# pmelchior/proxmin

Hardware: AMD Instinct MI355X
Metric: NMF iterations/sec at Y=16384x16384, K=64 (higher is better)
Workload: dtype f16x2r (fp16 split MFMA, fp32 accumulate: the residual from the high x high product + an exact K x K correction, two-term gradients; exact fp32's error class)

## Files before the change

### proxmin_amd/csrc/k_gfix.hip

```cpp
#include "pmx_common.h"

constexpr int GFIX_PARTS = 128;

struct GfixArgs {
    const float* X[2];
    int64_t rows[2];
    int K;
    const float* absmax;
    float* part;
    float* Q;
    float* out[2];
    int ld;
    int want[2];
    const DevStatus* status;
    long long* prof;
};
#define GFIX_STAMP(i) do { if (a.prof != nullptr && blockIdx.x == 0 && blockIdx.y == 0 && threadIdx.x == 0) a.prof[i] = wall_clock64(); } while (0)

typedef _Float16 gf16x8 __attribute__((ext_vector_type(8)));

__device__ __forceinline__ float gfix_scale(const float* absmax, int f, float* red) {
    float m = 0.f;
    for (int i = threadIdx.x; i < 256; i += blockDim.x) m = fmaxf(m, absmax[f * 256 + i]);
#pragma unroll
    for (int o = 32; o > 0; o >>= 1) m = fmaxf(m, __shfl_xor(m, o));
    if ((threadIdx.x & 63) == 0) red[threadIdx.x >> 6] = m;
    __syncthreads();
    float mx = red[0];
    for (int i = 1; i < (int)(blockDim.x >> 6); ++i) mx = fmaxf(mx, red[i]);
    int q = 0;
    (void)frexpf(mx, &q);
    return ldexpf(1.f, mx > 0.f ? 14 - q : 0);
}

template <int KT, int W>
__device__ __forceinline__ void gfix_gram_wave(const GfixArgs& a, int f, float* red) {
    constexpr int K = 32 * KT, TPW = KT * KT / 4, NB = KT == 2 ? 8 : 4;
    const int lane = threadIdx.x & 63, l31 = lane & 31, hi = lane >> 5;
    const int64_t rows = a.rows[f];
    const int64_t per = 16 * ((rows + 16 * GFIX_PARTS - 1) / (16 * GFIX_PARTS));
    const int64_t r0 = (int64_t)blockIdx.x * per, r1 = r0 + per < rows ? r0 + per : rows;
    const float* X = a.X[f] + 32 * 0 + l31;
    f32x16 acc0[TPW], accr[TPW];
#pragma unroll
    for (int t = 0; t < TPW; ++t)
#pragma unroll
        for (int i = 0; i < 16; ++i) { acc0[t][i] = 0.f; accr[t][i] = 0.f; }
    float v[NB][KT][8];
#define GFIX_REQUEST(rb_)                                                                          \
    _Pragma("unroll") for (int s = 0; s < NB; ++s)                                                 \
    _Pragma("unroll") for (int q = 0; q < 8; ++q) {                                                \
        const int64_t r = (rb_) + 16 * s + 8 * hi + q;                                             \
        _Pragma("unroll") for (int c = 0; c < KT; ++c) v[s][c][q] = r < r1 ? X[r * K + 32 * c] : 0.f; \
    }
    GFIX_STAMP(0);
    if (r0 < r1) { GFIX_REQUEST(r0) }
    const float sc = gfix_scale(a.absmax, f, red), un = 1.f / (sc * sc);
    GFIX_STAMP(1);
    for (int64_t rb = r0; rb < r1; rb += 16 * NB) {
        gf16x8 h[NB][KT], l[NB][KT];
#pragma unroll
        for (int s = 0; s < NB; ++s)
#pragma unroll
            for (int c = 0; c < KT; ++c)
#pragma unroll
                for (int q = 0; q < 8; ++q) {
                    const float x = v[s][c][q] * sc;
                    const _Float16 t = (_Float16)x;
                    h[s][c][q] = t;
                    l[s][c][q] = (_Float16)(x - (float)t);
                }
        if (rb + 16 * NB < r1) { GFIX_REQUEST(rb + 16 * NB) }
#pragma unroll
        for (int s = 0; s < NB; ++s)
#pragma unroll
            for (int t = 0; t < TPW; ++t) {
                constexpr int idx0 = W * TPW;
                const int ti = (idx0 + t) / KT, tj = (idx0 + t) % KT;
                acc0[t] = __builtin_amdgcn_mfma_f32_32x32x16_f16(h[s][ti], l[s][tj], acc0[t], 0, 0, 0);
                accr[t] = __builtin_amdgcn_mfma_f32_32x32x16_f16(l[s][ti], l[s][tj], accr[t], 0, 0, 0);
                acc0[t] = __builtin_amdgcn_mfma_f32_32x32x16_f16(h[s][ti], h[s][tj], acc0[t], 0, 0, 0);
                accr[t] = __builtin_amdgcn_mfma_f32_32x32x16_f16(l[s][ti], h[s][tj], accr[t], 0, 0, 0);
            }
    }
#undef GFIX_REQUEST
    GFIX_STAMP(2);
    float* out = a.part + ((int64_t)f * GFIX_PARTS + blockIdx.x) * 2 * K * K;
#pragma unroll
    for (int t = 0; t < TPW; ++t) {
        const int ti = (W * TPW + t) / KT, tj = (W * TPW + t) % KT;
#pragma unroll
        for (int i = 0; i < 16; ++i) {
            const int kp = 32 * ti + (i & 3) + 8 * (i >> 2) + 4 * hi, k = 32 * tj + l31;
            out[kp * K + k] = acc0[t][i] * un;
            out[K * K + kp * K + k] = accr[t][i] * un;
        }
    }
    GFIX_STAMP(3);
}
template <int W>
__device__ __forceinline__ void gfix_gram_wave_k128(const GfixArgs& a, int f, float* red, gf16x8* frag) {
    constexpr int K = 128, KT = 4, NB = 8;
    const int lane = threadIdx.x & 63, l31 = lane & 31, hi = lane >> 5;
    const int64_t rows = a.rows[f];
    const int64_t per = 16 * ((rows + 16 * GFIX_PARTS - 1) / (16 * GFIX_PARTS));
    const int64_t r0 = (int64_t)blockIdx.x * per, r1 = r0 + per < rows ? r0 + per : rows;
    const float* X = a.X[f] + 32 * W + l31;
    f32x16 acc0[KT], accr[KT];
#pragma unroll
    for (int t = 0; t < KT; ++t)
#pragma unroll
        for (int i = 0; i < 16; ++i) { acc0[t][i] = 0.f; accr[t][i] = 0.f; }
    float v[NB][8];
#define GFIX_REQUEST(rb_)                                                                          \
    _Pragma("unroll") for (int s = 0; s < NB; ++s)                                                 \
    _Pragma("unroll") for (int q = 0; q < 8; ++q) {                                                \
        const int64_t r = (rb_) + 16 * s + 8 * hi + q;                                             \
        v[s][q] = r < r1 ? X[r * K] : 0.f;                                                         \
    }
    if (r0 < r1) { GFIX_REQUEST(r0) }
    const float sc = gfix_scale(a.absmax, f, red), un = 1.f / (sc * sc);
    for (int64_t rb = r0; rb < r1; rb += 16 * NB) {
        gf16x8 h[NB], l[NB];
#pragma unroll
        for (int s = 0; s < NB; ++s) {
#pragma unroll
            for (int q = 0; q < 8; ++q) {
                const float x = v[s][q] * sc;
                const _Float16 t = (_Float16)x;
                h[s][q] = t;
                l[s][q] = (_Float16)(x - (float)t);
            }
            frag[((s * KT + W) * 2 + 0) * 64 + lane] = h[s];
            frag[((s * KT + W) * 2 + 1) * 64 + lane] = l[s];
        }
        if (rb + 16 * NB < r1) { GFIX_REQUEST(rb + 16 * NB) }
        __syncthreads();
#pragma unroll
        for (int s = 0; s < NB; ++s)
#pragma unroll
            for (int tj = 0; tj < KT; ++tj) {
                const gf16x8 hj = tj == W ? h[s] : frag[((s * KT + tj) * 2 + 0) * 64 + lane];
                const gf16x8 lj = tj == W ? l[s] : frag[((s * KT + tj) * 2 + 1) * 64 + lane];
                acc0[tj] = __builtin_amdgcn_mfma_f32_32x32x16_f16(h[s], lj, acc0[tj], 0, 0, 0);
                accr[tj] = __builtin_amdgcn_mfma_f32_32x32x16_f16(l[s], lj, accr[tj], 0, 0, 0);
                acc0[tj] = __builtin_amdgcn_mfma_f32_32x32x16_f16(h[s], hj, acc0[tj], 0, 0, 0);
                accr[tj] = __builtin_amdgcn_mfma_f32_32x32x16_f16(l[s], hj, accr[tj], 0, 0, 0);
            }
        __syncthreads();
    }
#undef GFIX_REQUEST
    float* out = a.part + ((int64_t)f * GFIX_PARTS + blockIdx.x) * 2 * K * K;
#pragma unroll
    for (int tj = 0; tj < KT; ++tj)
#pragma unroll
        for (int i = 0; i < 16; ++i) {
            const int kp = 32 * W + (i & 3) + 8 * (i >> 2) + 4 * hi, k = 32 * tj + l31;
            out[kp * K + k] = acc0[tj][i] * un;
            out[K * K + kp * K + k] = accr[tj][i] * un;
        }
}
template <int KT>
__global__ __launch_bounds__(256) void k_gfix_gram(GfixArgs a) {
    __shared__ float red[4];
    if (chain_halted(a.status)) return;
    const int f = blockIdx.y;
    if (!a.want[1 - f]) return;
    const int w = __builtin_amdgcn_readfirstlane(threadIdx.x >> 6);
    if constexpr (KT == 4) {
        extern __shared__ gf16x8 gfrag[];
        if (w == 0) gfix_gram_wave_k128<0>(a, f, red, gfrag);
        else if (w == 1) gfix_gram_wave_k128<1>(a, f, red, gfrag);
        else if (w == 2) gfix_gram_wave_k128<2>(a, f, red, gfrag);
        else gfix_gram_wave_k128<3>(a, f, red, gfrag);
    } else {
        if (w == 0) gfix_gram_wave<KT, 0>(a, f, red);
        else if (w == 1) gfix_gram_wave<KT, 1>(a, f, red);
        else if (w == 2) gfix_gram_wave<KT, 2>(a, f, red);
        else gfix_gram_wave<KT, 3>(a, f, red);
    }
}

__global__ __launch_bounds__(256) void k_gfix_reduce(GfixArgs a) {
    if (chain_halted(a.status)) return;
    const int f = blockIdx.y;
    if (!a.want[1 - f]) return;
    GFIX_STAMP(4);
    const int n = 2 * a.K * a.K;
    const int t = blockIdx.x * 256 + threadIdx.x, e = t >> 2, q = t & 3;
    static_assert(GFIX_PARTS == 128, "four threads x 32 partials");
    double s = 0.0;
    if (e < n) {
        const float* p = a.part + (int64_t)f * GFIX_PARTS * n + (int64_t)(q * 32) * n + e;
        float v[32];
#pragma unroll
        for (int i = 0; i < 32; ++i) v[i] = p[(int64_t)i * n];
#pragma unroll
        for (int i = 0; i < 32; ++i) s += (double)v[i];
    }
    const int base = threadIdx.x & 60;
    double tot = __shfl(s, base);
#pragma unroll
    for (int i = 1; i < 4; ++i) tot += __shfl(s, base + i);
    if (e < n && q == 0) a.Q[(int64_t)f * n + e] = (float)tot;
    GFIX_STAMP(5);
}

template <int KT>
__global__ __launch_bounds__(KT == 4 ? 512 : 256) void k_gfix_apply(GfixArgs a) {
    constexpr int K = 32 * KT, LDQ = K + 8;
    constexpr int NT = KT == 4 ? 512 : 256, NW = NT / 64;
    extern __shared__ _Float16 qpl[];
    __shared__ float red[8];
    if (chain_halted(a.status)) return;
    const int f = blockIdx.y;
    if (!a.want[f]) return;
    const int tid = threadIdx.x, lane = tid & 63, w = tid >> 6, l31 = lane & 31, hi = lane >> 5;
    const int64_t rows = a.rows[f];
    const float* X = a.X[f];
    float* out = a.out[f];
    const int64_t ntask = (rows + 31) / 32 * KT, stride = (int64_t)gridDim.x * NW;
    if ((int64_t)blockIdx.x * NW >= ntask) return;
    GFIX_STAMP(6);
    f32x4 x[K / 16][2];
#define GFIX_LOAD_X(t_)                                                                                                   \
    {                                                                                                                     \
        const int64_t row_ = ((t_) / KT) * 32 + l31;                                                                      \
        const f32x4* xr = reinterpret_cast<const f32x4*>(X + (row_ < rows ? row_ : 0) * K + 8 * hi);                       \
        _Pragma("unroll") for (int ks = 0; ks < K / 16; ++ks) { x[ks][0] = xr[4 * ks]; x[ks][1] = xr[4 * ks + 1]; }       \
    }
    const int64_t task0 = (int64_t)blockIdx.x * NW + w;
    if (task0 < ntask) GFIX_LOAD_X(task0)
    constexpr int TPK = NT / K, NBLK = K / 8 / TPK;
    const int kcol = tid % K, kb0 = tid / K;
    float tq[2][NBLK][8];
    {
        const float* src = a.Q + (int64_t)(1 - f) * 2 * K * K;
#pragma unroll
        for (int m = 0; m < 2; ++m)
#pragma unroll
            for (int i = 0; i < NBLK; ++i)
#pragma unroll
                for (int e = 0; e < 8; ++e) tq[m][i][e] = src[(size_t)m * K * K + (size_t)(8 * (kb0 + TPK * i) + e) * K + kcol];
    }
    float mx[2] = {0.f, 0.f};
#pragma unroll
    for (int m = 0; m < 2; ++m)
#pragma unroll
        for (int i = 0; i < NBLK; ++i)
#pragma unroll
            for (int e = 0; e < 8; ++e) mx[m] = fmaxf(mx[m], fabsf(tq[m][i][e]));
#pragma unroll
    for (int o = 32; o > 0; o >>= 1) { mx[0] = fmaxf(mx[0], __shfl_xor(mx[0], o)); mx[1] = fmaxf(mx[1], __shfl_xor(mx[1], o)); }
    __shared__ float redq[2][NW];
    if (lane == 0) { redq[0][w] = mx[0]; redq[1][w] = mx[1]; }
    const float sc = gfix_scale(a.absmax, f, red);
    GFIX_STAMP(7);
    float sq[2];
#pragma unroll
    for (int m = 0; m < 2; ++m) {
        float v = redq[m][0];
#pragma unroll
        for (int i = 1; i < NW; ++i) v = fmaxf(v, redq[m][i]);
        int q = 0;
        (void)frexpf(v, &q);
        sq[m] = ldexpf(1.f, v > 0.f ? 14 - q : 0);
    }
#pragma unroll
    for (int m = 0; m < 2; ++m) {
        _Float16* ph = qpl + (size_t)((1 - m) * 2) * K * LDQ + (size_t)kcol * LDQ;
        _Float16* pl = ph + (size_t)K * LDQ;
#pragma unroll
        for (int i = 0; i < NBLK; ++i) {
            gf16x8 h8, l8;
#pragma unroll
            for (int e = 0; e < 8; ++e) {
                const float v = tq[m][i][e] * sq[m];
                const _Float16 h = (_Float16)v;
                h8[e] = h;
                l8[e] = (_Float16)(v - (float)h);
            }
            *reinterpret_cast<gf16x8*>(ph + 8 * (kb0 + TPK * i)) = h8;
            *reinterpret_cast<gf16x8*>(pl + 8 * (kb0 + TPK * i)) = l8;
        }
    }
    __syncthreads();
    GFIX_STAMP(8);
    for (int64_t task = (int64_t)blockIdx.x * NW + w; task < ntask; task += stride) {
        const int64_t rt = task / KT;
        const int c = (int)(task % KT);
        const bool live = rt * 32 + l31 < rows;
        if (task != task0) GFIX_LOAD_X(task)
        f32x16 acc1, acc2;
#pragma unroll
        for (int i = 0; i < 16; ++i) { acc1[i] = 0.f; acc2[i] = 0.f; }
        const _Float16* qb = qpl + (size_t)(32 * c + l31) * LDQ + 8 * hi;
#pragma unroll
        for (int ks = 0; ks < K / 16; ++ks) {
            gf16x8 xh, xl, xm;
#pragma unroll
            for (int e = 0; e < 8; ++e) {
                const float v = (live ? x[ks][e >> 2][e & 3] : 0.f) * sc;
                const _Float16 h = (_Float16)v;
                const float r1 = v - (float)h;
                const _Float16 l = (_Float16)r1;
                xh[e] = h; xl[e] = l; xm[e] = (_Float16)(r1 - (float)l);
            }
            const gf16x8 qrh = *reinterpret_cast<const gf16x8*>(qb + 16 * ks);
            const gf16x8 qrl = *reinterpret_cast<const gf16x8*>(qb + (size_t)K * LDQ + 16 * ks);
            const gf16x8 q0h = *reinterpret_cast<const gf16x8*>(qb + (size_t)2 * K * LDQ + 16 * ks);
            const gf16x8 q0l = *reinterpret_cast<const gf16x8*>(qb + (size_t)3 * K * LDQ + 16 * ks);
            acc1 = __builtin_amdgcn_mfma_f32_32x32x16_f16(xl, qrh, acc1, 0, 0, 0);
            acc2 = __builtin_amdgcn_mfma_f32_32x32x16_f16(xm, q0h, acc2, 0, 0, 0);
            acc1 = __builtin_amdgcn_mfma_f32_32x32x16_f16(xh, qrl, acc1, 0, 0, 0);
            acc2 = __builtin_amdgcn_mfma_f32_32x32x16_f16(xl, q0l, acc2, 0, 0, 0);
            acc1 = __builtin_amdgcn_mfma_f32_32x32x16_f16(xh, qrh, acc1, 0, 0, 0);
            acc2 = __builtin_amdgcn_mfma_f32_32x32x16_f16(xl, q0h, acc2, 0, 0, 0);
        }
        const float u1 = 1.f / (sc * sq[1]), u2 = 1.f / (sc * sq[0]);
#pragma unroll
        for (int i = 0; i < 16; ++i) {
            const int64_t r = rt * 32 + (i & 3) + 8 * (i >> 2) + 4 * hi;
            if (r < rows) out[r * a.ld + 32 * c + l31] = acc1[i] * u1 + acc2[i] * u2;
        }
        GFIX_STAMP(9);
    }
#undef GFIX_LOAD_X
    GFIX_STAMP(10);
}

static hipError_t launch_gfix(const GfixArgs& a, hipStream_t s) {
    const int n = 2 * a.K * a.K;
    const size_t lds = (size_t)4 * a.K * (a.K + 8) * sizeof(_Float16);
    const int64_t rmax = a.rows[0] > a.rows[1] ? a.rows[0] : a.rows[1];
    const int nw = a.K == 128 ? 8 : 4;
    unsigned nb = (unsigned)(((rmax + 31) / 32 * (a.K / 32) + nw - 1) / nw);
    if (nb > (a.K == 128 ? 128u : 256u)) nb = a.K == 128 ? 128 : 256;
    if (a.K == 64) {
        hipError_t e = hipFuncSetAttribute((const void*)k_gfix_apply<2>, hipFuncAttributeMaxDynamicSharedMemorySize, (int)lds);
        if (e != hipSuccess) return e;
        hipLaunchKernelGGL(k_gfix_gram<2>, dim3(GFIX_PARTS, 2), dim3(256), 0, s, a);
        hipLaunchKernelGGL(k_gfix_reduce, dim3((n * 4 + 255) / 256, 2), dim3(256), 0, s, a);
        hipLaunchKernelGGL(k_gfix_apply<2>, dim3(nb, 2), dim3(256), lds, s, a);
    } else if (a.K == 128) {
        hipError_t e = hipFuncSetAttribute((const void*)k_gfix_apply<4>, hipFuncAttributeMaxDynamicSharedMemorySize, (int)lds);
        if (e != hipSuccess) return e;
        e = hipFuncSetAttribute((const void*)k_gfix_gram<4>, hipFuncAttributeMaxDynamicSharedMemorySize, 64 * 1024);
        if (e != hipSuccess) return e;
        hipLaunchKernelGGL(k_gfix_gram<4>, dim3(GFIX_PARTS, 2), dim3(256), 64 * 1024, s, a);
        hipLaunchKernelGGL(k_gfix_reduce, dim3((n * 4 + 255) / 256, 2), dim3(256), 0, s, a);
        hipLaunchKernelGGL(k_gfix_apply<4>, dim3(nb, 2), dim3(512), lds, s, a);
    } else return hipErrorInvalidValue;
    return hipGetLastError();
}
```

### proxmin_amd/csrc/k_update.hip

```cpp
#include <type_traits>
#include "pmx_common.h"

template <int CTRL>
__device__ __forceinline__ float dpp_f(float v) {
    return __builtin_bit_cast(float, __builtin_amdgcn_update_dpp(0, __builtin_bit_cast(int, v), CTRL, 0xf, 0xf, true));
}
template <int CTRL>
__device__ __forceinline__ double dpp_d(double v) {
    const unsigned long long u = __builtin_bit_cast(unsigned long long, v);
    const unsigned lo = (unsigned)__builtin_amdgcn_update_dpp(0, (int)(unsigned)u, CTRL, 0xf, 0xf, true);
    const unsigned hi = (unsigned)__builtin_amdgcn_update_dpp(0, (int)(unsigned)(u >> 32), CTRL, 0xf, 0xf, true);
    return __builtin_bit_cast(double, ((unsigned long long)hi << 32) | lo);
}
constexpr int DPP_XOR1 = 0xB1, DPP_XOR2 = 0x4E, DPP_HALF_MIRROR = 0x141, DPP_MIRROR = 0x140;
constexpr int SWZ_XOR16 = (0x10 << 10) | 0x1f;

constexpr int SWZ_XOR8 = (0x08 << 10) | 0x1f, SWZ_XOR4 = (0x04 << 10) | 0x1f;
__device__ __forceinline__ double swz16_d(double v) {
    const unsigned long long u = __builtin_bit_cast(unsigned long long, v);
    const unsigned lo = (unsigned)__builtin_amdgcn_ds_swizzle((int)(unsigned)u, SWZ_XOR16);
    const unsigned hi = (unsigned)__builtin_amdgcn_ds_swizzle((int)(unsigned)(u >> 32), SWZ_XOR16);
    return __builtin_bit_cast(double, ((unsigned long long)hi << 32) | lo);
}
template <class T, int G>
// ... 1440 lines not shown
                }
                cs[c] += x;
            }
        }
    ROW_LOOP_END
    double red[2] = {(double)d2, (double)n2};
    block_sum_store<2>(red, part_ptr(a.s.partials, SL_DIFF2, j) + blockIdx.x, (int64_t)2 * EW_BLOCKS, scratch);
    colsum_store<NC>(cs, a.colpart, j, sm);
    if (a.absmax_out != nullptr) {
        const double m = wave_max((double)xmax);
        __syncthreads();
        if ((threadIdx.x & 63) == 0) scratch[threadIdx.x >> 6] = m;
        __syncthreads();
        if (threadIdx.x == 0) {
            double mm = scratch[0];
            for (int q = 1; q < EW_WAVES; ++q) mm = fmax(mm, scratch[q]);
            a.absmax_out[j * EW_BLOCKS + blockIdx.x] = (float)mm;
        }
    }
}

struct AdaDecideArgs {
    AlphaArgs al;
    double* partials;
    double e_rel[2];
    int check_convergence;
    int has_prox[2];
    int host_tau[2];
};
__global__ __launch_bounds__(EW_THREADS) void k_ada_decide(AdaDecideArgs a) {
    __shared__ double scratch[EW_WAVES];
    DevStatus* st = a.al.status;
    if (chain_halted(st)) return;
    __shared__ int need;
    if (threadIdx.x == 0) need = st->need_sub[0] | st->need_sub[1];
    __syncthreads();
    if (need) {
        if (threadIdx.x == 0) {
            st->reason = HALT_NEED_SUB;
            __threadfence();
            st->halt = 1;
        }
        return;
    }
    double d[2] = {0, 0}, n[2] = {0, 0};
    if (a.check_convergence)
        for (int j = 0; j < 2; ++j) {
            d[j] = fold_partials(part_ptr(a.partials, SL_DIFF2, j), scratch);
            n[j] = fold_partials(part_ptr(a.partials, SL_NORM2, j), scratch);
        }
    compute_alpha(a.al);
    if (threadIdx.x == 0) {
        int all = 1;
        for (int j = 0; j < 2; ++j) {
            const int c = a.check_convergence ? (d[j] <= a.e_rel[j] * a.e_rel[j] * n[j]) : 0;
            st->conv[j] = c;
            st->norms[j][0] = d[j];
            st->norms[j][1] = n[j];
            all &= c;
            const int tau = a.has_prox[j] ? st->sub_tau[j] : a.host_tau[j];
            st->sub_total[j] += tau;
            st->last_tau[j] = tau;
            st->sub_done[j] = 0;
            st->sub_tau[j] = 0;
        }
        st->it_done += 1;
        if (a.check_convergence && all) {
            st->stopped = 1;
            st->reason = HALT_CONVERGED;
            __threadfence();
            st->halt = 1;
        }
    }
}

struct GridBar {
    unsigned cnt[8][16];
    unsigned top[16];
    unsigned gen[8][16];
    unsigned verdict[16];
    unsigned epoch[16];
};
__device__ __forceinline__ unsigned gb_load(const unsigned* p) { return __hip_atomic_load(p, __ATOMIC_RELAXED, __HIP_MEMORY_SCOPE_AGENT); }
__device__ __forceinline__ void gb_store(unsigned* p, unsigned v) { __hip_atomic_store(p, v, __ATOMIC_RELAXED, __HIP_MEMORY_SCOPE_AGENT); }
__device__ __forceinline__ void gb_arrive(GridBar* b, unsigned e, bool census) {
    const unsigned ng = 8, per = gridDim.x / ng, g = blockIdx.x & 7;
    const unsigned a = __hip_atomic_fetch_add(&b->cnt[g][0], 1u, __ATOMIC_RELAXED, __HIP_MEMORY_SCOPE_AGENT);
    if (a + 1 == per * e) {
        const unsigned t = __hip_atomic_fetch_add(&b->top[0], 1u, __ATOMIC_RELAXED, __HIP_MEMORY_SCOPE_AGENT);
        if (t + 1 == ng * e) {
            unsigned word = 2 * e;
            if (census) {
                unsigned expect = 2 * (e - 1);
                if (!__hip_atomic_compare_exchange_strong(&b->verdict[0], &expect, word, __ATOMIC_RELAXED, __ATOMIC_RELAXED, __HIP_MEMORY_SCOPE_AGENT)) word = expect;
            } else {
                gb_store(&b->verdict[0], word);
            }
            for (unsigned q = 0; q < ng; ++q) gb_store(&b->gen[q][0], word);
        }
    }
}
__device__ __forceinline__ unsigned gb_wait(GridBar* b, unsigned e, long long give_up_ticks) {
    const unsigned g = blockIdx.x & 7;
    const long long t0 = wall_clock64();
    for (;;) {
        const unsigned v = gb_load(&b->gen[g][0]);
        if ((v >> 1) >= e) return v;
        __builtin_amdgcn_s_sleep(4);
        if (give_up_ticks > 0 && wall_clock64() - t0 > give_up_ticks) {
            unsigned expect = 2 * (e - 1);
            if (__hip_atomic_compare_exchange_strong(&b->verdict[0], &expect, 2 * e + 1, __ATOMIC_RELAXED, __ATOMIC_RELAXED, __HIP_MEMORY_SCOPE_AGENT)) {
                for (unsigned q = 0; q < 8; ++q) gb_store(&b->gen[q][0], 2 * e + 1);
                return 2 * e + 1;
            }
            give_up_ticks = 0;
        }
    }
}
__device__ __forceinline__ void gb_sync(GridBar* b, unsigned e, DevStatus* st) {
    asm volatile("s_waitcnt vmcnt(0)" ::: "memory");
    __syncthreads();
    if (threadIdx.x == 0) {
        gb_arrive(b, e, false);
        const unsigned g = blockIdx.x & 7;
        const long long t0 = wall_clock64();
        for (unsigned spins = 1; (gb_load(&b->gen[g][0]) >> 1) < e; ++spins) {
            __builtin_amdgcn_s_sleep(4);
            if ((spins & 1023u) == 0 && wall_clock64() - t0 > 10000000) {
                st->tail_fault = 2;
                st->reason = HALT_ERROR;
                __threadfence();
                st->halt = 1;
                break;
            }
        }
    }
    __syncthreads();
}

constexpr int TAIL_NT = 4;
struct TailArgs {
    MomentArgs m;
    ProxSeq prox[2];
    double e_rel[2];
    int prox_max_iter;
    double* colpart;
    float* absmax_out;
    AlphaArgs al;
    int decide_check;
    GridBar* bar;
    int slots[2];
    long long* prof;
    int prof_fine;
};
template <int NC>
__global__ __launch_bounds__(EW_THREADS) void k_ada_tail(TailArgs a) {
    __shared__ double scratch[4 * TAIL_NT * EW_WAVES];
    __shared__ double dbuf[EW_BLOCKS + 8];
    __shared__ unsigned s_word;
    extern __shared__ float lds[];
    static_assert(EW_BLOCKS == 2 * MAXK, "the step-size phase gives one (block, component) to each workgroup");
    DevStatus* st = a.m.status;
    if (chain_halted(st)) return;
    const int tid = threadIdx.x, l32 = tid & 31;
    const int K = a.m.K;
    GridBar* bar = a.bar;
    unsigned ep = bar->epoch[0];
    int nstamp = 0;
    auto stamp = [&]() { if (a.prof != nullptr && blockIdx.x == 0 && tid == 0) a.prof[nstamp++] = wall_clock64(); };
    stamp();
    if (tid == 0) gb_arrive(bar, ep + 1, true);
    const int64_t hw = ((int64_t)blockIdx.x * EW_THREADS + tid) >> 5;
    const int64_t nhw = ((int64_t)EW_BLOCKS * EW_THREADS) >> 5;
    const int nslot = a.slots[0] + a.slots[1];
    float* Lx = lds;
    float* Lz = lds + (size_t)nslot * NC * EW_THREADS;
    float* Lp = lds + (size_t)2 * nslot * NC * EW_THREADS;
    auto slot = [&](int j, int i, int c) { return ((size_t)((j ? a.slots[0] : 0) + i) * NC + c) * EW_THREADS + tid; };
    bool ok[NC];
#pragma unroll
    for (int c = 0; c < NC; ++c) ok[c] = l32 + 32 * c < K;
    const MomentScalars ms = moment_scalars(a.m);
    const bool any_prox = a.m.has_prox[0] || a.m.has_prox[1];

    float g_pre[NC], x_pre[NC];
    const bool pre = a.slots[0] > 0 && hw < a.m.rows[0];
    if (pre) {
        load_grad<NC>(g_pre, ok, a.m.slab[0], a.m.rows[0], K, hw, l32);
#pragma unroll
        for (int c = 0; c < NC; ++c) x_pre[c] = ok[c] ? a.m.X[0][hw * K + l32 + 32 * c] : 0.f;
    }
    float alpha0[NC], alpha1[NC];
#pragma unroll
    for (int c = 0; c < NC; ++c) {
        alpha0[c] = ok[c] ? st->alpha[0][l32 + 32 * c] : 0.f;
        alpha1[c] = ok[c] ? st->alpha[1][l32 + 32 * c] : 0.f;
    }
    const int last_tau0 = st->last_tau[0], last_tau1 = st->last_tau[1];
    {
        if (tid == 0) s_word = gb_wait(bar, ep + 1, 200000);
        __syncthreads();
        if (s_word & 1u) {
            if (blockIdx.x == 0 && tid == 0) {
                st->tail_fault = 1;
                st->reason = HALT_ERROR;
                __threadfence();
                st->halt = 1;
            }
            return;
        }
        ep += 1;
    }
    stamp();
    float mpsi0 = -1.f, mpsi1 = -1.f;
    for (int j = 0; j < 2; ++j) {
        const int64_t rows = a.m.rows[j];
        float alpha[NC];
#pragma unroll
        for (int c = 0; c < NC; ++c) alpha[c] = j ? alpha1[c] : alpha0[c];
        float maxpsi = -1.f;
        for (int i = 0; i < a.slots[j]; ++i) {
            const int64_t r = hw + (int64_t)i * nhw;
            if (r >= rows) break;
            float g[NC], xo[NC];
            if (j == 0 && i == 0 && pre) {
#pragma unroll
                for (int c = 0; c < NC; ++c) { g[c] = g_pre[c]; xo[c] = x_pre[c]; }
            } else {
                load_grad<NC>(g, ok, a.m.slab[j], rows, K, r, l32);
#pragma unroll
                for (int c = 0; c < NC; ++c) xo[c] = ok[c] ? a.m.X[j][r * K + l32 + 32 * c] : 0.f;
            }
#pragma unroll
            for (int c = 0; c < NC; ++c) {
                if (!ok[c]) continue;
                const int64_t e = r * K + l32 + 32 * c;
                float psi;
                const float xn = moment_elem(a.m, ms, j, e, g[c], alpha[c], xo[c], psi);
                if (a.m.check_convergence) a.m.Xp[j][e] = xo[c];
                Lx[slot(j, i, c)] = xn;
                Lp[slot(j, i, c)] = psi;
                maxpsi = nanmaxf(maxpsi, psi);
            }
        }
        if (j) mpsi1 = maxpsi; else mpsi0 = maxpsi;
    }
    {
        const double mv0 = wave_nanmax((double)mpsi0), mv1 = wave_nanmax((double)mpsi1);
        __syncthreads();
        if ((tid & 63) == 0) { scratch[tid >> 6] = mv0; scratch[EW_WAVES + (tid >> 6)] = mv1; }
        __syncthreads();
        if (tid == 0 || tid == 64) {
            const int jj = tid >> 6;
            double m = scratch[jj * EW_WAVES];
            for (int q = 1; q < EW_WAVES; ++q) m = nanmax(m, scratch[jj * EW_WAVES + q]);
            sc1_store(part_ptr(a.m.partials, SL_MAXPSI, jj) + blockIdx.x, m);
        }
    }

    int tau0 = 0, tau1 = 0;
    stamp();
    if (any_prox) {
        gb_sync(bar, ++ep, st);
        stamp();
        bool done0 = !a.m.has_prox[0], done1 = !a.m.has_prox[1];
        double mp0, mp1;
        {
            const int lane = tid & 63;
            const double* q0 = part_ptr(a.m.partials, SL_MAXPSI, 0);
            const double* q1 = part_ptr(a.m.partials, SL_MAXPSI, 1);
            double u0[EW_BLOCKS / 64], u1[EW_BLOCKS / 64];
#pragma unroll
            for (int i = 0; i < EW_BLOCKS / 64; ++i) { u0[i] = sc1_load(q0 + i * 64 + lane); u1[i] = sc1_load(q1 + i * 64 + lane); }
            double v0 = -1.0, v1 = -1.0;
#pragma unroll
            for (int i = 0; i < EW_BLOCKS / 64; ++i) { v0 = nanmax(v0, u0[i]); v1 = nanmax(v1, u1[i]); }
            mp0 = wave_nanmax(v0);
            mp1 = wave_nanmax(v1);
        }
        stamp();
        auto steps = [&](int j, float (&gam)[NC], float (&rat)[NC]) {
            const float mp = (float)(j ? mp1 : mp0);
#pragma unroll
            for (int c = 0; c < NC; ++c) {
                const float al = j ? alpha1[c] : alpha0[c];
                gam[c] = al / mp;
                rat[c] = gam[c] / al;
            }
        };
        auto passes = [&](int j, int i, int n, bool first_round, const float (&gam)[NC], const float (&rat)[NC], float (&z)[NC],
                          auto sums_c, float (&d2)[TAIL_NT], float (&n2)[TAIL_NT]) {
            constexpr bool SUMS = decltype(sums_c)::value;
            float x[NC], ps[NC];
#pragma unroll
            for (int c = 0; c < NC; ++c) {
                x[c] = Lx[slot(j, i, c)];
                ps[c] = Lp[slot(j, i, c)];
                z[c] = first_round ? x[c] : Lz[slot(j, i, c)];
                if (!ok[c]) { x[c] = 0.f; ps[c] = 0.f; z[c] = 0.f; }
            }
#pragma unroll
            for (int q = 0; q < TAIL_NT; ++q) {
                if (q < n) {
                    float v[NC];
#pragma unroll
                    for (int c = 0; c < NC; ++c) v[c] = z[c] - rat[c] * ps[c] * (z[c] - x[c]);
                    prox_row(v, ok, a.prox[j], gam);
#pragma unroll
                    for (int c = 0; c < NC; ++c) {
                        if (SUMS && ok[c]) {
                            const float d = v[c] - z[c];
                            d2[q] += d * d;
                            n2[q] += z[c] * z[c];
                        }
                        z[c] = v[c];
                    }
                }
            }
        };
        using yes = std::integral_constant<bool, true>;
        using no = std::integral_constant<bool, false>;
        int t0_0 = 0, t0_1 = 0;
        for (int round = 0; !(done0 && done1); ++round) {
            int nt_0 = TAIL_NT, nt_1 = TAIL_NT;
            if (round == 0) {
                const int l0 = last_tau0, l1 = last_tau1;
                nt_0 = l0 >= 1 && l0 <= TAIL_NT ? l0 : TAIL_NT;
                nt_1 = l1 >= 1 && l1 <= TAIL_NT ? l1 : TAIL_NT;
            }
            double red[2][2 * TAIL_NT];
#pragma unroll
            for (int q = 0; q < 2 * TAIL_NT; ++q) { red[0][q] = 0.0; red[1][q] = 0.0; }
            for (int j = 0; j < 2; ++j) {
                if (j ? done1 : done0) continue;
                const int nt = j ? nt_1 : nt_0;
                float gam[NC], rat[NC];
                steps(j, gam, rat);
                float d2[TAIL_NT], n2[TAIL_NT];
#pragma unroll
                for (int q = 0; q < TAIL_NT; ++q) { d2[q] = 0.f; n2[q] = 0.f; }
                for (int i = 0; i < a.slots[j]; ++i) {
                    if (hw + (int64_t)i * nhw >= a.m.rows[j]) break;
                    float z[NC];
                    passes(j, i, nt, round == 0, gam, rat, z, yes{}, d2, n2);
                    if (round == 0) {
#pragma unroll
                        for (int c = 0; c < NC; ++c) Lz[slot(j, i, c)] = z[c];
                    }
                }
#pragma unroll
                for (int q = 0; q < TAIL_NT; ++q) {
                    if (j) { red[1][2 * q] = (double)d2[q]; red[1][2 * q + 1] = (double)n2[q]; }
                    else { red[0][2 * q] = (double)d2[q]; red[0][2 * q + 1] = (double)n2[q]; }
                }
                if (round == 0 && a.prof_fine) stamp();
            }
            {
                static_assert(4 * TAIL_NT == 16, "wave_sum16");
                const int lane = tid & 63, w = tid >> 6;
                double all[16];
#pragma unroll
                for (int q = 0; q < 2 * TAIL_NT; ++q) { all[q] = red[0][q]; all[2 * TAIL_NT + q] = red[1][q]; }
                const double tot = wave_sum16(all);
                __syncthreads();
                if (lane < 16) scratch[lane * EW_WAVES + w] = tot;
                __syncthreads();
                if (tid < 4 * TAIL_NT) {
                    const int jj = tid / (2 * TAIL_NT), q = tid - jj * 2 * TAIL_NT;
                    if (!(jj ? done1 : done0)) {
                        double sum = 0.0;
                        for (int u = 0; u < EW_WAVES; ++u) sum += scratch[tid * EW_WAVES + u];
                        sc1_store(part_ptr(a.m.partials, SL_SUBR0 + 2 * TAIL_NT * (round & 3), jj) + blockIdx.x + (int64_t)q * 2 * EW_BLOCKS, sum);
                    }
                }
            }
            if (round == 0) stamp();
            gb_sync(bar, ++ep, st);
            if (round == 0) stamp();
            for (int j = 0; j < 2; ++j) {
                if (j ? done1 : done0) continue;
                const int nt = j ? nt_1 : nt_0, t0 = j ? t0_1 : t0_0;
                const int w = tid >> 6;
                __syncthreads();
                if (w < 2 * nt) {
// ... 602 lines not shown
};
template <int NC>
__global__ __launch_bounds__(EW_THREADS) void k_shard_pack_split(PackSplitArgs a) {
    const int64_t ex0 = a.sncol * a.K;
    const int64_t sc0 = ex0 + (int64_t)a.KP * a.KP + 2 * MAXK;
    if (chain_halted(a.status)) {
        if (blockIdx.x == 0 && threadIdx.x < a.world) a.comm[threadIdx.x * a.chunk + sc0 + SHARD_HALT_SLOT] = 1.f;
        return;
    }
    const int K = a.K;
    if (blockIdx.x >= PACK_XWG) {
        if (a.fold_grad) {
            const int l32 = threadIdx.x & 31;
            const int64_t hw_ = ((int64_t)(blockIdx.x - PACK_XWG) * EW_THREADS + threadIdx.x) >> 5;
            const int64_t nhw_ = ((int64_t)EW_BLOCKS * EW_THREADS) >> 5;
            for (int64_t r = hw_; r < a.N; r += nhw_) {
                bool ok[NC];
                float g[NC];
#pragma unroll
                for (int c = 0; c < NC; ++c) ok[c] = l32 + 32 * c < K;
                load_grad<NC>(g, ok, a.slabS, a.N, K, r, l32);
                const int q = (int)r / (int)a.sncol;
                float* dst = a.comm + (int64_t)q * a.chunk + (int64_t)((int)r - q * (int)a.sncol) * K;
#pragma unroll
                for (int c = 0; c < NC; ++c)
                    if (ok[c]) dst[l32 + 32 * c] = g[c];
            }
        }
        return;
    }
    const int t = threadIdx.x;
    if (blockIdx.x < 2) {
        const int j = blockIdx.x;
        __shared__ double asum[ALPHA_NG][MAXK];
        colsum_fold(a.colpart + (int64_t)j * EW_BLOCKS * MAXK, K, false, asum);
        if (t < MAXK) {
            double s = 0.0;
            for (int q = 0; q < ALPHA_NG; ++q) s += asum[q][t];
            const float v = (float)s;
            for (int q = 0; q < a.world; ++q) a.comm[q * a.chunk + ex0 + (int64_t)a.KP * a.KP + j * MAXK + t] = v;
        }
        return;
    }
    const double* const four[4] = {a.partials + ((int64_t)SL_DIFF2 * 2 + 0) * EW_BLOCKS, a.partials + ((int64_t)SL_NORM2 * 2 + 0) * EW_BLOCKS,
                                   a.partials + ((int64_t)SL_DIFF2 * 2 + 1) * EW_BLOCKS, a.partials + ((int64_t)SL_NORM2 * 2 + 1) * EW_BLOCKS};
    double sums[4];
    fold_partials_many<4>(four, sums);
    for (int q = 0; q < a.world; ++q) {
        float* ex = a.comm + q * a.chunk + ex0;
        if (a.gramA != nullptr)
            for (int e = t; e < a.KP * a.KP; e += EW_THREADS) ex[e] = (float)a.gramA[e];
        else if (a.zero_gram)
            for (int e = t; e < a.KP * a.KP; e += EW_THREADS) ex[e] = 0.f;
        if (t < 32) ex[a.KP * a.KP + 2 * MAXK + t] = t < 4 ? (float)sums[t] : 0.f;
    }
}
struct ShardPostSplitArgs {
    DevStatus* status;
    const float* extras;
    int64_t rows_global[2];
    int K;
    int use_fixed;
    float fixed[2];
    double e_rel[2];
    int check_convergence;
    int have_prev;
};
__global__ __launch_bounds__(EW_THREADS) void k_shard_post_split(ShardPostSplitArgs a) {
    DevStatus* st = a.status;
    if (chain_halted(st)) return;
    const float* sc = a.extras + 2 * MAXK;
    if (sc[SHARD_HALT_SLOT] > 0.5f) {
        if (threadIdx.x == 0) {
            st->reason = HALT_PEER;
            __threadfence();
            st->halt = 1;
        }
        return;
    }
    const int t = threadIdx.x;
    if (a.use_fixed != 2 && t < a.K)
        for (int j = 0; j < 2; ++j)
            st->alpha[j][t] = a.use_fixed ? a.fixed[j] : (float)((double)a.extras[j * MAXK + t] / (double)a.rows_global[j]) / 10.f;
    if (a.check_convergence && a.have_prev && t == 0) {
        const double dA = (double)sc[0], nA = (double)sc[1], dS = (double)sc[2], nS = (double)sc[3];
        const int cA = dA <= a.e_rel[0] * a.e_rel[0] * nA;
        const int cS = dS <= a.e_rel[1] * a.e_rel[1] * nS;
        st->conv[0] = cA;
        st->conv[1] = cS;
        st->norms[0][0] = dA; st->norms[0][1] = nA;
        st->norms[1][0] = dS; st->norms[1][1] = nS;
        if (cA && cS) {
            st->stopped = 1;
            st->reason = HALT_CONVERGED;
            __threadfence();
            st->halt = 1;
        }
    }
}

#define DISPATCH_NC(K, KERNEL, grid, stream, args)                                               \
    do {                                                                                         \
        if ((K) <= 32) hipLaunchKernelGGL(KERNEL<1>, grid, dim3(EW_THREADS), 0, stream, args);    \
        else if ((K) <= 64) hipLaunchKernelGGL(KERNEL<2>, grid, dim3(EW_THREADS), 0, stream, args); \
        else hipLaunchKernelGGL(KERNEL<4>, grid, dim3(EW_THREADS), 0, stream, args);              \
    } while (0)

#define DISPATCH_NC_ME(K, me, KERNEL, grid, stream, args)                                                          \
    do {                                                                                                           \
        if (!(me)) DISPATCH_NC(K, KERNEL, grid, stream, args);                                                     \
        else if ((K) <= 32) hipLaunchKernelGGL((KERNEL<1, true>), grid, dim3(EW_THREADS), 0, stream, args);         \
        else if ((K) <= 64) hipLaunchKernelGGL((KERNEL<2, true>), grid, dim3(EW_THREADS), 0, stream, args);         \
        else hipLaunchKernelGGL((KERNEL<4, true>), grid, dim3(EW_THREADS), 0, stream, args);                        \
    } while (0)

void launch_fold(const FoldArgs& a, int nblocks_y, hipStream_t s) { DISPATCH_NC(a.K, k_fold, dim3(EW_BLOCKS, nblocks_y), s, a); }
void launch_prox_apply(const ProxArgs& a, hipStream_t s) { DISPATCH_NC_ME(a.K, seq_has_me(a.prox), k_prox_apply, dim3(EW_BLOCKS), s, a); }
void launch_pgm_update(const PgmArgs& a, hipStream_t s) {
    DISPATCH_NC_ME(a.K, seq_has_me(a.prox[0]) || seq_has_me(a.prox[1]), k_pgm_update, dim3(a.nbx > 0 ? a.nbx : EW_BLOCKS, 2), s, a);
}
void launch_pgm_unity(const PgmUnityArgs& a, hipStream_t s) {
    DISPATCH_NC_ME(a.u.K, seq_has_me(a.u.prox[0]) || seq_has_me(a.u.prox[1]), k_pgm_unity, dim3(a.u.nbx > 0 ? a.u.nbx : EW_BLOCKS, 2), s, a);
}
void launch_bb_reduce(const BBArgs& a, hipStream_t s) { DISPATCH_NC(a.K, k_bb_reduce, dim3(EW_BLOCKS, 2), s, a); }
void launch_bb_step(const BBStepArgs& a, hipStream_t s) { hipLaunchKernelGGL(k_bb_step, dim3(1), dim3(EW_THREADS), 0, s, a); }
void launch_bt_update(const BtArgs& a, hipStream_t s) { DISPATCH_NC_ME(a.K, seq_has_me(a.prox[0]) || seq_has_me(a.prox[1]), k_bt_update, dim3(EW_BLOCKS, 2), s, a); }
void launch_bt_collect(const BtCollectArgs& a, hipStream_t s) { hipLaunchKernelGGL(k_bt_collect, dim3(1), dim3(EW_THREADS), 0, s, a); }
void launch_bt_finish(const BtFinishArgs& a, hipStream_t s) { hipLaunchKernelGGL(k_bt_finish, dim3(EW_BLOCKS, 2), dim3(EW_THREADS), 0, s, a); }
void launch_pgm_decide(const DecideArgs& a, hipStream_t s) { hipLaunchKernelGGL(k_pgm_decide, dim3(1), dim3(EW_THREADS), 0, s, a); }
void launch_colsum(const ColsumArgs& a, hipStream_t s) { DISPATCH_NC(a.K, k_colsum, dim3(EW_BLOCKS, 2), s, a); }
void launch_alpha_init(const AlphaArgs& a, hipStream_t s) { hipLaunchKernelGGL(k_alpha_init, dim3(1), dim3(EW_THREADS), 0, s, a); }
void launch_colscale(const ColScaleArgs& a, hipStream_t s) { DISPATCH_NC(a.K, k_colscale, dim3(EW_BLOCKS), s, a); }
void launch_ada_moment(const MomentArgs& a, hipStream_t s) { DISPATCH_NC(a.K, k_ada_moment, dim3(EW_BLOCKS, 2), s, a); }
#define DISPATCH_NC_NT(K, NT, ME, KERNEL, grid, stream, args)                                                      \
    do {                                                                                                           \
        if ((K) <= 32) hipLaunchKernelGGL((KERNEL<1, NT, ME>), grid, dim3(EW_THREADS), 0, stream, args);            \
        else if ((K) <= 64) hipLaunchKernelGGL((KERNEL<2, NT, ME>), grid, dim3(EW_THREADS), 0, stream, args);       \
        else hipLaunchKernelGGL((KERNEL<4, NT, ME>), grid, dim3(EW_THREADS), 0, stream, args);                      \
    } while (0)
template <bool ME>
static void launch_ada_sub_t(const SubArgs& a, hipStream_t s) {
    if (a.nt == 1) DISPATCH_NC_NT(a.K, 1, ME, k_ada_sub, dim3(EW_BLOCKS, 2), s, a);
    else if (a.nt == 4) DISPATCH_NC_NT(a.K, 4, ME, k_ada_sub, dim3(EW_BLOCKS, 2), s, a);
    else DISPATCH_NC_NT(a.K, SUB_NT_MAX, ME, k_ada_sub, dim3(EW_BLOCKS, 2), s, a);
}
void launch_ada_sub(const SubArgs& a, hipStream_t s) {
    if (seq_has_me(a.prox[0]) || seq_has_me(a.prox[1])) launch_ada_sub_t<true>(a, s);
    else launch_ada_sub_t<false>(a, s);
}
void launch_ada_finish(const FinishArgs& a, hipStream_t s) {
    DISPATCH_NC_ME(a.s.K, seq_has_me(a.s.prox[0]) || seq_has_me(a.s.prox[1]), k_ada_finish, dim3(EW_BLOCKS, 2), s, a);
}
void launch_ada_decide(const AdaDecideArgs& a, hipStream_t s) { hipLaunchKernelGGL(k_ada_decide, dim3(1), dim3(EW_THREADS), 0, s, a); }
static size_t ada_tail_lds_bytes(const TailArgs& a) {
    const int NC = a.m.K <= 32 ? 1 : (a.m.K <= 64 ? 2 : 4);
    const size_t arr = (size_t)(a.slots[0] + a.slots[1]) * NC * EW_THREADS * sizeof(float);
    return 2 * arr + std::max(arr, (size_t)(EW_THREADS / 32) * MAXK * sizeof(float));
}
constexpr size_t ADA_TAIL_LDS_MAX = 160 * 1024 - 6 * 1024;
template <int NC>
static hipError_t launch_ada_tail_t(const TailArgs& a, hipStream_t s) {
    const size_t lds = ada_tail_lds_bytes(a);
    hipError_t e = hipFuncSetAttribute((const void*)k_ada_tail<NC>, hipFuncAttributeMaxDynamicSharedMemorySize, (int)lds);
    if (e != hipSuccess) return e;
    hipLaunchKernelGGL(k_ada_tail<NC>, dim3(EW_BLOCKS), dim3(EW_THREADS), lds, s, a);
    return hipGetLastError();
}
hipError_t launch_ada_tail(const TailArgs& a, hipStream_t s) {
    if (a.m.K <= 32) return launch_ada_tail_t<1>(a, s);
    if (a.m.K <= 64) return launch_ada_tail_t<2>(a, s);
    return launch_ada_tail_t<4>(a, s);
}
void launch_bsdmm_update(const BsdmmArgs& a, hipStream_t s) {
    bool me = seq_has_me(a.prox_f);
    for (int i = 0; i < a.n_g && i < PMX_MAX_G; ++i) me = me || seq_has_me(a.prox_g[i]);
    DISPATCH_NC_ME(a.K, me, k_bsdmm_update, dim3(EW_BLOCKS), s, a);
}
void launch_shard_pack(const PackArgs& a, hipStream_t s) { DISPATCH_NC(a.K, k_shard_pack, dim3(EW_BLOCKS + PACK_XWG), s, a); }
void launch_shard_gram_in(const GramInArgs& a, hipStream_t s) { hipLaunchKernelGGL(k_shard_gram_in, dim3((a.n + 255) / 256), dim3(256), 0, s, a); }
void launch_shard_post(const ShardPostArgs& a, hipStream_t s) { hipLaunchKernelGGL(k_shard_post, dim3(1), dim3(EW_THREADS), 0, s, a); }
void launch_shard_pack_split(const PackSplitArgs& a, hipStream_t s) { DISPATCH_NC(a.K, k_shard_pack_split, dim3(EW_BLOCKS + PACK_XWG), s, a); }
void launch_shard_post_split(const ShardPostSplitArgs& a, hipStream_t s) { hipLaunchKernelGGL(k_shard_post_split, dim3(1), dim3(EW_THREADS), 0, s, a); }
void launch_bsdmm_decide(const BsdmmDecideArgs& a, hipStream_t s) { hipLaunchKernelGGL(k_bsdmm_decide, dim3(1), dim3(EW_THREADS), 0, s, a); }
```

### proxmin_amd/csrc/pmx_api.hip

```cpp
#include <stdarg.h>
#include <stdio.h>
#include <string.h>
#include <math.h>
#include <vector>
#include <string>
#include <algorithm>
#include <mutex>

#include <fcntl.h>
#include <sys/file.h>
#include <unistd.h>
#include <dlfcn.h>
#include <link.h>
#include "pmx_common.h"
#include "chain_link.h"
#include "k_grad.hip"
#include "k_grad_bf16.hip"
#include "k_grad_k128.hip"
#include "k_grad_f16_k32.hip"
#include "k_grad_f32pc.hip"
#include "k_update.hip"
#include "k_gram.hip"
#include "k_gfix.hip"
#include "k_small_f64.hip"
#include "k_grad_f64.hip"
#include "k_big_f64.hip"
#include "k_xfer.hip"

static thread_local char g_err[512] = "";
void pmx_set_error(const char* fmt, ...) {
    va_list ap;
    va_start(ap, fmt);
    vsnprintf(g_err, sizeof(g_err), fmt, ap);
    va_end(ap);
}
#define FAIL(code, ...)            \
    do {                           \
        pmx_set_error(__VA_ARGS__); \
        return (code);             \
    } while (0)

enum Algo { ALG_NONE = 0, ALG_PGM, ALG_ADAPROX, ALG_BSDMM };

struct pmx_ctx {
    int device = 0;
    hipStream_t stream = nullptr;
    bool own_stream = false;
    int64_t M = 0, N = 0, K = 0;
    int KP = 0, mode = PMX_MODE_F32;
    int64_t rows[2] = {0, 0};

    const float* Y = nullptr;
    float* Yown = nullptr;
    int64_t ldY = 0;
    bool haveY = false;
    int64_t Mk = 0, Nk = 0;
    int64_t rowsK[2] = {0, 0};
    bool framed = false;
    int64_t Kk = 0;
    float* Xk[2] = {nullptr, nullptr};

    float* X[2] = {nullptr, nullptr};
    float* G[2] = {nullptr, nullptr};
    float* Xe[2] = {nullptr, nullptr};
    float* Xp[2] = {nullptr, nullptr};
    float* Mm[2] = {nullptr, nullptr};
    float* Vv[2] = {nullptr, nullptr};
    float* Vh[2] = {nullptr, nullptr};
    float* Psi[2] = {nullptr, nullptr};
    float* zb[2][2] = {{nullptr, nullptr}, {nullptr, nullptr}};
    float* Zg[2][PMX_MAX_G] = {};
    float* Ug[2][PMX_MAX_G] = {};
    float* bbX[2] = {nullptr, nullptr};
    float* bbG[2] = {nullptr, nullptr};

    bool f64 = false;
    double* Yd = nullptr;
    double* Xd[2] = {nullptr, nullptr};
    double* Xed[2] = {nullptr, nullptr};
    double* Gd[2] = {nullptr, nullptr};
    double* slabd[2] = {nullptr, nullptr};
    double* Md[2] = {nullptr, nullptr};
    double* Vd[2] = {nullptr, nullptr};
    double* Vhd[2] = {nullptr, nullptr};
    double* Xpd[2] = {nullptr, nullptr};
    double* Psid[2] = {nullptr, nullptr};
    double* zd[2] = {nullptr, nullptr};
    double* alpha64 = nullptr;
    double* Zd[2][PMX_MAX_G] = {};
    double* Ud[2][PMX_MAX_G] = {};
    int t64x = 0, t64y = 0;
    bool f64big = false;
    double* gramPart64 = nullptr;
    double* colpart64 = nullptr;
    int nsplit64[2] = {1, 1}, bps64[2] = {1, 1};
    int nsub64 = 4;
    bool Wd_on = false;
    double* Xprevd[2] = {nullptr, nullptr};
    double* Wd = nullptr;
    double* Xk64[2] = {nullptr, nullptr};
    int64_t ldY64 = 0;

    bool host_grad = false;
    float* Tg[2][PMX_MAX_G] = {};
    float* Tf[2] = {};
    unsigned long long* k1prof = nullptr;
    K1Kind k1 = K1_F32;
    bool k1_pairs = true;
    float rangeRatio = 65536.f;
    int rangeFaults = 0;
    int f16_r3 = 0;
    float* fixPart = nullptr;
    float* fixQ = nullptr;
    float* fixSlab[2] = {nullptr, nullptr};
    long long* fixProf = nullptr;
    bool fix_on = false;
    bool k1_sync_check = false;
    int ncu = 0;
    _Float16* A16[2] = {nullptr, nullptr};
    float* absmax = nullptr;
    float ymax = 0.f;
    float wmax = 1.f;
    bool absmax_by_finish = false;
    bool gram_by_update = false;
    bool bsd_decide_pending = false;
    BsdmmDecideArgs bsd_decide{};
    bool gram_fresh[2] = {false, false};
    bool gram_in_update = true;
    bool fold_in_k1 = true;
    K1GramFold k1_fold{};
    bool decide_pending = false;
    __bf16* Bp[2] = {nullptr, nullptr};
    __bf16* Bt[2] = {nullptr, nullptr};
    int64_t rowsPad[2] = {0, 0};
    GradPlan plan{};
    int chainL = 0;
    unsigned* chainFlags = nullptr;
    unsigned chainSeq = 0;
    int nSlabA = 0;
    int nSlabS = 0;
    int chainFaults = 0;
    int hook_inject_k1 = 0;
    std::string hook_tail_lockfile;
    bool tail_fused = false;
    GridBar* gridbar = nullptr;
    long long* tailprof = nullptr;
    unsigned* tickets = nullptr;
    bool pgm_long = false;
    double* unityPart = nullptr;
    unsigned ticketLaunches = 0;
    int tailFaults = 0;
    float* slab[2] = {nullptr, nullptr};
    const float* W = nullptr;
    int64_t ldW = 0;
    float* Wown = nullptr;
    double* lossPart = nullptr;
    int nloss = 0;

    double* partials = nullptr;
    double* colpart = nullptr;
    float* gramPart = nullptr;
    double* gramG = nullptr;
    double* eigQ = nullptr;
    DevStatus* dstatus = nullptr;
    DevStatus* hstatus = nullptr;

    Algo algo = ALG_NONE;
    pmx_pgm_params pgm{};
    pmx_adaprox_params ada{};
    pmx_bsdmm_params bsd{};
    int host_tau[2] = {0, 0};
    int it = 0;
    double nest_t = 1.0;
    double btT[2] = {1.0, 1.0};
    double bt_fprev = 0.0, bt_fnow = 0.0;
    bool bt_grad_fresh = false;
    int bt_pending = 0;
    int bt_trial = 3;
    float* btBuf[2] = {nullptr, nullptr};
    float omega_cur = 0.f;
    int nsub_guess = 2;
    int sub_nt = SUB_NT_MAX;
    struct SubRec { int it = -1, nt = 0, enq = 0; } sub_rec[64];
    std::vector<void*> allocs;

    bool timing = false;
    int timing_stride = 1;
    unsigned timing_seq = 0;
    std::vector<hipEvent_t> ev;
    size_t ev_used = 0;

    int ph_every = 0;
    unsigned ph_seq = 0;
    bool ph_cur = false, ph_prev = false;
    std::vector<hipEvent_t> ph_ev;
    std::vector<int> ph_mark;

    int rank = 0, world = 1;
    int64_t M_global = 0;
    float* comm = nullptr;
    bool comm_gram_dirty = true;
    bool shard_grad_from_comm = false;
    bool ssplit = false;
    int64_t scol0 = 0, sncol = 0;
    float* comm_out = nullptr;
    pmx_prox* tabs = nullptr;
    bool tab_set[PMX_MAX_TABLES] = {};
    float* stepArr[2] = {nullptr, nullptr};
    int step_arr_mask = 0;
    void* rccl_comm = nullptr;
    int rccl_rank = 0, rccl_world = 0;
};

static int dalloc(pmx_ctx* c, void** p, size_t bytes, bool zero = true) {
    if (*p) return PMX_OK;
    hipError_t e = hipMalloc(p, bytes ? bytes : 16);
    if (e != hipSuccess) FAIL(PMX_E_NOMEM, "hipMalloc(%zu) failed: %s", bytes, hipGetErrorString(e));
    c->allocs.push_back(*p);
    if (zero) HIP_CHECK(hipMemsetAsync(*p, 0, bytes ? bytes : 16, c->stream));
    return PMX_OK;
}
template <class T>
static int dallocT(pmx_ctx* c, T** p, size_t count, bool zero = true) { return dalloc(c, (void**)p, count * sizeof(T), zero); }

static ProxSeq to_dev(const pmx_proxseq& p, const pmx_prox* tab) {
    ProxSeq d{};
    d.n = p.n;
    d.repeat = p.repeat < 1 ? 1 : p.repeat;
    for (int i = 0; i < PMX_MAX_SEQ; ++i) d.seq[i] = p.seq[i];
    d.tab = tab;
    return d;
}
static bool prox_long_axis(const pmx_proxseq& p) {
    for (int i = 0; i < p.n && i < PMX_MAX_SEQ; ++i)
        if ((p.seq[i].op == PMX_PROX_UNITY || p.seq[i].op == PMX_PROX_UNITY_PLUS) && p.seq[i].unit != 0) return true;
    return false;
}
static bool seq_is_projection(const pmx_proxseq& p) {
    for (int i = 0; i < p.n; ++i) {
        const pmx_prox& q = p.seq[i];
        const bool box = q.op == PMX_PROX_ID || q.op == PMX_PROX_ZERO || q.op == PMX_PROX_PLUS ||
                         ((q.op == PMX_PROX_MIN || q.op == PMX_PROX_MAX || q.op == PMX_PROX_HARD || q.op == PMX_PROX_HARD_PLUS) && !q.relative);
        if (!box) return false;
    }
    return true;
}
static bool prox_has_max_entropy(const pmx_proxseq& p) {
    for (int i = 0; i < p.n && i < PMX_MAX_SEQ; ++i)
        if (p.seq[i].op == PMX_PROX_MAX_ENTROPY || p.seq[i].op == PMX_PROX_COMPONENTS) return true;
    return false;
}
static bool row_op_ok(int op) {
    return op == PMX_PROX_ID || op == PMX_PROX_ZERO || op == PMX_PROX_PLUS || (op >= PMX_PROX_MIN && op <= PMX_PROX_MAX_ENTROPY);
}
static int check_prox(const pmx_proxseq& p, const char* what, bool long_axis_ok = false, const bool* tab_set = nullptr, int ntables = -1) {
    if (p.n < 0 || p.n > PMX_MAX_SEQ) FAIL(PMX_E_INVALID, "%s: bad operator count %d", what, p.n);
    for (int i = 0; i < p.n; ++i) {
        const pmx_prox& q = p.seq[i];
        if (q.op < PMX_PROX_ID || q.op > PMX_PROX_COMPONENTS) FAIL(PMX_E_INVALID, "%s: unknown prox op %d", what, q.op);
        if (q.op != PMX_PROX_COMPONENTS) continue;
        if (q.unit != 0) FAIL(PMX_E_INVALID, "%s: PMX_PROX_COMPONENTS works along the components of a row (unit 0)", what);
        if (q.reserved < 1) FAIL(PMX_E_INVALID, "%s: PMX_PROX_COMPONENTS without a table (reserved = 1 + its index)", what);
        if (tab_set != nullptr && q.reserved > PMX_MAX_TABLES)
            FAIL(PMX_E_UNSUPPORTED, "%s: table %d of at most %d per-component tables", what, q.reserved - 1, PMX_MAX_TABLES);
        if (tab_set != nullptr ? !tab_set[q.reserved - 1] : q.reserved > ntables)
            FAIL(PMX_E_INVALID, "%s: PMX_PROX_COMPONENTS names table %d, which has not been set (pmx_prox_table)", what, q.reserved - 1);
    }
    if (prox_long_axis(p) && !long_axis_ok)
        FAIL(PMX_E_UNSUPPORTED, "%s: prox_unity along the row dimension (numpy axis=0 on A / axis=1 on S) needs a grid-wide sum per "
                                "application: pgm / FISTA run it inside the update chain (pmx_pgm_begin without line search, user prox, "
                                "row sharding or fp64), every other solver entry point does not contain it (the host wrappers apply it "
                                "between kernel launches through pmx_prox_apply)", what);
    return PMX_OK;
}

static int apply_prox_standalone(float* X, int64_t rows, int K, const pmx_proxseq& prox, const float* step_k, double* colpart, hipStream_t stream,
                                 const pmx_prox* tab = nullptr) {
    bool along_rows = false;
    for (int i = 0; i < prox.n; ++i)
        along_rows |= (prox.seq[i].op == PMX_PROX_UNITY || prox.seq[i].op == PMX_PROX_UNITY_PLUS) && prox.seq[i].unit != 0;
    ProxArgs a{};
    a.X = X;
    a.rows = rows;
    a.K = K;
    for (int k = 0; k < K; ++k) a.stepk[k] = step_k[k];
    if (!along_rows) {
        a.prox = to_dev(prox, tab);
        launch_prox_apply(a, stream);
        return PMX_OK;
    }
    const int repeat = prox.repeat < 1 ? 1 : prox.repeat;
    for (int r = 0; r < repeat; ++r)
        for (int i = 0; i < prox.n; ++i) {
            pmx_proxseq one{};
            one.n = 1; one.repeat = 1; one.seq[0] = prox.seq[i];
            const bool rows_unity = (one.seq[0].op == PMX_PROX_UNITY || one.seq[0].op == PMX_PROX_UNITY_PLUS) && one.seq[0].unit != 0;
            if (!rows_unity) {
// ... 204 lines not shown
        if (rc == PMX_OK) rc = dallocT(c, &c->fixQ, (size_t)4 * c->Kk * c->Kk);
        for (int j = 0; j < 2 && rc == PMX_OK; ++j) rc = dallocT(c, &c->fixSlab[j], (size_t)c->rowsK[j] * c->Kk);
        if (rc == PMX_OK && getenv("PMX_GFIX_PROF")) rc = dallocT(c, &c->fixProf, 16);
    }
    for (int t = 0; t < 2 && rc == PMX_OK && c->k1 == K1_F16_K128; ++t) rc = dallocT(c, &c->A16[t], (size_t)Mk * c->Kk, c->framed || c->Kk != K);
    for (int j = 0; j < 2 && rc == PMX_OK && c->Kk != K; ++j) rc = dallocT(c, &c->Xk[j], (size_t)c->rowsK[j] * c->Kk);
    if (c->k1 == K1_BF16 || c->k1 == K1_BF16_V7 || c->k1 == K1_F16_V8) {
        for (int j = 0; j < 2 && rc == PMX_OK; ++j) {
            c->rowsPad[j] = (c->rowsK[j] + 127) / 128 * 128;
            rc = dallocT(c, &c->Bp[j], (size_t)3 * c->rowsPad[j] * c->KP, false);
            if (rc == PMX_OK) rc = dallocT(c, &c->Bt[j], (size_t)2 * c->KP * c->rowsPad[j], false);
        }
    }
    for (int j = 0; j < 2 && rc == PMX_OK; ++j) {
        rc = dallocT(c, &c->X[j], (size_t)c->rowsK[j] * K);
        if (rc == PMX_OK) rc = dallocT(c, &c->G[j], (size_t)c->rows[j] * K);
    }
    if (rc == PMX_OK) rc = dallocT(c, &c->slab[0], (size_t)c->nSlabA * Mk * c->Kk, false);
    if (rc == PMX_OK) rc = dallocT(c, &c->slab[1], (size_t)c->plan.nSlabS * Nk * c->Kk, false);
    if (rc == PMX_OK) rc = dallocT(c, &c->lossPart, (size_t)2 * c->plan.gridX * c->plan.gridY);
    if (rc == PMX_OK) rc = dallocT(c, &c->partials, (size_t)SL_COUNT * 2 * EW_BLOCKS);
    if (rc == PMX_OK) rc = dallocT(c, &c->colpart, (size_t)2 * EW_BLOCKS * MAXK);
    if (rc == PMX_OK) rc = dallocT(c, &c->gramPart, (size_t)2 * GRAM_BLOCKS * c->KP * c->KP);
    if (rc == PMX_OK) rc = dallocT(c, &c->gramG, (size_t)2 * c->KP * c->KP);
    if (rc == PMX_OK) rc = dallocT(c, &c->eigQ, (size_t)2 * c->KP * c->KP);
    if (rc == PMX_OK) rc = dallocT(c, &c->dstatus, 1);
    if (rc == PMX_OK) {
        hipError_t e = hipHostMalloc((void**)&c->hstatus, sizeof(DevStatus), hipHostMallocDefault);
        if (e != hipSuccess) { pmx_set_error("hipHostMalloc: %s", hipGetErrorString(e)); rc = PMX_E_NOMEM; }
    }
    if (rc != PMX_OK) { pmx_ctx_destroy(c); return rc; }
    *out = c;
    return PMX_OK;
}

extern "C" int pmx_ctx_destroy(pmx_ctx* c) {
    if (!c) return PMX_OK;
    (void)hipSetDevice(c->device);
    if (c->stream) (void)hipStreamSynchronize(c->stream);
    (void)pmx_comm_destroy(c);
    for (void* p : c->allocs) (void)hipFree(p);
    for (auto& e : c->ev) (void)hipEventDestroy(e);
    for (auto& e : c->ph_ev) (void)hipEventDestroy(e);
    if (c->hstatus) (void)hipHostFree(c->hstatus);
    if (c->own_stream && c->stream) (void)hipStreamDestroy(c->stream);
    delete c;
    return PMX_OK;
}

extern "C" int pmx_set_timing(pmx_ctx* c, int on) {
    if (!c) FAIL(PMX_E_INVALID, "ctx is NULL");
    HIP_CHECK(hipSetDevice(c->device));
    HIP_CHECK(hipStreamSynchronize(c->stream));
    if (on && c->ev.empty()) {
        c->ev.resize(2 * 8192);
        for (auto& e : c->ev) HIP_CHECK(hipEventCreate(&e));
    }
    c->timing = on != 0;
    c->timing_stride = on > 1 ? on : 1;
    c->timing_seq = 0;
    c->ev_used = 0;
    return PMX_OK;
}

extern "C" int pmx_get_timing(pmx_ctx* c, double* total_ms, int* launches) {
    if (!c || !total_ms || !launches) FAIL(PMX_E_INVALID, "NULL argument");
    HIP_CHECK(hipSetDevice(c->device));
    HIP_CHECK(hipStreamSynchronize(c->stream));
    std::vector<float> d;
    float mx = 0.f;
    for (size_t i = 0; i + 1 < c->ev_used; i += 2) {
        float ms = 0.f;
        HIP_CHECK(hipEventElapsedTime(&ms, c->ev[i], c->ev[i + 1]));
        d.push_back(ms);
        mx = std::max(mx, ms);
    }
    double tot = 0.0;
    int n = 0;
    for (float ms : d)
        if (ms >= 0.05f * mx) { tot += ms; ++n; }
    *total_ms = tot;
    *launches = n;
    return PMX_OK;
}

static int phase_mark(pmx_ctx* c, int m) {
    if (c->ph_every <= 0) return PMX_OK;
    if (m == 0) {
        if (c->ph_prev && c->ph_mark.size() < c->ph_ev.size()) {
            HIP_CHECK(hipEventRecord(c->ph_ev[c->ph_mark.size()], c->stream));
            c->ph_mark.push_back(6);
        }
        c->ph_cur = (c->ph_seq++ % (unsigned)c->ph_every) == 0 && c->ph_mark.size() + 8 <= c->ph_ev.size();
        c->ph_prev = c->ph_cur;
    }
    if (!c->ph_cur) return PMX_OK;
    HIP_CHECK(hipEventRecord(c->ph_ev[c->ph_mark.size()], c->stream));
    c->ph_mark.push_back(m);
    return PMX_OK;
}
extern "C" int pmx_set_phase_timing(pmx_ctx* c, int every) {
    if (!c) FAIL(PMX_E_INVALID, "ctx is NULL");
    HIP_CHECK(hipSetDevice(c->device));
    HIP_CHECK(hipStreamSynchronize(c->stream));
    if (every > 0 && c->ph_ev.empty()) {
        c->ph_ev.resize(4096);
        for (auto& e : c->ph_ev) HIP_CHECK(hipEventCreate(&e));
    }
    c->ph_every = every > 0 ? every : 0;
    c->ph_seq = 0;
    c->ph_cur = c->ph_prev = false;
    c->ph_mark.clear();
    return PMX_OK;
}
extern "C" int pmx_get_phase_timing(pmx_ctx* c, double ms[6], int* iterations) {
    if (!c || !ms || !iterations) FAIL(PMX_E_INVALID, "NULL argument");
    HIP_CHECK(hipSetDevice(c->device));
    HIP_CHECK(hipStreamSynchronize(c->stream));
    double sum[6] = {0, 0, 0, 0, 0, 0};
    int cnt[6] = {0, 0, 0, 0, 0, 0};
    for (size_t i = 0; i + 1 < c->ph_mark.size(); ++i) {
        const int a = c->ph_mark[i], b = c->ph_mark[i + 1];
        if (b != a + 1 || a > 5) continue;
        float t = 0.f;
        HIP_CHECK(hipEventElapsedTime(&t, c->ph_ev[i], c->ph_ev[i + 1]));
        sum[a] += t;
        cnt[a] += 1;
    }
    for (int a = 0; a < 6; ++a) ms[a] = cnt[a] ? sum[a] / cnt[a] : 0.0;
    *iterations = cnt[0];
    return PMX_OK;
}

extern "C" int pmx_k1_info(pmx_ctx* c, int info[8]) {
    if (!c || !info) FAIL(PMX_E_INVALID, "NULL argument");
    const K1Inst inst = k1_instance(c->k1, c->f16_r3, c->W != nullptr, true, c->k1_pairs);
    switch (c->k1) {
    case K1_F32: info[0] = 0; break;
    case K1_BF16: case K1_BF16_V7: info[0] = 1; break;
    case K1_F16_V8: info[0] = inst == K1_V7 ? 1 : inst == K1_HH ? 11 : inst == K1_R3 ? 9 : 2; break;
    case K1_SMALL: info[0] = 4; break;
    case K1_F16_K128: info[0] = inst == K1_HH ? 12 : 5; break;
    case K1_F32PC: info[0] = 6; break;
    case K1_F64_SMALL: info[0] = 7; break;
    case K1_F16_K32: info[0] = inst == K1_R3 ? 10 : 8; break;
    case K1_F64_BIG: info[0] = 13; break;
    }
    info[1] = c->chainL;
    info[2] = c->nSlabA;
    info[3] = c->nSlabS;
    info[4] = c->plan.gridX;
    info[5] = c->plan.gridY;
    info[6] = c->plan.RP;
    info[7] = c->chainFaults + 1000 * c->tailFaults + (c->tail_fused ? 1000000 : 0) + 10000000 * std::min(c->rangeFaults, 9);
    return PMX_OK;
}

extern "C" int pmx_k1_frame(pmx_ctx* c, int64_t frame[3]) {
    if (!c || !frame) FAIL(PMX_E_INVALID, "NULL argument");
    frame[0] = c->f64 ? c->M : c->Mk;
    frame[1] = c->f64 ? c->N : c->Nk;
    frame[2] = c->f64 ? c->K : c->Kk;
    return PMX_OK;
}

extern "C" int pmx_ctx_sync(pmx_ctx* c) {
    if (!c) FAIL(PMX_E_INVALID, "ctx is NULL");
    HIP_CHECK(hipStreamSynchronize(c->stream));
    return PMX_OK;
}

static int measure_ymax(pmx_ctx* c) {
    if (!k1_fp16(c->k1)) return PMX_OK;
    launch_absmax_pitched(c->Y, c->ldY, c->M, c->N, c->absmax + 512, c->stream);
    HIP_CHECK(hipGetLastError());
    float h[256];
    HIP_CHECK(hipMemcpyAsync(h, c->absmax + 512, sizeof(h), hipMemcpyDeviceToHost, c->stream));
    HIP_CHECK(hipStreamSynchronize(c->stream));
    float m = 0.f;
    for (float v : h) m = v > m ? v : m;
    if (!(m < 3.0e38f)) FAIL(PMX_E_INVALID, "Y contains non-finite values");
    c->ymax = m;
    return PMX_OK;
}

static int own_frame_copy(pmx_ctx* c, float** own, const float* src, int64_t ld, hipMemcpyKind kind) {
    if (!*own) {
        int rc = dallocT(c, own, (size_t)c->Mk * c->Nk, c->framed);
        if (rc != PMX_OK) return rc;
    }
    HIP_CHECK(hipMemcpy2DAsync(*own, c->Nk * sizeof(float), src, ld * sizeof(float), c->N * sizeof(float), c->M, kind, c->stream));
    HIP_CHECK(hipStreamSynchronize(c->stream));
    return PMX_OK;
}

extern "C" int pmx_set_Y_host(pmx_ctx* c, const float* Y, int64_t ld) {
    if (!c || !Y) FAIL(PMX_E_INVALID, "NULL argument");
    if (c->f64) FAIL(PMX_E_UNSUPPORTED, "an fp64 context takes Y through pmx_set_Y_host_f64");
    if (ld < c->N) FAIL(PMX_E_INVALID, "ld %lld < N", (long long)ld);
    HIP_CHECK(hipSetDevice(c->device));
    int rc = own_frame_copy(c, &c->Yown, Y, ld, hipMemcpyHostToDevice);
    if (rc != PMX_OK) return rc;
    c->Y = c->Yown;
    c->ldY = c->Nk;
    c->haveY = true;
    return measure_ymax(c);
}

extern "C" int pmx_set_Y_device(pmx_ctx* c, const float* dY, int64_t ld, int copy) {
    if (!c || !dY) FAIL(PMX_E_INVALID, "NULL argument");
    if (c->f64) FAIL(PMX_E_UNSUPPORTED, "an fp64 context takes Y through pmx_set_Y_host_f64");
    if (ld < c->N) FAIL(PMX_E_INVALID, "ld %lld < N", (long long)ld);
    HIP_CHECK(hipSetDevice(c->device));
    if (copy || c->framed) {
        int rc = own_frame_copy(c, &c->Yown, dY, ld, hipMemcpyDeviceToDevice);
        if (rc != PMX_OK) return rc;
        c->Y = c->Yown;
        c->ldY = c->Nk;
    } else {
        c->Y = dY;
        c->ldY = ld;
    }
    c->haveY = true;
    return measure_ymax(c);
}

static int measure_wmax(pmx_ctx* c) {
    c->wmax = 1.f;
    if (!k1_fp16(c->k1) || !c->W) return PMX_OK;
    launch_absmax_pitched(c->W, c->ldW, c->M, c->N, c->absmax + 512, c->stream);
    HIP_CHECK(hipGetLastError());
    float h[256];
    HIP_CHECK(hipMemcpyAsync(h, c->absmax + 512, sizeof(h), hipMemcpyDeviceToHost, c->stream));
    HIP_CHECK(hipStreamSynchronize(c->stream));
    float m = 1.f;
    for (float v : h) m = v > m ? v : m;
    if (!(m < 3.0e38f)) FAIL(PMX_E_INVALID, "W contains non-finite values");
    c->wmax = m;
    return PMX_OK;
}

static int set_W_common(pmx_ctx* c, const float* W, int64_t ld, int from_host, int copy) {
    if (c && c->f64 && W) FAIL(PMX_E_UNSUPPORTED, "weights are not implemented in fp64 contexts");
    if (!c) FAIL(PMX_E_INVALID, "ctx is NULL");
    if (!W) { c->W = nullptr; c->ldW = 0; c->wmax = 1.f; return PMX_OK; }
    if (ld < c->N) FAIL(PMX_E_INVALID, "ld %lld < N", (long long)ld);
    if (c->k1 == K1_F16_K32) FAIL(PMX_E_UNSUPPORTED, "k_grad_f16_k32 takes no weights; create the context with PMX_MODE_F32");
    if (c->k1 == K1_BF16)
        FAIL(PMX_E_UNSUPPORTED, "a weighted likelihood in a split-precision mode needs K = 64 with M %% 128 = 0, N %% 256 = 0 or K = 128 with M %% 128 = 0, N %% 128 = 0; create the context with PMX_MODE_F32");
    if (c->comm) FAIL(PMX_E_UNSUPPORTED, "weights are not supported in row-sharded runs");
    HIP_CHECK(hipSetDevice(c->device));
    if (from_host || copy || c->framed) {
        int rc = own_frame_copy(c, &c->Wown, W, ld, from_host ? hipMemcpyHostToDevice : hipMemcpyDeviceToDevice);
        if (rc != PMX_OK) return rc;
        c->W = c->Wown;
        c->ldW = c->Nk;
    } else {
        c->W = W;
        c->ldW = ld;
    }
    return measure_wmax(c);
}
extern "C" int pmx_set_W_host(pmx_ctx* c, const float* W, int64_t ld) { return set_W_common(c, W, ld, 1, 1); }
extern "C" int pmx_set_W_device(pmx_ctx* c, const float* dW, int64_t ld, int copy) { return set_W_common(c, dW, ld, 0, copy); }

static int buf_lookup(pmx_ctx* c, int buf, float*** slot, int64_t* count, bool create) {
    if (c->f64) FAIL(PMX_E_UNSUPPORTED, "an fp64 context has no float arrays: pmx_upload_f64 / pmx_download_f64");
    int j;
    float** p = nullptr;
    if (buf >= PMX_BUF_A && buf <= PMX_BUF_PSI_ST) {
        j = buf & 1;
        switch (buf >> 1) {
            case 0: p = &c->X[j]; break;
            case 1: p = &c->G[j]; break;
            case 2: p = &c->Mm[j]; break;
            case 3: p = &c->Vv[j]; break;
            case 4: p = &c->Vh[j]; break;
            case 5: p = (c->algo == ALG_PGM && c->pgm.accelerated) ? &c->Xe[j] : &c->X[j]; break;
            case 6: p = &c->Xp[j]; break;
            case 7: p = &c->Psi[j]; break;
        }
    } else if (buf >= PMX_BUF_Z0 && buf < PMX_BUF_Z0 + 2 * PMX_MAX_G) {
        j = (buf - PMX_BUF_Z0) / PMX_MAX_G;
        p = &c->Zg[j][(buf - PMX_BUF_Z0) % PMX_MAX_G];
    } else if (buf >= PMX_BUF_U0 && buf < PMX_BUF_U0 + 2 * PMX_MAX_G) {
        j = (buf - PMX_BUF_U0) / PMX_MAX_G;
        p = &c->Ug[j][(buf - PMX_BUF_U0) % PMX_MAX_G];
    } else if (buf >= PMX_BUF_TG0 && buf < PMX_BUF_TG0 + 2 * PMX_MAX_G) {
        j = (buf - PMX_BUF_TG0) / PMX_MAX_G;
        p = &c->Tg[j][(buf - PMX_BUF_TG0) % PMX_MAX_G];
    } else if (buf == PMX_BUF_STEP_A || buf == PMX_BUF_STEP_ST) {
        j = buf - PMX_BUF_STEP_A;
        p = &c->stepArr[j];
    } else if (buf == PMX_BUF_BT_A || buf == PMX_BUF_BT_ST) {
        j = buf - PMX_BUF_BT_A;
        p = &c->btBuf[j];
    } else FAIL(PMX_E_INVALID, "unknown buffer id %d", buf);
    *count = c->rows[j] * c->K;
    if (!*p) {
        if (!create) FAIL(PMX_E_STATE, "buffer %d has not been created yet", buf);
        int rc = dallocT(c, p, (size_t)c->rowsK[j] * c->K);
        if (rc != PMX_OK) return rc;
    }
    *slot = p;
    return PMX_OK;
}

// ... 172 lines not shown
extern "C" int pmx_factor_from_device(pmx_ctx* c, int buf, const void* dptr, int64_t stride0, int64_t stride1, int is_f64) {
    if (c) { c->absmax_by_finish = false; c->gram_by_update = false; c->bt_grad_fresh = false; }
    void* arr; int64_t rows, sr, sk;
    int rc = xfer_lookup(c, buf, dptr, stride0, stride1, is_f64, true, &arr, &rows, &sr, &sk);
    if (rc != PMX_OK) return rc;
    HIP_CHECK(hipDeviceSynchronize());
    if (c->f64) launch_xfer<double>((double*)arr, (double*)const_cast<void*>(dptr), rows, c->K, sr, sk, false, c->stream);
    else launch_xfer<float>((float*)arr, (float*)const_cast<void*>(dptr), rows, c->K, sr, sk, false, c->stream);
    HIP_CHECK(hipGetLastError());
    HIP_CHECK(hipStreamSynchronize(c->stream));
    return PMX_OK;
}

extern "C" int pmx_factor_to_device(pmx_ctx* c, int buf, void* dptr, int64_t stride0, int64_t stride1, int is_f64) {
    void* arr; int64_t rows, sr, sk;
    int rc = xfer_lookup(c, buf, dptr, stride0, stride1, is_f64, false, &arr, &rows, &sr, &sk);
    if (rc != PMX_OK) return rc;
    if (c->f64) launch_xfer<double>((double*)arr, (double*)dptr, rows, c->K, sr, sk, true, c->stream);
    else launch_xfer<float>((float*)arr, (float*)dptr, rows, c->K, sr, sk, true, c->stream);
    HIP_CHECK(hipGetLastError());
    HIP_CHECK(hipStreamSynchronize(c->stream));
    return PMX_OK;
}

static int read_status(pmx_ctx* c) {
    HIP_CHECK(hipMemcpyAsync(c->hstatus, c->dstatus, sizeof(DevStatus), hipMemcpyDeviceToHost, c->stream));
    HIP_CHECK(hipStreamSynchronize(c->stream));
    return PMX_OK;
}

static int reset_status(pmx_ctx* c) {
    DevStatus s;
    memset(&s, 0, sizeof(s));
    for (int f = 0; f < 2; ++f)
        for (int k = 0; k < MAXK; ++k) s.eigvec[f][k] = 1.0;
    memcpy(c->hstatus, &s, sizeof(s));
    HIP_CHECK(hipMemcpyAsync(c->dstatus, c->hstatus, sizeof(DevStatus), hipMemcpyHostToDevice, c->stream));
    HIP_CHECK(hipStreamSynchronize(c->stream));
    return PMX_OK;
}

static const char* chain_error_text(pmx_ctx* c) {
    if (c->hstatus && c->hstatus->k1_fault == 4)
        return "mode f16x2: K max|A| max|S| is more than 2^16 max|Y| -- one fp16 scale cannot carry this residual (f16_range_fault); create the context with PMX_MODE_F32";
    return "device chain reported an error";
}
static int clear_halt(pmx_ctx* c) {
    static const int zeros[2] = {0, 0};
    HIP_CHECK(hipMemcpyAsync(&c->dstatus->halt, zeros, sizeof(int) * 2, hipMemcpyHostToDevice, c->stream));
    HIP_CHECK(hipMemcpyAsync(&c->dstatus->need_sub[0], zeros, sizeof(int) * 2, hipMemcpyHostToDevice, c->stream));
    return PMX_OK;
}

static int chain_disable(pmx_ctx* c) {
    if (c->chainL == 0) return PMX_OK;
    c->chainL = 0;
    c->nSlabA = c->plan.nSlabA;
    float* big = nullptr;
    int rc = dallocT(c, &big, (size_t)c->nSlabA * c->Mk * c->Kk, false);
    if (rc != PMX_OK) return rc;
    c->slab[0] = big;
    return PMX_OK;
}
static int one_iteration_per_call(pmx_ctx* c) {
    c->k1_sync_check = true;
    return chain_disable(c);
}
static int k1_leave_f16(pmx_ctx* c) {
    c->mode = PMX_MODE_F32;
    select_k1(c, c->Mk, c->Nk, c->ncu);
    c->fix_on = false;
    if (c->k1_sync_check) {
        c->chainL = 0;
        c->nSlabA = c->plan.nSlabA;
    }
    c->chainFlags = nullptr;
    c->chainSeq = 0;
    c->slab[0] = c->slab[1] = nullptr;
    c->lossPart = nullptr;
    int rc = PMX_OK;
    if (c->chainL > 0) rc = dallocT(c, &c->chainFlags, (size_t)(c->plan.gridX * c->plan.gridY / c->chainL) * c->plan.RP * 4);
    if (rc == PMX_OK) rc = dallocT(c, &c->slab[0], (size_t)c->nSlabA * c->Mk * c->Kk, false);
    if (rc == PMX_OK) rc = dallocT(c, &c->slab[1], (size_t)c->plan.nSlabS * c->Nk * c->Kk, false);
    if (rc == PMX_OK) rc = dallocT(c, &c->lossPart, (size_t)2 * c->plan.gridX * c->plan.gridY);
    c->rangeFaults += 1;
    return rc;
}
static int chain_fault_fallback(pmx_ctx* c, int* again) {
    *again = 0;
    if (!c->hstatus->k1_fault && !c->hstatus->tail_fault) return PMX_OK;
    if (c->hstatus->tail_fault == 2)
        FAIL(PMX_E_HIP, "k_ada_tail: a grid barrier timed out after the census had passed (a workgroup was lost); the factors are not usable");
    int rc = PMX_OK;
    if (c->hstatus->k1_fault == 4) {
        rc = k1_leave_f16(c);
        if (rc != PMX_OK) return rc;
    } else if (c->hstatus->k1_fault) {
        rc = chain_disable(c);
        if (rc != PMX_OK) return rc;
        c->chainFaults += 1;
    }
    if (c->hstatus->tail_fault) {
        c->tail_fused = false;
        c->tailFaults += 1;
    }
    static const int zeros[4] = {0, 0, 0, 0};
    HIP_CHECK(hipMemcpyAsync(&c->dstatus->tail_fault, zeros, 3 * sizeof(int), hipMemcpyHostToDevice, c->stream));
    rc = clear_halt(c);
    if (rc != PMX_OK) return rc;
    HIP_CHECK(hipStreamSynchronize(c->stream));
    if (c->tickets) {
        HIP_CHECK(hipMemsetAsync(c->tickets, 0, sizeof(unsigned), c->stream));
        HIP_CHECK(hipStreamSynchronize(c->stream));
        c->ticketLaunches = 0;
    }
    c->hstatus->k1_fault = 0;
    c->hstatus->tail_fault = 0;
    c->hstatus->halt = 0;
    c->hstatus->reason = 0;
    c->absmax_by_finish = false;
    c->gram_by_update = false;
    *again = 1;
    return PMX_OK;
}

static GradArgs small_grad_args(pmx_ctx* c, const float* A, const float* St, int doA, int doS) {
    GradArgs g{};
    g.Y = c->Y; g.ldY = c->ldY;
    g.W = c->W; g.ldW = c->ldW;
    g.A = A; g.St = St;
    g.slabA = c->slab[0]; g.slabS = c->slab[1];
    g.lossPart = c->lossPart;
    g.status = c->dstatus;
    g.M = (int)c->Mk; g.N = (int)c->Nk; g.K = (int)c->Kk;
    g.RP = c->plan.RP;
    g.doA = doA; g.doS = doS;
    return g;
}
static bool eig_small_applies(const pmx_ctx* c) { return c->K <= 16 && c->M <= 8192 && c->N <= 8192; }
static EigArgs small_eig_args(pmx_ctx* c, const float* A, const float* St, bool wantStepA, bool wantStepS, double scale) {
    EigArgs e{};
    e.G = c->gramG; e.Gw = c->gramG; e.KP = c->KP; e.K = (int)c->K; e.status = c->dstatus;
    e.want[0] = wantStepS; e.want[1] = wantStepA;
    e.scale = scale;
    e.max_iter = 200;
    e.Q = c->eigQ;
    e.X[0] = A; e.X[1] = St;
    e.rows[0] = c->M; e.rows[1] = c->N;
    return e;
}

static int k1_prio_for(int kk) { return kk == 64 ? 0 : 1; }

static int enqueue_gfix(pmx_ctx* c, const float* A, const float* St, int doA, int doS, hipStream_t stream) {
    GfixArgs f{};
    f.X[0] = A; f.X[1] = St;
    f.rows[0] = c->M; f.rows[1] = c->N;
    f.K = (int)c->Kk;
    f.absmax = c->absmax;
    f.part = c->fixPart; f.Q = c->fixQ;
    f.out[0] = c->fixSlab[0]; f.out[1] = c->fixSlab[1];
    f.ld = (int)c->Kk;
    f.want[0] = (doA & 1) != 0; f.want[1] = doS != 0;
    f.status = c->dstatus;
    f.prof = c->fixProf;
    HIP_CHECK(launch_gfix(f, stream));
    return PMX_OK;
}

static void enqueue_absmax(pmx_ctx* c, const float* A, const float* St) {
    AbsmaxArgs am{};
    am.X[0] = A; am.X[1] = St;
    am.count[0] = c->M * c->Kk; am.count[1] = c->N * c->Kk;
    am.out = c->absmax;
    am.status = c->dstatus;
    launch_absmax(am, c->stream);
}
template <class Args>
static int chain_arm(pmx_ctx* c, Args& g) {
    if (c->chainSeq >= (1u << 21)) {
        HIP_CHECK(hipMemsetAsync(c->chainFlags, 0, (size_t)(c->plan.gridX * c->plan.gridY / c->chainL) * c->plan.RP * 4 * sizeof(unsigned), c->stream));
        c->chainSeq = 0;
    }
    g.chainL = c->chainL; g.chainFlags = c->chainFlags; g.chainBase = (++c->chainSeq) * 64u; g.wstatus = c->dstatus;
    g.chainInject = c->hook_inject_k1 > 0 && (int)c->chainSeq == c->hook_inject_k1;
    return PMX_OK;
}
template <class Launch>
static int k1_timed(pmx_ctx* c, Launch&& launch) {
    const bool timed = c->timing && (c->timing_seq++ % (unsigned)c->timing_stride) == 0 && c->ev_used + 2 <= c->ev.size();
    if (timed) HIP_CHECK(hipEventRecord(c->ev[c->ev_used], c->stream));
    HIP_CHECK(launch());
    c->nloss = c->plan.gridX * c->plan.gridY;
    if (timed) {
        HIP_CHECK(hipEventRecord(c->ev[c->ev_used + 1], c->stream));
        c->ev_used += 2;
    }
    return PMX_OK;
}
static GradV4Args v4_args(pmx_ctx* c, const float* A, const float* St, int doA, int doS) {
    GradV4Args g{};
    g.Y = c->Y; g.ldY = c->ldY;
    g.A = A; g.St = St;
    g.slabA = c->slab[0]; g.slabS = c->slab[1];
    g.lossPart = c->lossPart;
    g.status = c->dstatus;
    g.M = (int)c->Mk; g.N = (int)c->Nk;
    g.RP = c->plan.RP;
    g.doA = doA; g.doS = doS;
    g.gridX = c->plan.gridX; g.gridY = c->plan.gridY;
    return g;
}
static void v4_f16_args(pmx_ctx* c, GradV4Args& g, int kk) {
    g.absmax = c->absmax; g.ymax = c->ymax; g.wmax = c->wmax;
    g.wstatus = c->dstatus; g.rangeRatio = c->rangeRatio; g.r3 = c->f16_r3; g.consPrio = k1_prio_for(kk);
}

static int enqueue_small_front(pmx_ctx* c, const float* A, const float* St, double scale) {
    const GradArgs g = small_grad_args(c, A, St, 1, 1);
    const EigArgs e = small_eig_args(c, A, St, true, true, scale);
    return k1_timed(c, [&] { return launch_small_front(c->plan, g, e, c->stream); });
}

static int enqueue_grad_once(pmx_ctx* c, const float* A, const float* St, int doA, int doS, bool absmax_fresh) {
    const K1GramFold fold = c->k1_fold;
    c->k1_fold = K1GramFold{};
    if (c->host_grad) return PMX_OK;
    if (c->Kk != c->K) {
        PadArgs pa{};
        pa.src[0] = A; pa.src[1] = St;
        pa.dst[0] = c->Xk[0]; pa.dst[1] = c->Xk[1];
        pa.rows[0] = c->M; pa.rows[1] = c->N;
        pa.K = (int)c->K; pa.Kk = (int)c->Kk;
        pa.status = c->dstatus;
        launch_pad_factors(pa, c->stream);
        A = c->Xk[0]; St = c->Xk[1];
    }
    const bool grad = (doA & 1) || doS;
    if (k1_fp16(c->k1) && !absmax_fresh) enqueue_absmax(c, A, St);
    K1Inst inst = K1_PLAIN;
    int rc = PMX_OK;
    switch (c->k1) {
    case K1_F16_K128: {
        SplitAArgs sp{};
        sp.X = A; sp.count = c->M * c->Kk;  sp.absmax = c->absmax; sp.H = c->A16[0]; sp.L = c->A16[1]; sp.status = c->dstatus;
        launch_split_a_f16(sp, c->stream);
        GradK128Args g{};
        g.Y = c->Y; g.ldY = c->ldY;
        g.Ah = c->A16[0]; g.Al = c->A16[1]; g.St = St;
        g.slabA = c->slab[0]; g.slabS = c->slab[1];
        g.lossPart = c->lossPart;
        g.status = c->dstatus;
        g.M = (int)c->Mk; g.N = (int)c->Nk;
        g.RP = c->plan.RP;
        g.doA = doA; g.doS = doS;
        g.gridX = c->plan.gridX; g.gridY = c->plan.gridY;
        g.absmax = c->absmax; g.ymax = c->ymax;
        g.W = c->W; g.ldW = c->ldW; g.wmax = c->wmax;
        g.wstatus = c->dstatus; g.rangeRatio = c->rangeRatio;
        if (c->chainL > 0 && (doA & 1)) {
            g.chainStride = 1;
            rc = chain_arm(c, g);
        }
        inst = k1_instance(c->k1, c->f16_r3, c->W != nullptr, grad, true);
        g.hh = inst == K1_HH;
        g.consPrio = k1_prio_for(128);
        if (rc == PMX_OK) rc = k1_timed(c, [&] { return grad_launch_k128(g, inst, c->stream); });
        break;
    }
    case K1_F16_K32: {
        GradV4Args g = v4_args(c, A, St, doA, doS);
        v4_f16_args(c, g, 32);
        g.fold = fold;
        inst = k1_instance(c->k1, c->f16_r3, false, grad, true);
        rc = k1_timed(c, [&] { return grad_launch_f16_k32(g, inst, c->stream); });
        break;
    }
    case K1_F16_V8:
    case K1_BF16_V7: {
        GradV4Args g = v4_args(c, A, St, doA, doS);
        g.prof = c->k1prof;
        g.W = c->W; g.ldW = c->ldW;
        if (c->k1 == K1_F16_V8) {
            v4_f16_args(c, g, 64);
            c->k1_pairs = (c->ldY % 2) == 0 && (((uintptr_t)c->Y) & 7) == 0 && (c->W == nullptr || (c->ldW == c->ldY && (((uintptr_t)c->W) & 7) == 0));
            inst = k1_instance(c->k1, c->f16_r3, c->W != nullptr, grad, c->k1_pairs);
            g.y16 = c->k1_pairs && (c->ldY % 4) == 0 && (((uintptr_t)c->Y) & 15) == 0;
        }
        if (c->chainL > 0) rc = chain_arm(c, g);
        const bool v8 = c->k1 == K1_F16_V8 && inst != K1_V7;
        if (rc == PMX_OK) rc = k1_timed(c, [&] { return v8 ? grad_launch_f16_v8(g, inst, c->stream) : grad_launch_bf16_v7(g, c->stream); });
        break;
    }
    case K1_BF16: {
        PresplitArgs ps{};
        ps.X[0] = A; ps.X[1] = St;
        for (int j = 0; j < 2; ++j) { ps.Xp[j] = c->Bp[j]; ps.Xt[j] = c->Bt[j]; ps.rows[j] = c->rowsK[j]; ps.rowsPad[j] = c->rowsPad[j]; }
        ps.K = (int)c->Kk; ps.KP = c->KP;
        ps.status = c->dstatus;
        launch_presplit(ps, c->stream);
        GradBfArgs g{};
        g.Y = c->Y; g.ldY = c->ldY;
        g.Ap = c->Bp[0]; g.At = c->Bt[0]; g.Sp = c->Bp[1]; g.Stt = c->Bt[1];
        g.MPad = c->rowsPad[0]; g.NPad = c->rowsPad[1];
        g.slabA = c->slab[0]; g.slabS = c->slab[1];
        g.lossPart = c->lossPart;
        g.status = c->dstatus;
        g.M = (int)c->Mk; g.N = (int)c->Nk; g.K = (int)c->Kk;
        g.RP = c->plan.RP;
        g.doA = doA; g.doS = doS;
        g.prof = c->k1prof;
        g.W = c->W; g.ldW = c->ldW;
        rc = k1_timed(c, [&] { return grad_launch_bf16(c->plan, g, c->stream); });
        break;
    }
    default: {
        GradArgs g = small_grad_args(c, A, St, doA, doS);
        if (c->k1 == K1_F32PC) {
            g.fold = fold;
            if (c->chainL > 0) rc = chain_arm(c, g);
        }
        if (rc == PMX_OK)
            rc = k1_timed(c, [&] { return k1_small(c->k1) ? grad_launch_small(c->plan, g, c->stream) : c->k1 == K1_F32PC ? grad_launch_f32pc(c->plan, g, c->stream) : grad_launch_f32(c->plan, g, c->stream); });
        break;
    }
    }
    if (rc != PMX_OK) return rc;
    if (grad) c->fix_on = inst == K1_HH;
    if (inst == K1_HH) return enqueue_gfix(c, A, St, doA, doS, c->stream);
    return PMX_OK;
}

static int enqueue_grad(pmx_ctx* c, const float* A, const float* St, int doA, int doS, bool absmax_fresh = false) {
    int rc = enqueue_grad_once(c, A, St, doA, doS, absmax_fresh);
    if (rc != PMX_OK || !c->k1_sync_check || !k1_fp16(c->k1) || c->host_grad || !(doA | doS)) return rc;
    rc = read_status(c);
    if (rc != PMX_OK) return rc;
    if (c->hstatus->k1_fault != 4) return PMX_OK;
    int again = 0;
    rc = chain_fault_fallback(c, &again);
    if (rc != PMX_OK) return rc;
    return enqueue_grad_once(c, A, St, doA, doS, false);
}

static SlabRef slab_ref(pmx_ctx* c, int j) {
    SlabRef s;
    s.stride = c->rowsK[j] * c->Kk;
    s.ld = (int)c->Kk;
    if (c->host_grad) {
        s.base = c->G[j];
        s.n = 1;
        s.ld = (int)c->K;
        return s;
    }
    s.base = c->slab[j];
    s.n = j == 0 ? c->nSlabA : c->nSlabS;
    if (c->fix_on) s.extra = c->fixSlab[j];
    return s;
}

static int bsdmm_flush_decide(pmx_ctx* c) {
    if (!c->bsd_decide_pending) return PMX_OK;
    launch_bsdmm_decide(c->bsd_decide, c->stream);
    HIP_CHECK(hipGetLastError());
    c->bsd_decide_pending = false;
    return PMX_OK;
}
static int enqueue_steps(pmx_ctx* c, const float* A, const float* St, bool wantStepA, bool wantStepS, double scale, bool have_partials = false, bool with_decide = false) {
    if (eig_small_applies(c)) {
        int frc = bsdmm_flush_decide(c);
        if (frc != PMX_OK) return frc;
        const EigArgs e = small_eig_args(c, A, St, wantStepA, wantStepS, scale);
        HIP_CHECK(launch_eig(e, c->stream));
        return PMX_OK;
    }
    GramArgs g{};
    g.X[0] = A; g.X[1] = St;
    g.rows[0] = c->M; g.rows[1] = c->N;
    g.K = (int)c->K;
    g.part = c->gramPart;
    g.status = c->dstatus;
    g.want[0] = wantStepS;
    g.want[1] = wantStepA;
    if (!have_partials) launch_gram(g, c->KP, c->stream);
    GramReduceArgs r{};
    r.part = c->gramPart; r.G = c->gramG; r.KP = c->KP; r.status = c->dstatus;
    r.want[0] = g.want[0]; r.want[1] = g.want[1];
    r.nparts[0] = gram_nparts(c->M); r.nparts[1] = gram_nparts(c->N);
    if (with_decide) {
        r.dec_partials = c->partials; r.dec_status = c->dstatus;
        r.dec_e_rel[0] = c->pgm.e_rel[0]; r.dec_e_rel[1] = c->pgm.e_rel[1];
    }
    if (c->bsd_decide_pending) {
        r.dec_bsdmm = c->bsd_decide;
        c->bsd_decide_pending = false;
    }
    launch_gram_reduce(r, c->stream);
    EigArgs e{};
    e.G = c->gramG; e.KP = c->KP; e.K = (int)c->K; e.status = c->dstatus;
    e.want[0] = g.want[0]; e.want[1] = g.want[1];
    e.scale = scale;
    e.max_iter = 200;
    e.Q = c->eigQ;
    HIP_CHECK(launch_eig(e, c->stream));
    return PMX_OK;
}

static int enqueue_gram_only(pmx_ctx* c, const float* A, const float* St, bool wantA_factor, bool wantS_factor) {
    GramArgs g{};
    g.X[0] = A; g.X[1] = St;
    g.rows[0] = c->M; g.rows[1] = c->N;
    g.K = (int)c->K;
    g.part = c->gramPart;
    g.status = c->dstatus;
    g.want[0] = wantA_factor; g.want[1] = wantS_factor;
    launch_gram(g, c->KP, c->stream);
    GramReduceArgs r{};
    r.part = c->gramPart; r.G = c->gramG; r.KP = c->KP; r.status = c->dstatus;
    r.want[0] = g.want[0]; r.want[1] = g.want[1];
    r.nparts[0] = gram_nparts(c->M); r.nparts[1] = gram_nparts(c->N);
    launch_gram_reduce(r, c->stream);
    HIP_CHECK(hipGetLastError());
    return PMX_OK;
}
static int enqueue_eig_only(pmx_ctx* c, bool wantA_factor, bool wantS_factor, double scale) {
    EigArgs e{};
    e.G = c->gramG; e.KP = c->KP; e.K = (int)c->K; e.status = c->dstatus;
    e.want[0] = wantA_factor; e.want[1] = wantS_factor;
    e.scale = scale;
    e.max_iter = 200;
    e.Q = c->eigQ;
    HIP_CHECK(launch_eig(e, c->stream));
    return PMX_OK;
}
static int shard_gram_in(pmx_ctx* c) {
    GramInArgs g{};
    g.comm_gram = c->ssplit ? c->comm_out + c->sncol * c->K : c->comm + c->N * c->K;
    g.G = c->gramG;
    g.n = c->KP * c->KP;
    g.status = c->dstatus;
    g.peer_halt = c->algo == ALG_BSDMM ? c->comm + c->N * c->K + (int64_t)c->KP * c->KP + MAXK + SHARD_HALT_SLOT : nullptr;
    g.wstatus = c->dstatus;
    launch_shard_gram_in(g, c->stream);
    HIP_CHECK(hipGetLastError());
    return PMX_OK;
}

static int require_ready(pmx_ctx* c, bool f64_ok = false) {
    if (!c) FAIL(PMX_E_INVALID, "ctx is NULL");
    if (c->f64 && !f64_ok) FAIL(PMX_E_UNSUPPORTED, "this entry point has no fp64 implementation (PMX_MODE_F64 covers the fused pgm / FISTA, adaprox and bsdmm loops on small problems)");
    if (!c->haveY) FAIL(PMX_E_STATE, "Y has not been set");
    HIP_CHECK(hipSetDevice(c->device));
    return PMX_OK;
}
static int begin_call(pmx_ctx* c, Algo algo, bool f64_ok, bool reset_flags = true) {
    if (c && reset_flags) { c->absmax_by_finish = false; c->gram_by_update = false; }
    int rc = require_ready(c, f64_ok);
    if (rc != PMX_OK) return rc;
    if (algo != ALG_NONE && c->algo != algo)
        FAIL(PMX_E_STATE, "pmx_%s_begin has not been called", algo == ALG_PGM ? "pgm" : algo == ALG_ADAPROX ? "adaprox" : "bsdmm");
    return PMX_OK;
}
static double next_omega64(pmx_ctx* c) {
    if (!c->pgm.accelerated) return 0.0;
    const double t = c->nest_t;
    const double t1 = 0.5 * (1.0 + sqrt(4.0 * t * t + 1.0));
    c->nest_t = t1;
    return (t - 1.0) / t1;
}
static float next_omega(pmx_ctx* c) { return (float)next_omega64(c); }
static void enqueue_pgm_decide(pmx_ctx* c, int check = 1) {
    DecideArgs d{};
    d.status = c->dstatus; d.partials = c->partials;
    d.e_rel[0] = c->pgm.e_rel[0]; d.e_rel[1] = c->pgm.e_rel[1];
    d.check = check;
    launch_pgm_decide(d, c->stream);
}

static void fill_result(pmx_ctx* c, pmx_result* r, int it_before) {
    if (!r) return;
    const DevStatus* s = c->hstatus;
    r->iterations = s->it_done - it_before;
    r->total_iterations = s->it_done;
    r->stopped = s->stopped;
    r->converged[0] = s->conv[0];
    r->converged[1] = s->conv[1];
    r->steps[0] = s->step[0];
    r->steps[1] = s->step[1];
    r->sub_iterations[0] = s->sub_total[0];
    r->sub_iterations[1] = s->sub_total[1];
}

static int enqueue_front64_big(pmx_ctx* c, const double* A, const double* St, int doA, int doS, bool tiles, bool steps, double scale) {
    if (tiles) {
        const bool loss_only = !doA && !doS;
        const double* X[2] = {A, St};
        if (c->Xk64[0] || c->Xk64[1]) {
            Pad64Args pa{};
            for (int j = 0; j < 2; ++j) { pa.X[j] = X[j]; pa.P[j] = c->Xk64[j]; pa.rows[j] = c->Xk64[j] ? c->rows[j] : 0; }
            pa.K = (int)c->K; pa.KP = c->KP; pa.status = c->dstatus;
            launch_pad64(pa, c->stream);
            for (int j = 0; j < 2; ++j) if (c->Xk64[j]) X[j] = c->Xk64[j];
        }
        for (int j = 1; j >= 0; --j) {
            const bool want = j ? (doS || loss_only) : (doA != 0);
            if (!want) continue;
            Pass64Args p{};
            p.Y = c->Yd; p.ldY = c->ldY64;
            p.Wt = c->Wd_on ? c->Wd : nullptr;
            p.F = X[j]; p.W = X[1 - j];
// ... 949 lines not shown
    if (p.backtracking && phase != 0) FAIL(PMX_E_UNSUPPORTED, "pmx_pgm_split: not with backtracking");
    if (c->pgm_long) FAIL(PMX_E_UNSUPPORTED, "pmx_pgm_split: prox_unity along the row dimension runs inside pmx_pgm_run only (a split iteration takes it as a user prox: host_prox)");
    const float* A = p.accelerated ? c->Xe[0] : c->X[0];
    const float* St = p.accelerated ? c->Xe[1] : c->X[1];
    const bool any_host = p.host_prox[0] || p.host_prox[1];
    auto update = [&](int stage) {
        PgmArgs u = pgm_args(c);
        for (int j = 0; j < 2; ++j) {
            u.slab[j] = single_slab(c->G[j], c->K);
            u.T[j] = c->Xp[j];
            u.stepArr[j] = (c->step_arr_mask >> j) & 1 ? c->stepArr[j] : nullptr;
            u.mode[j] = stage == 1 ? (p.host_prox[j] ? 1 : 3) : (p.host_prox[j] ? 2 : 0);
        }
        u.omega_next = stage == 2 ? next_omega(c) : 0.f;
        launch_pgm_update(u, c->stream);
    };
    switch (phase) {
        case 0: {
            { rc = one_iteration_per_call(c); if (rc != PMX_OK) return rc; }
            if (!p.use_fixed_steps && !p.bb_type) {
                rc = enqueue_steps(c, A, St, true, true, (double)p.step_scale);
                if (rc != PMX_OK) return rc;
            } else if (p.use_fixed_steps && !steps) {
                rc = set_fixed_steps(c, p.fixed_steps);
                if (rc != PMX_OK) return rc;
            }
            rc = enqueue_grad(c, A, St, 1, 1);
            if (rc != PMX_OK) return rc;
            c->bt_grad_fresh = p.backtracking != 0;
            if (p.bb_type) {
                enqueue_bb(c, A, St);
            } else {
                FoldArgs f{};
                for (int j = 0; j < 2; ++j) { f.slab[j] = slab_ref(c, j); f.G[j] = c->G[j]; f.rows[j] = c->rows[j]; }
                f.K = (int)c->K;
                f.status = c->dstatus;
                launch_fold(f, 2, c->stream);
            }
            HIP_CHECK(hipGetLastError());
            rc = read_status(c);
            if (rc != PMX_OK) return rc;
            if (res) { res->steps[0] = c->hstatus->step[0]; res->steps[1] = c->hstatus->step[1]; }
            return PMX_OK;
        }
        case 1:
            if (!any_host) return PMX_OK;
            if (steps) { rc = set_fixed_steps(c, steps); if (rc != PMX_OK) return rc; }
            update(1);
            HIP_CHECK(hipGetLastError());
            HIP_CHECK(hipStreamSynchronize(c->stream));
            return PMX_OK;
        case 2: {
            const int it0 = c->hstatus->it_done;
            if (steps) { rc = set_fixed_steps(c, steps); if (rc != PMX_OK) return rc; }
            update(2);
            enqueue_pgm_decide(c);
            HIP_CHECK(hipGetLastError());
            c->it += 1;
            rc = read_status(c);
            if (rc != PMX_OK) return rc;
            fill_result(c, res, it0);
            return PMX_OK;
        }
        default: FAIL(PMX_E_INVALID, "bad phase %d", phase);
    }
}

extern "C" int pmx_adaprox_begin(pmx_ctx* c, const pmx_adaprox_params* p, int warm_moments) {
    int rc = begin_call(c, ALG_NONE, true);
    if (rc != PMX_OK) return rc;
    if (!p) FAIL(PMX_E_INVALID, "params is NULL");
    if (p->scheme < PMX_ADAM || p->scheme > PMX_RADAM) FAIL(PMX_E_INVALID, "unknown scheme %d", p->scheme);
    if (!(p->b2 >= 0 && p->b2 < 1)) FAIL(PMX_E_INVALID, "b2 out of [0,1)");
    if (!(p->eps >= 0)) FAIL(PMX_E_INVALID, "eps < 0");
    if (!(p->p > 0 && p->p <= 0.5)) FAIL(PMX_E_INVALID, "p out of (0,0.5]");
    for (int j = 0; j < 2; ++j) {
        rc = check_prox(p->prox[j], j ? "prox_S" : "prox_A", false, c->tab_set);
        if (rc != PMX_OK) return rc;
    }
    if (c->f64) {
        if (p->host_prox[0] || p->host_prox[1] || p->use_fixed_steps == 2)
            FAIL(PMX_E_UNSUPPORTED, "fp64 contexts run adaprox with this library's operators and step rule (no user prox / step)");
        c->ada = *p;
        c->algo = ALG_ADAPROX;
        c->it = 0;
        rc = reset_status(c);
        if (rc != PMX_OK) return rc;
        for (int j = 0; j < 2; ++j) {
            const size_t n = (size_t)c->rows[j] * c->K;
            const bool fresh_m = c->Md[j] == nullptr, fresh_v = c->Vd[j] == nullptr;
            rc = dallocT(c, &c->Md[j], n);
            if (rc == PMX_OK) rc = dallocT(c, &c->Vd[j], n);
            if (rc != PMX_OK) return rc;
            if (!warm_moments) {
                if (!fresh_m) HIP_CHECK(hipMemsetAsync(c->Md[j], 0, n * sizeof(double), c->stream));
                if (!fresh_v) HIP_CHECK(hipMemsetAsync(c->Vd[j], 0, n * sizeof(double), c->stream));
            }
            if (p->warm_vhat && !c->Vhd[j]) FAIL(PMX_E_STATE, "warm_vhat set but Vhat buffers were not uploaded");
            if (p->check_convergence) rc = dallocT(c, &c->Xpd[j], n, false);
            if (rc == PMX_OK && p->prox[j].n > 0) {
                rc = dallocT(c, &c->Psid[j], n, false);
                if (rc == PMX_OK) rc = dallocT(c, &c->zd[j], n, false);
            }
            if (rc != PMX_OK) return rc;
        }
        rc = dallocT(c, &c->alpha64, c->f64big ? 2 * MAXK : 32);
        if (rc == PMX_OK && c->f64big) rc = dallocT(c, &c->colpart64, (size_t)2 * EW_BLOCKS * MAXK);
        if (rc != PMX_OK) return rc;
        c->nsub64 = 4;
        HIP_CHECK(hipStreamSynchronize(c->stream));
        return PMX_OK;
    }
    c->ada = *p;
    c->algo = ALG_ADAPROX;
    c->it = 0;
    c->nsub_guess = 2;
    c->sub_nt = (getenv("PMX_SUB_BATCH") && atoi(getenv("PMX_SUB_BATCH")) == 1) ? 1 : SUB_NT_MAX;
    for (auto& r : c->sub_rec) r = pmx_ctx::SubRec{};
    rc = reset_status(c);
    if (rc != PMX_OK) return rc;
    for (int j = 0; j < 2; ++j) {
        const size_t n = (size_t)c->rows[j] * c->K;
        const bool fresh_m = c->Mm[j] == nullptr, fresh_v = c->Vv[j] == nullptr;
        rc = dallocT(c, &c->Mm[j], n);
        if (rc == PMX_OK) rc = dallocT(c, &c->Vv[j], n);
        if (rc != PMX_OK) return rc;
        if (!warm_moments) {
            if (!fresh_m) HIP_CHECK(hipMemsetAsync(c->Mm[j], 0, n * sizeof(float), c->stream));
            if (!fresh_v) HIP_CHECK(hipMemsetAsync(c->Vv[j], 0, n * sizeof(float), c->stream));
        }
        if (p->warm_vhat && !c->Vh[j]) FAIL(PMX_E_STATE, "warm_vhat set but Vhat buffers were not uploaded");
        if (p->check_convergence) {
            rc = dallocT(c, &c->Xp[j], n, false);
            if (rc != PMX_OK) return rc;
        }
        if (p->prox[j].n > 0 || p->host_prox[j]) {
            rc = dallocT(c, &c->Psi[j], n, false);
            if (rc == PMX_OK) rc = dallocT(c, &c->zb[j][0], n, false);
            if (rc == PMX_OK) rc = dallocT(c, &c->zb[j][1], n, false);
            if (rc != PMX_OK) return rc;
        }
    }
    c->tail_fused = false;
    if (!(getenv("PMX_TAIL_FUSED") && atoi(getenv("PMX_TAIL_FUSED")) == 0) && c->sub_nt != 1 && c->tailFaults == 0 &&
        !p->host_prox[0] && !p->host_prox[1] &&
        !prox_has_max_entropy(p->prox[0]) && !prox_has_max_entropy(p->prox[1])) {
        int ncu = 0;
        if (hipDeviceGetAttribute(&ncu, hipDeviceAttributeMultiprocessorCount, c->device) != hipSuccess) ncu = 0;
        TailArgs probe{};
        probe.m.K = (int)c->K;
        for (int j = 0; j < 2; ++j) probe.slots[j] = (int)((c->rows[j] + 8191) / 8192);
        if (ncu >= EW_BLOCKS && ada_tail_lds_bytes(probe) <= ADA_TAIL_LDS_MAX) {
            rc = dallocT(c, &c->gridbar, 1);
            if (rc == PMX_OK && getenv("PMX_TAIL_PROF")) rc = dallocT(c, &c->tailprof, 16);
            if (rc != PMX_OK) return rc;
            c->tail_fused = true;
        }
    }
    AlphaArgs al = alpha_args(c);
    al.use_fixed = p->use_fixed_steps;
    al.fixed[0] = (float)p->fixed_alpha[0];
    al.fixed[1] = (float)p->fixed_alpha[1];
    rc = enqueue_alpha_from_factors(c, al);
    if (rc != PMX_OK) return rc;
    HIP_CHECK(hipStreamSynchronize(c->stream));
    return PMX_OK;
}

static SubArgs sub_args(pmx_ctx* c, int t) {
    const pmx_adaprox_params& p = c->ada;
    SubArgs s{};
    for (int j = 0; j < 2; ++j) {
        s.X[j] = s_view(c, j, c->X[j]);
        s.Psi[j] = s_view(c, j, c->Psi[j]);
        s.zb[j][0] = s_view(c, j, c->zb[j][0]);
        s.zb[j][1] = s_view(c, j, c->zb[j][1]);
        s.rows[j] = upd_rows(c, j);
        s.prox[j] = to_dev(p.prox[j], c->tabs);
        s.e_rel[j] = p.e_rel[j];
        s.has_prox[j] = p.prox[j].n > 0;
    }
    s.K = (int)c->K;
    s.status = c->dstatus;
    s.partials = c->partials;
    s.t = t;
    s.nt = c->sub_nt;
    s.prox_max_iter = p.prox_max_iter;
    return s;
}

static int ada_enqueue_subs(pmx_ctx* c, int t0, int n) {
    const int nt = c->sub_nt;
    int t = t0;
    for (; t < t0 + n; t += nt) launch_ada_sub(sub_args(c, t), c->stream);
    return t;
}

static int ada_enqueue_tail(pmx_ctx* c, int t) {
    const pmx_adaprox_params& p = c->ada;
    FinishArgs f{};
    f.s = sub_args(c, t);
    f.Xp[0] = c->Xp[0]; f.Xp[1] = s_view(c, 1, c->Xp[1]);
    f.colpart = c->colpart;
    f.check_convergence = p.check_convergence;
    static_assert(EW_BLOCKS == 256, "k_grad_f16_v8 folds 256 partial maxima per factor");
    f.absmax_out = k1_fp16(c->k1) ? c->absmax : nullptr;
    launch_ada_finish(f, c->stream);
    AdaDecideArgs d{};
    d.al = alpha_args(c);
    d.al.use_fixed = p.use_fixed_steps;
    d.al.fixed[0] = (float)p.fixed_alpha[0];
    d.al.fixed[1] = (float)p.fixed_alpha[1];
    d.partials = c->partials;
    d.e_rel[0] = p.e_rel[0]; d.e_rel[1] = p.e_rel[1];
    d.check_convergence = c->comm ? 0 : p.check_convergence;
    d.has_prox[0] = p.prox[0].n > 0; d.has_prox[1] = p.prox[1].n > 0;
    d.host_tau[0] = c->host_tau[0]; d.host_tau[1] = c->host_tau[1];
    launch_ada_decide(d, c->stream);
    HIP_CHECK(hipGetLastError());
    return PMX_OK;
}

static MomentArgs moment_args(pmx_ctx* c, int it, double b1t, double b1prev, bool for_tail) {
    const pmx_adaprox_params& p = c->ada;
    MomentArgs m{};
    for (int j = 0; j < 2; ++j) {
        m.X[j] = s_view(c, j, c->X[j]); m.Xp[j] = s_view(c, j, c->Xp[j]);
        m.Mm[j] = s_view(c, j, c->Mm[j]); m.Vv[j] = s_view(c, j, c->Vv[j]);
        m.Vh[j] = p.warm_vhat ? s_view(c, j, c->Vh[j]) : nullptr;
        m.Psi[j] = for_tail ? nullptr : s_view(c, j, c->Psi[j]);
        m.slab[j] = slab_ref(c, j);
        m.rows[j] = upd_rows(c, j);
        m.has_prox[j] = p.prox[j].n > 0 || (!for_tail && p.host_prox[j]);
    }
    if (c->shard_grad_from_comm) m.slab[1] = comm_slab(c);
    m.K = (int)c->K;
    m.status = c->dstatus;
    m.partials = c->partials;
    m.scheme = p.scheme;
    m.it = it;
    m.b1t = b1t; m.b1prev = b1prev; m.b2 = p.b2; m.eps = p.eps; m.p = p.p;
    m.check_convergence = p.check_convergence;
    return m;
}
static int ada_enqueue_moment(pmx_ctx* c, int it, double b1t, double b1prev) {
    launch_ada_moment(moment_args(c, it, b1t, b1prev, false), c->stream);
    HIP_CHECK(hipGetLastError());
    return PMX_OK;
}

static int ada_enqueue_tail_fused(pmx_ctx* c, int it, double b1t, double b1prev) {
    const pmx_adaprox_params& p = c->ada;
    TailArgs t{};
    t.m = moment_args(c, it, b1t, b1prev, true);
    for (int j = 0; j < 2; ++j) {
        t.prox[j] = to_dev(p.prox[j], c->tabs);
        t.e_rel[j] = p.e_rel[j];
        t.slots[j] = (int)((upd_rows(c, j) + 8191) / 8192);
    }
    t.prox_max_iter = p.prox_max_iter;
    t.colpart = c->colpart;
    t.absmax_out = k1_fp16(c->k1) ? c->absmax : nullptr;
    t.al = alpha_args(c);
    t.al.use_fixed = p.use_fixed_steps;
    t.al.fixed[0] = (float)p.fixed_alpha[0];
    t.al.fixed[1] = (float)p.fixed_alpha[1];
    t.decide_check = c->comm ? 0 : 1;
    t.bar = c->gridbar;
    t.prof = c->tailprof;
    t.prof_fine = getenv("PMX_TAIL_PROF") && atoi(getenv("PMX_TAIL_PROF")) == 2;
    const char* lockfile = c->hook_tail_lockfile.empty() ? nullptr : c->hook_tail_lockfile.c_str();
    int lockfd = -1;
    if (lockfile) {
        lockfd = open(lockfile, O_CREAT | O_RDWR, 0600);
        if (lockfd < 0) FAIL(PMX_E_STATE, "PMX_TAIL_LOCKFILE: cannot open %s", lockfile);
        HIP_CHECK(hipStreamSynchronize(c->stream));
        if (flock(lockfd, LOCK_EX) != 0) { close(lockfd); FAIL(PMX_E_STATE, "PMX_TAIL_LOCKFILE: flock failed"); }
    }
    hipError_t le = launch_ada_tail(t, c->stream);
    if (lockfd >= 0) {
        hipError_t se = hipStreamSynchronize(c->stream);
        flock(lockfd, LOCK_UN);
        close(lockfd);
        HIP_CHECK(se);
    }
    HIP_CHECK(le);
    return PMX_OK;
}

static int ada_enqueue_head(pmx_ctx* c, int it, double b1t, double b1prev, bool after_tail) {
    int rc = enqueue_grad(c, c->X[0], c->X[1], 1, 1, after_tail);
    if (rc != PMX_OK) return rc;
    return ada_enqueue_moment(c, it, b1t, b1prev);
}

static int ada_pick_sub_batch(pmx_ctx* c, int wanted) {
    const pmx_adaprox_params& p = c->ada;
    const bool any_prox = p.prox[0].n > 0 || p.prox[1].n > 0;
    const int nsub = any_prox ? std::max(1, std::min(wanted, p.prox_max_iter)) : 0;
    if (c->sub_nt != 1) c->sub_nt = nsub <= 4 ? 4 : SUB_NT_MAX;
    return nsub;
}
static int ada_feed_more_subs(pmx_ctx* c, int* t_enq) {
    int rc = clear_halt(c);
    if (rc != PMX_OK) return rc;
    *t_enq = ada_enqueue_subs(c, *t_enq, std::min(std::max(4, *t_enq), 64));
    return ada_enqueue_tail(c, *t_enq);
}

static Ada64Args ada64_args(pmx_ctx* c, int it, double b1t, double b1prev) {
    const pmx_adaprox_params& p = c->ada;
    Ada64Args a{};
    for (int j = 0; j < 2; ++j) {
        a.X[j] = c->Xd[j]; a.Xp[j] = c->Xpd[j]; a.Mm[j] = c->Md[j]; a.Vv[j] = c->Vd[j];
        a.Vh[j] = p.warm_vhat ? c->Vhd[j] : nullptr;
        a.Psi[j] = c->Psid[j]; a.z[j] = c->zd[j];
        a.slab[j] = c->slabd[j];
        a.nslab[j] = j == 0 ? c->nSlabA : c->nSlabS;
        a.rows[j] = c->rows[j];
        a.prox[j] = to_dev(p.prox[j], c->tabs);
        a.has_prox[j] = p.prox[j].n > 0;
        a.e_rel[j] = p.e_rel[j];
        a.fixed[j] = p.fixed_alpha[j];
    }
    a.K = (int)c->K;
    a.status = c->dstatus;
    a.scheme = p.scheme;
    a.it = it;
    a.b1t = b1t; a.b1prev = b1prev;
    a.b2 = p.b2; a.eps = p.eps; a.p = p.p;
    a.check_convergence = p.check_convergence;
    a.prox_max_iter = p.prox_max_iter;
    a.use_fixed = p.use_fixed_steps;
    a.alpha_out = c->alpha64;
    return a;
}

extern "C" int pmx_adaprox_run(pmx_ctx* c, int n_iter, const double* b1, double b1_prev, pmx_result* res) {
    int rc = begin_call(c, ALG_ADAPROX, true);
    if (rc != PMX_OK) return rc;
    if (n_iter < 0 || (n_iter > 0 && !b1)) FAIL(PMX_E_INVALID, "bad n_iter / b1");
    for (int i = 0; i < n_iter; ++i)
        if (!(b1[i] >= 0 && b1[i] < 1)) FAIL(PMX_E_INVALID, "b1 out of [0,1)");
    const pmx_adaprox_params& p = c->ada;
    const bool any_prox = p.prox[0].n > 0 || p.prox[1].n > 0;
    const int it0 = c->hstatus->it_done;
    if (c->f64big) {
        auto args_of = [&](int gi) {
            Ada64bArgs b{};
            b.a = ada64_args(c, it0 + gi, b1[gi], gi == 0 ? b1_prev : b1[gi - 1]);
            b.partials = c->partials;
            b.colpart = c->colpart64;
            return b;
        };
        int gi = 0;
        while (gi < n_iter && !c->hstatus->stopped) {
            const int chunk = std::min(n_iter - gi, 16);
            const int nsub = any_prox ? std::max(1, std::min(c->nsub64, p.prox_max_iter)) : 0;
            for (int i = 0; i < chunk; ++i) {
                rc = enqueue_front64(c, c->Xd[0], c->Xd[1], 1, 1, true, false, 1.0);
                if (rc != PMX_OK) return rc;
                Ada64bArgs b = args_of(gi + i);
                launch_ada64b_head(b, c->stream);
                for (int t = 1; t <= nsub; ++t) { b.t = t; launch_ada64b_sub(b, c->stream); }
                b.t = nsub;
                launch_ada64b_close(b, c->stream);
                HIP_CHECK(hipGetLastError());
            }
            rc = read_status(c);
            if (rc != PMX_OK) return rc;
            if (c->hstatus->halt && c->hstatus->reason == HALT_ERROR) FAIL(PMX_E_HIP, "%s", chain_error_text(c));
            int done = c->hstatus->it_done - it0;
            int passes = nsub;
            while (c->hstatus->halt && c->hstatus->reason == HALT_NEED_SUB) {
                const int more = std::min(p.prox_max_iter - passes, std::max(passes, 4));
                if (more <= 0) FAIL(PMX_E_STATE, "adaprox (fp64): the proximal loop asks for passes beyond prox_max_iter");
                HIP_CHECK(hipMemsetAsync(&c->dstatus->halt, 0, 2 * sizeof(int), c->stream));
                Ada64bArgs b = args_of(done);
                for (int t = passes + 1; t <= passes + more; ++t) { b.t = t; launch_ada64b_sub(b, c->stream); }
                passes += more;
                b.t = passes;
                launch_ada64b_close(b, c->stream);
                HIP_CHECK(hipGetLastError());
                rc = read_status(c);
                if (rc != PMX_OK) return rc;
                if (c->hstatus->halt && c->hstatus->reason == HALT_ERROR) FAIL(PMX_E_HIP, "%s", chain_error_text(c));
                done = c->hstatus->it_done - it0;
            }
            if (any_prox) c->nsub64 = std::max(c->hstatus->last_tau[0], c->hstatus->last_tau[1]) + 2;
            gi = done;
        }
        fill_result(c, res, it0);
        return PMX_OK;
    }
    if (c->f64) {
        for (int left = n_iter, gi = 0; left > 0 && !c->hstatus->stopped; left -= 16) {
            for (int i = 0; i < std::min(left, 16); ++i, ++gi) {
                rc = enqueue_front64(c, c->Xd[0], c->Xd[1], 1, 1, true, false, 1.0);
                if (rc != PMX_OK) return rc;
                launch_ada64_iter(ada64_args(c, it0 + gi, b1[gi], gi == 0 ? b1_prev : b1[gi - 1]), c->stream);
                HIP_CHECK(hipGetLastError());
            }
            rc = read_status(c);
            if (rc != PMX_OK) return rc;
            if (c->hstatus->halt && c->hstatus->reason == HALT_ERROR) FAIL(PMX_E_HIP, "%s", chain_error_text(c));
        }
        fill_result(c, res, it0);
        return PMX_OK;
    }
    int done = 0;
    int tails = 0;
    while (done < n_iter && !c->hstatus->stopped) {
        const int chunk = std::min(n_iter - done, c->tail_fused ? 64 : 16);
        const int nsub = ada_pick_sub_batch(c, c->nsub_guess);
        for (int i = 0; i < chunk; ++i) {
            const int gi = done + i;
            if (c->tail_fused) {
                rc = enqueue_grad(c, c->X[0], c->X[1], 1, 1, tails > 0);
                if (rc == PMX_OK) rc = ada_enqueue_tail_fused(c, it0 + gi, b1[gi], gi == 0 ? b1_prev : b1[gi - 1]);
                ++tails;
                if (rc != PMX_OK) return rc;
                continue;
            }
            rc = ada_enqueue_head(c, it0 + gi, b1[gi], gi == 0 ? b1_prev : b1[gi - 1], tails > 0);
            if (rc != PMX_OK) return rc;
            rc = ada_enqueue_tail(c, ada_enqueue_subs(c, 0, nsub));
            ++tails;
            if (rc != PMX_OK) return rc;
        }
        rc = read_status(c);
        if (rc != PMX_OK) return rc;
        const int nsub_enq = nsub > 0 ? ((nsub + c->sub_nt - 1) / c->sub_nt) * c->sub_nt : 0;
        int t_enq = nsub_enq;
        while (c->hstatus->halt && c->hstatus->reason == HALT_NEED_SUB) {
            rc = ada_feed_more_subs(c, &t_enq);
            if (rc != PMX_OK) return rc;
            const int finished_if_ok = c->hstatus->it_done - it0 + 1;
            for (int gi = finished_if_ok; gi < done + chunk; ++gi) {
                rc = ada_enqueue_head(c, it0 + gi, b1[gi], gi == 0 ? b1_prev : b1[gi - 1], true);
                if (rc != PMX_OK) return rc;
                rc = ada_enqueue_tail(c, ada_enqueue_subs(c, 0, nsub));
                if (rc != PMX_OK) return rc;
            }
            const int it_before = c->hstatus->it_done;
            rc = read_status(c);
            if (rc != PMX_OK) return rc;
            if (c->hstatus->it_done > it_before) t_enq = nsub_enq;
        }
        done = c->hstatus->it_done - it0;
        {
            int again = 0;
            rc = chain_fault_fallback(c, &again);
            if (rc != PMX_OK) return rc;
            if (again) { tails = 0; continue; }
        }
        if (any_prox) c->nsub_guess = std::max(2, std::max(c->hstatus->last_tau[0], c->hstatus->last_tau[1]));
        if (c->hstatus->halt && c->hstatus->reason == HALT_ERROR) FAIL(PMX_E_HIP, "%s", chain_error_text(c));
    }
    if (c->tailprof && c->tail_fused) {
        long long h[16];
        HIP_CHECK(hipMemcpy(h, c->tailprof, sizeof(h), hipMemcpyDeviceToHost));
        static const char* nm[] = {"census", "moment", "B1", "maxpsi", "sub", "B2", "judge+replay", "finish", "B3", "decide"};
        static const char* nf[] = {"census", "moment", "B1", "maxpsi", "passesA", "sumsA", "passesS", "sumsS", "(end)", "B2", "judge+replay", "finish", "B3", "decide"};
        const bool fine = getenv("PMX_TAIL_PROF") && atoi(getenv("PMX_TAIL_PROF")) == 2;
        const int np = fine ? 14 : 10;
        fprintf(stderr, "[tailprof] us:");
        for (int i = 0; i < np; ++i) fprintf(stderr, " %s=%.2f", fine ? nf[i] : nm[i], (double)(h[i + 1] - h[i]) / 100.0);
        fprintf(stderr, " total=%.2f\n", (double)(h[np] - h[0]) / 100.0);
    }
    fill_result(c, res, it0);
    return PMX_OK;
}

extern "C" int pmx_adaprox_set_alpha(pmx_ctx* c, const float* alpha) {
    REJECT_F64(c);
    if (!c || !alpha) FAIL(PMX_E_INVALID, "NULL argument");
    if (c->algo != ALG_ADAPROX || c->ada.use_fixed_steps != 2) FAIL(PMX_E_STATE, "pmx_adaprox_begin with use_fixed_steps = 2 has not been called");
    HIP_CHECK(hipSetDevice(c->device));
    HIP_CHECK(hipMemcpyAsync(&c->dstatus->alpha[0][0], alpha, sizeof(float) * c->K, hipMemcpyHostToDevice, c->stream));
    HIP_CHECK(hipMemcpyAsync(&c->dstatus->alpha[1][0], alpha + c->K, sizeof(float) * c->K, hipMemcpyHostToDevice, c->stream));
    HIP_CHECK(hipStreamSynchronize(c->stream));
    return PMX_OK;
}

extern "C" int pmx_adaprox_split(pmx_ctx* c, int phase, int it, double b1_it, double b1_prev, const int* host_tau, double* maxpsi, pmx_result* res) {
    int rc = begin_call(c, ALG_ADAPROX, false);
    if (rc != PMX_OK) return rc;
    if (c->tail_fused) FAIL(PMX_E_STATE, "pmx_adaprox_split needs a context begun with host_prox");
    if (!(b1_it >= 0 && b1_it < 1)) FAIL(PMX_E_INVALID, "b1 out of [0,1)");
    const pmx_adaprox_params& p = c->ada;
    if (phase == 0) {
        { rc = one_iteration_per_call(c); if (rc != PMX_OK) return rc; }
        rc = ada_enqueue_head(c, it, b1_it, b1_prev, false);
        if (rc != PMX_OK) return rc;
        rc = read_status(c);
        if (rc != PMX_OK) return rc;
        if (maxpsi) {
            std::vector<double> h(2 * EW_BLOCKS);
            HIP_CHECK(hipMemcpy(h.data(), c->partials + (size_t)SL_MAXPSI * 2 * EW_BLOCKS, sizeof(double) * 2 * EW_BLOCKS, hipMemcpyDeviceToHost));
            for (int j = 0; j < 2; ++j) {
                double m = -1.0;
                for (int b = 0; b < EW_BLOCKS; ++b) { const double v = h[j * EW_BLOCKS + b]; m = (m != m || v != v) ? NAN : std::max(m, v); }
                maxpsi[j] = m;
            }
        }
        return PMX_OK;
    }
    if (phase != 1) FAIL(PMX_E_INVALID, "bad phase %d", phase);
    c->host_tau[0] = host_tau ? host_tau[0] : 0;
    c->host_tau[1] = host_tau ? host_tau[1] : 0;
    const bool any_prox = p.prox[0].n > 0 || p.prox[1].n > 0;
    const int it0 = c->hstatus->it_done;
    int t_enq = ada_enqueue_subs(c, 0, ada_pick_sub_batch(c, c->nsub_guess));
    rc = ada_enqueue_tail(c, t_enq);
    if (rc != PMX_OK) return rc;
    rc = read_status(c);
    if (rc != PMX_OK) return rc;
    while (c->hstatus->halt && c->hstatus->reason == HALT_NEED_SUB) {
        rc = ada_feed_more_subs(c, &t_enq);
        if (rc != PMX_OK) return rc;
        rc = read_status(c);
        if (rc != PMX_OK) return rc;
    }
    if (any_prox) c->nsub_guess = std::max(2, std::max(c->hstatus->last_tau[0], c->hstatus->last_tau[1]));
    c->host_tau[0] = c->host_tau[1] = 0;
    if (c->hstatus->halt && c->hstatus->reason == HALT_ERROR) FAIL(PMX_E_HIP, "%s", chain_error_text(c));
    fill_result(c, res, it0);
    return PMX_OK;
}

extern "C" int pmx_bsdmm_begin(pmx_ctx* c, const pmx_bsdmm_params* p) {
    int rc = begin_call(c, ALG_NONE, true);
    if (rc != PMX_OK) return rc;
    if (!p) FAIL(PMX_E_INVALID, "params is NULL");
    if (c->W || c->Wd_on)
        FAIL(PMX_E_INVALID, "The truth value of an array with more than one element is ambiguous. Use a.any() or a.all()");
    for (int j = 0; j < 2; ++j) {
        rc = check_prox(p->prox_f[j], j ? "prox_S" : "prox_A", false, c->tab_set);
        if (rc != PMX_OK) return rc;
        if (p->n_g[j] < 0 || p->n_g[j] > PMX_MAX_G) FAIL(PMX_E_UNSUPPORTED, "at most %d constraints per block", PMX_MAX_G);
        for (int i = 0; i < p->n_g[j]; ++i) {
            rc = check_prox(p->prox_g[j][i], "proxs_g", false, c->tab_set);
            if (rc != PMX_OK) return rc;
        }
    }
    if (p->n_order < 0 || p->n_order > 8) FAIL(PMX_E_INVALID, "update_order: at most 8 entries");
    for (int i = 0; i < p->n_order; ++i)
        if (p->order[i] != 0 && p->order[i] != 1) FAIL(PMX_E_INVALID, "update_order: block %d out of range", p->order[i]);
    c->bsd = *p;
    c->algo = ALG_BSDMM;
    c->it = 0;
    rc = reset_status(c);
    if (rc != PMX_OK) return rc;
    if (c->f64) {
        for (int j = 0; j < 2; ++j) {
            const size_t n = (size_t)c->rows[j] * c->K;
            for (int i = 0; i < p->n_g[j]; ++i) {
                rc = dallocT(c, &c->Zd[j][i], n, false);
                if (rc == PMX_OK) rc = dallocT(c, &c->Ud[j][i], n, false);
                if (rc != PMX_OK) return rc;
                HIP_CHECK(hipMemcpyAsync(c->Zd[j][i], c->Xd[j], n * sizeof(double), hipMemcpyDeviceToDevice, c->stream));
                HIP_CHECK(hipMemsetAsync(c->Ud[j][i], 0, n * sizeof(double), c->stream));
            }
        }
        HIP_CHECK(hipStreamSynchronize(c->stream));
        return PMX_OK;
    }
    for (int j = 0; j < 2; ++j) {
        const size_t n = (size_t)c->rows[j] * c->K;
        for (int i = 0; i < p->n_g[j]; ++i) {
            rc = dallocT(c, &c->Zg[j][i], n, false);
            if (rc == PMX_OK) rc = dallocT(c, &c->Ug[j][i], n, false);
            if (rc != PMX_OK) return rc;
            HIP_CHECK(hipMemcpyAsync(c->Zg[j][i], c->X[j], n * sizeof(float), hipMemcpyDeviceToDevice, c->stream));
            HIP_CHECK(hipMemsetAsync(c->Ug[j][i], 0, n * sizeof(float), c->stream));
        }
    }
    HIP_CHECK(hipStreamSynchronize(c->stream));
    return PMX_OK;
}

static BsdmmArgs bsdmm_args(pmx_ctx* c, int j) {
    const pmx_bsdmm_params& p = c->bsd;
    BsdmmArgs u{};
    u.X = c->X[j];
    u.slab = slab_ref(c, j);
    for (int i = 0; i < p.n_g[j]; ++i) { u.Z[i] = c->Zg[j][i]; u.U[i] = c->Ug[j][i]; u.prox_g[i] = to_dev(p.prox_g[j][i], c->tabs); }
    u.rows = c->rows[j];
    u.K = (int)c->K;
    u.j = j;
    u.n_g = p.n_g[j];
    u.prox_f = to_dev(p.prox_f[j], c->tabs);
    u.status = c->dstatus;
    u.partials = c->partials;
    return u;
}
static Bsdmm64Args bsdmm64_args(pmx_ctx* c, int j, int last_block) {
    const pmx_bsdmm_params& p = c->bsd;
    Bsdmm64Args u{};
    u.X = c->Xd[j];
    u.slab = c->slabd[j];
    u.nslab = j == 0 ? c->nSlabA : c->nSlabS;
    for (int i = 0; i < p.n_g[j]; ++i) { u.Z[i] = c->Zd[j][i]; u.U[i] = c->Ud[j][i]; u.prox_g[i] = to_dev(p.prox_g[j][i], c->tabs); }
    u.rows = c->rows[j];
    u.K = (int)c->K;
    u.j = j;
    u.n_g = p.n_g[j];
    u.prox_f = to_dev(p.prox_f[j], c->tabs);
    u.status = c->dstatus;
    u.e_rel = p.e_rel[j];
    u.e_abs = p.e_abs[j];
    u.last_block = last_block;
    return u;
}
static BsdmmDecideArgs bsdmm_decide_args(pmx_ctx* c, int j, int64_t size, int last_block) {
    const pmx_bsdmm_params& p = c->bsd;
    BsdmmDecideArgs d{};
    d.status = c->dstatus;
    d.partials = c->partials;
    d.j = j;
// ... 621 lines not shown
```

### proxmin_amd/engine.py

```python
from __future__ import annotations

import ctypes as C
import logging
import os

import numpy as np

from . import _lib

logger = logging.getLogger("proxmin")
_noticed = set()


def _notice(key, msg):
    if key not in _noticed:
        _noticed.add(key)
        logger.info(msg)


LIBRARY_DEFAULT_MODE = "f16x2r"
_DEFAULT_MODE = os.environ.get("PMX_MODE", LIBRARY_DEFAULT_MODE)
assert _DEFAULT_MODE in ("f32", "bf16x3", "f16x2", "f16x2r"), "PMX_MODE must be one of f32, bf16x3, f16x2, f16x2r"


# ... 208 lines not shown
        return self

    def __exit__(self, *exc):
        self.close()

    def sync(self):
        _lib.check(self.lib.pmx_ctx_sync(self.h))

    def set_Y(self, Y):
        ref = as_device_array(Y)
        if ref is not None:
            assert ref.shape == (self.M, self.N), "Y must be M x N"
            if ref.dtype == np.float64:
                if not self.f64:
                    raise NotImplementedError("a float64 device-resident Y is taken by the fp64 kernels only (library operators and step rules, K <= 128); "
                                              "this call computes in float32: hand it a float32 array")
                _lib.check(self.lib.pmx_set_Y_device_f64(self.h, C.c_void_p(int(ref.ptr)), int(ref.ld)))
                return
            if self.f64:
                raise NotImplementedError("an fp64 context takes a float64 Y")
            self.set_Y_device(ref.ptr, ld=ref.ld, copy=False, keepalive=ref.owner)
            return
        Y = np.asarray(Y)
        assert Y.shape == (self.M, self.N), "Y must be M x N"
        if self.f64:
            Yd = np.ascontiguousarray(Y, dtype=np.float64)
            _lib.check(self.lib.pmx_set_Y_host_f64(self.h, _vp(Yd), self.N))
            return
        Yf = _f32(Y)
        _lib.check(self.lib.pmx_set_Y_host(self.h, _vp(Yf), self.N))

    def set_Y_device(self, dptr, ld=None, copy=False, keepalive=None):
        if keepalive is not None:
            self._keep.append(keepalive)
        _lib.check(self.lib.pmx_set_Y_device(self.h, C.c_void_p(int(dptr)), int(ld or self.N), int(bool(copy))))
        if not copy and not self.f64:
            fr = self.k1_info()["frame"]
            if tuple(fr) != (self.M, self.N):
                _notice(("frame-copy", self.M, self.N, self.K),
                        "proxmin_amd: %d x %d x %d runs on the zero-padded frame %d x %d of its tuned kernel: the device array handed over with copy=False is "
                        "COPIED into a frame-sized buffer (%.2f GiB more device memory; PMX_FRAME=0 keeps the caller's array and the guarded kernels)"
                        % (self.M, self.N, self.K, fr[0], fr[1], fr[0] * fr[1] * 4 / 2.0 ** 30))

    def set_W(self, W):
        if W is None:
            _lib.check((self.lib.pmx_set_W_host_f64 if self.f64 else self.lib.pmx_set_W_host)(self.h, None, 0))
            return
        W = np.asarray(W)
        assert W.shape == (self.M, self.N), "W must be M x N"
        if self.f64:
            Wd = np.ascontiguousarray(W, dtype=np.float64)
            _lib.check(self.lib.pmx_set_W_host_f64(self.h, _vp(Wd), self.N))
            return
        Wf = _f32(W)
        _lib.check(self.lib.pmx_set_W_host(self.h, _vp(Wf), self.N))

    def set_W_device(self, dptr, ld=None, copy=False, keepalive=None):
        if keepalive is not None:
            self._keep.append(keepalive)
        _lib.check(self.lib.pmx_set_W_device(self.h, C.c_void_p(int(dptr)), int(ld or self.N), int(bool(copy))))

    def _upload(self, buf, arr2d):
        if self.f64:
            a = np.ascontiguousarray(arr2d, dtype=np.float64)
            _lib.check(self.lib.pmx_upload_f64(self.h, buf, _vp(a), a.size))
            return
        a = _f32(arr2d)
        _lib.check(self.lib.pmx_upload(self.h, buf, _vp(a), a.size))

    def _download(self, buf, rows):
        if self.f64:
            out = np.empty((rows, self.K), dtype=np.float64)
            _lib.check(self.lib.pmx_download_f64(self.h, buf, _vp(out), out.size))
            return out
        out = np.empty((rows, self.K), dtype=np.float32)
        _lib.check(self.lib.pmx_download(self.h, buf, _vp(out), out.size))
        return out

    def _check_ref(self, ref, j):
        want = (self.M, self.K) if j == 0 else (self.K, self.N)
        assert ref.shape == want, "A must be M x K and S K x N"
        if ref.device != self.device:
            raise ValueError("the array lives on GPU %d, this context on GPU %d" % (ref.device, self.device))
        if (ref.dtype == np.float64) != self.f64:
            raise NotImplementedError(_F64_FACTORS_IN_F32 if not self.f64 else "an fp64 context takes float64 device-resident factors")

    def _from_device(self, buf, ref, j=None):
        self._check_ref(ref, buf & 1 if j is None else j)
        old = self._kept_for.get(buf)
        if old is not None:
            self._keep[:] = [o for o in self._keep if o is not old]
        self._kept_for[buf] = ref.owner
        self._keep.append(ref.owner)
        _lib.check(self.lib.pmx_factor_from_device(self.h, buf, C.c_void_p(ref.ptr), ref.strides[0], ref.strides[1], int(self.f64)))

    def _to_device(self, buf, ref, j=None):
        self._check_ref(ref, buf & 1 if j is None else j)
        _lib.check(self.lib.pmx_factor_to_device(self.h, buf, C.c_void_p(ref.ptr), ref.strides[0], ref.strides[1], int(self.f64)))

    def set_factors(self, A, S):
        if isinstance(A, DeviceFactorRef) or isinstance(S, DeviceFactorRef):
            A, S = factor_pair(A, S)
            self._check_ref(A, 0)
            self._check_ref(S, 1)
            self._from_device(_lib.BUF_A, A)
            self._from_device(_lib.BUF_ST, S)
            return
        assert A.shape == (self.M, self.K) and S.shape == (self.K, self.N), "A must be M x K and S K x N"
        self._upload(_lib.BUF_A, A)
        self._upload(_lib.BUF_ST, np.asarray(S).T)

    def get_factors(self):
        return self._download(_lib.BUF_A, self.M), self._download(_lib.BUF_ST, self.N).T

    def write_factors(self, A, S):
        self._check_ref(A, 0)
        self._check_ref(S, 1)
        self._to_device(_lib.BUF_A, A)
        self._to_device(_lib.BUF_ST, S)

    def put(self, base, j, arr):
        if isinstance(arr, DeviceFactorRef):
            self._from_device(base + j, arr, j)
            return
        self._upload(base + j, arr if j == 0 else np.asarray(arr).T)

    def get(self, base, j):
        out = self._download(base + j, self.M if j == 0 else self.N)
        return out if j == 0 else out.T

    def set_timing(self, on=True, every=1):
        _lib.check(self.lib.pmx_set_timing(self.h, int(every) if on else 0))

    def get_timing(self):
        ms, n = C.c_double(), C.c_int()
        _lib.check(self.lib.pmx_get_timing(self.h, C.byref(ms), C.byref(n)))
        return ms.value, n.value

    PHASES = ("k1_with_prologue", "pack", "collective", "post", "update", "after_update_to_next_k1")

    def set_phase_timing(self, every=4):
        _lib.check(self.lib.pmx_set_phase_timing(self.h, int(every)))

    def get_phase_timing(self):
        ms, n = (C.c_double * 6)(), C.c_int()
        _lib.check(self.lib.pmx_get_phase_timing(self.h, ms, C.byref(n)))
        return {k: ms[i] for i, k in enumerate(self.PHASES)}, n.value

    def time_grad(self, do_A=True, do_S=True, reps=10):
        ms = C.c_double()
        _lib.check(self.lib.pmx_time_grad(self.h, int(do_A), int(do_S), int(reps), C.byref(ms)))
        return ms.value

    def k1_info(self):
        v = (C.c_int * 8)()
        _lib.check(self.lib.pmx_k1_info(self.h, v))
        keys = ("kernel", "chain", "slabs_A", "slabs_S", "row_regions", "col_regions", "panels_per_region", "chain_faults")
        d = dict(zip(keys, list(v)))
        d["kernel"] = ("k_grad_f32", "k_grad_bf16", "k_grad_f16_v8", "k_grad_f16_v9", "k_grad_small", "k_grad_f16_k128", "k_grad_f32_pc", "k64_front", "k_grad_f16_k32", "k_grad_f16_v8_r3", "k_grad_f16_k32_r3", "k_grad_f16_v8_hh", "k_grad_f16_k128_hh", "k64_grad_pass")[d["kernel"]]
        v7 = d.pop("chain_faults")
        d["chain_faults"], d["tail_faults"], d["tail_fused"] = v7 % 1000, (v7 // 1000) % 1000, bool((v7 // 1000000) % 10)
        d["range_faults"] = v7 // 10000000
        fr = (C.c_int64 * 3)()
        _lib.check(self.lib.pmx_k1_frame(self.h, fr))
        d["frame"] = (fr[0], fr[1])
        d["frame_K"] = fr[2]
        return d

    def grad(self):
        _lib.check(self.lib.pmx_grad(self.h))
        return self._download(_lib.BUF_GA, self.M), self._download(_lib.BUF_GST, self.N).T

    def loglike(self):
        out = C.c_double()
        _lib.check(self.lib.pmx_loglike(self.h, C.byref(out)))
        return out.value

    def step_pgm(self):
        out = (C.c_double * 2)()
        _lib.check(self.lib.pmx_step_pgm(self.h, out))
        return out[0], out[1]

    def step_adaprox(self):
        out = np.empty(2 * self.K, dtype=np.float32)
        _lib.check(self.lib.pmx_step_adaprox(self.h, _vp(out)))
        return out[: self.K].copy(), out[self.K:].copy()

    def _stamp_tables(self, seqs, first=0):
        from . import operators
        operators.check_tables(seqs, self.K)
        if first + sum(len(operators.seq_tables(q)) for q in seqs) > _lib.MAX_TABLES:
            raise NotImplementedError("more than %d per-component operator tables in one call" % _lib.MAX_TABLES)
        out, nxt = [], first
        for q in seqs:
            tables = operators.seq_tables(q)
            if not tables:
                out.append(q)
                continue
            c = _lib.ProxSeq.from_buffer_copy(q)
            for i in range(c.n):
                if c.seq[i].op == _lib.PROX["components"]:
                    tab = tables[c.seq[i].reserved - 1]
                    _lib.check(self.lib.pmx_prox_table(self.h, nxt, tab, len(tab)))
                    c.seq[i].reserved = nxt + 1
                    nxt += 1
            out.append(c)
        self._ntab = nxt
        return out

    def prox_apply(self, buf, seq, step_k):
        seq, = self._stamp_tables([seq], first=getattr(self, "_ntab_solver", 0))
        sk = np.ascontiguousarray(np.broadcast_to(np.asarray(step_k, dtype=np.float32).reshape(-1), (self.K,)))
        _lib.check(self.lib.pmx_prox_apply(self.h, int(buf), C.byref(seq), _vp(sk)))

    def pgm_begin(self, prox, accelerated=False, step_scale=1.0, fixed_steps=None, e_rel=(1e-6, 1e-6), bb=None, backtracking=False,
                  host_prox=(False, False), unweighted_rule=False):
        p = _lib.PgmParams()
        p.prox[0], p.prox[1] = self._stamp_tables(list(prox))
        self._ntab_solver = self._ntab
        p.accelerated = int(bool(accelerated))
        p.step_scale = float(step_scale)
        p.use_fixed_steps = int(fixed_steps is not None)
        p.unweighted_rule = int(bool(unweighted_rule))
        if fixed_steps is not None:
            p.fixed_steps[0], p.fixed_steps[1] = float(fixed_steps[0]), float(fixed_steps[1])
        p.e_rel[0], p.e_rel[1] = float(e_rel[0]), float(e_rel[1])
        if bb is not None:
            p.bb_type, p.bb_init_r = int(bb[0]), float(bb[1])
        p.backtracking = int(bool(backtracking))
        p.host_prox[0], p.host_prox[1] = int(bool(host_prox[0])), int(bool(host_prox[1]))
        _lib.check(self.lib.pmx_pgm_begin(self.h, C.byref(p)))

    def pgm_split(self, phase, steps=None):
        r = _lib.Result()
        st = (C.c_double * 2)(float(steps[0]), float(steps[1])) if steps is not None else None
        _lib.check(self.lib.pmx_pgm_split(self.h, int(phase), st, C.byref(r)))
        return r

    def pgm_bt_split(self, phase):
        r = _lib.Result()
        need, eff = C.c_int(), (C.c_double * 2)()
        _lib.check(self.lib.pmx_pgm_bt_split(self.h, int(phase), C.byref(need), eff, C.byref(r)))
        return need.value, (eff[0], eff[1]), r

    def pgm_set_fixed_steps(self, steps):
        _lib.check(self.lib.pmx_pgm_set_fixed_steps(self.h, (C.c_double * 2)(float(steps[0]), float(steps[1]))))

    def pgm_step_arrays(self, arrays):
        mask = 0
        for j, a in enumerate(arrays):
            if a is None:
                continue
            shape = (self.M, self.K) if j == 0 else (self.K, self.N)
            self.put(_lib.BUF_STEP_A, j, np.broadcast_to(np.asarray(a, dtype=np.float32), shape))
            mask |= 1 << j
        _lib.check(self.lib.pmx_pgm_step_arrays(self.h, mask))

    def pgm_run(self, n_iter):
        r = _lib.Result()
        _lib.check(self.lib.pmx_pgm_run(self.h, int(n_iter), C.byref(r)))
        return r

    def adaprox_begin(self, prox, scheme="adam", b2=0.999, eps=1e-8, p=0.25, check_convergence=True,
                      prox_max_iter=1000, warm_moments=False, warm_vhat=False, fixed_alpha=None, e_rel=(1e-6, 1e-6),
                      host_step=False, host_prox=(False, False)):
        q = _lib.AdaproxParams()
        q.prox[0], q.prox[1] = self._stamp_tables(list(prox))
        self._ntab_solver = self._ntab
        q.scheme = _lib.SCHEME[scheme]
        q.b2, q.eps, q.p = float(b2), float(eps), float(p)
        q.check_convergence = int(bool(check_convergence))
        q.prox_max_iter = int(prox_max_iter)
        q.warm_vhat = int(bool(warm_vhat))
        q.use_fixed_steps = 2 if host_step else int(fixed_alpha is not None)
        q.host_prox[0], q.host_prox[1] = int(bool(host_prox[0])), int(bool(host_prox[1]))
        if fixed_alpha is not None:
            q.fixed_alpha[0], q.fixed_alpha[1] = float(fixed_alpha[0]), float(fixed_alpha[1])
        q.e_rel[0], q.e_rel[1] = float(e_rel[0]), float(e_rel[1])
        _lib.check(self.lib.pmx_adaprox_begin(self.h, C.byref(q), int(bool(warm_moments))))

    def adaprox_run(self, b1_slice, b1_prev):
        b1 = np.ascontiguousarray(b1_slice, dtype=np.float64)
        r = _lib.Result()
        _lib.check(self.lib.pmx_adaprox_run(self.h, int(b1.size), b1.ctypes.data_as(C.POINTER(C.c_double)),
                                            float(b1_prev), C.byref(r)))
        return r

    def adaprox_set_alpha(self, alpha_A, alpha_S):
        a = np.ascontiguousarray(np.concatenate([np.asarray(alpha_A, np.float32).ravel(), np.asarray(alpha_S, np.float32).ravel()]))
        assert a.size == 2 * self.K
        _lib.check(self.lib.pmx_adaprox_set_alpha(self.h, _vp(a)))

    def adaprox_split(self, phase, it, b1_it, b1_prev, host_tau=(0, 0)):
        r = _lib.Result()
        tau = (C.c_int * 2)(int(host_tau[0]), int(host_tau[1]))
        mp = (C.c_double * 2)()
        _lib.check(self.lib.pmx_adaprox_split(self.h, int(phase), int(it), float(b1_it), float(b1_prev), tau, mp, C.byref(r)))
        return r, (mp[0], mp[1])

    def bsdmm_begin(self, prox_f, proxs_g, e_rel=(1e-6, 1e-6), e_abs=(0.0, 0.0), update_order=None):
        p = _lib.BsdmmParams()
        if update_order is not None:
            order = [int(j) for j in update_order]
            if len(order) > 8:
                raise NotImplementedError("update_order with more than 8 entries")
            p.n_order = len(order)
# ... 48 lines not shown
```

Baseline: 2853.

## Add optional gfix gram fusion into tail kernel and restructure K=64 gram partials

Restructures the K=64 correction-gram kernel so each block processes interleaved 32-row groups across 256 partitions with two-slot prefetch, and widens the partial reduction accordingly. Adds an opt-in path (env PMX_GFIX_IN_TAIL, default off) that computes the gram, reduce and apply stages inside the fused adaprox tail kernel using grid barriers, skipping separate gfix launches. Helpers are factored out for reuse by the tail. More partials increase reduction traffic, and the fused path adds LDS and barrier pressure in the tail.

```diff
diff --git a/proxmin_amd/csrc/k_gfix.hip b/proxmin_amd/csrc/k_gfix.hip
--- a/proxmin_amd/csrc/k_gfix.hip
+++ b/proxmin_amd/csrc/k_gfix.hip
@@ -1,6 +1,8 @@
 #include "pmx_common.h"
 
-constexpr int GFIX_PARTS = 128;
+constexpr int GFIX_PARTS = 256;
+constexpr int GFIX_GROUP = 32;
+constexpr int GFIX_SPAN = GFIX_GROUP * GFIX_PARTS;
 
 struct GfixArgs {
     const float* X[2];
@@ -19,9 +21,10 @@
 
 typedef _Float16 gf16x8 __attribute__((ext_vector_type(8)));
 
-__device__ __forceinline__ float gfix_scale(const float* absmax, int f, float* red) {
-    float m = 0.f;
-    for (int i = threadIdx.x; i < 256; i += blockDim.x) m = fmaxf(m, absmax[f * 256 + i]);
+template <bool SC1> __device__ __forceinline__ float gfix_ld(const float* p) { return SC1 ? __hip_atomic_load(p, __ATOMIC_RELAXED, __HIP_MEMORY_SCOPE_AGENT) : *p; }
+template <bool SC1> __device__ __forceinline__ void gfix_st(float* p, float v) { if (SC1) __hip_atomic_store(p, v, __ATOMIC_RELAXED, __HIP_MEMORY_SCOPE_AGENT); else *p = v; }
+
+__device__ __forceinline__ float gfix_scale_of(float m, float* red) {
 #pragma unroll
     for (int o = 32; o > 0; o >>= 1) m = fmaxf(m, __shfl_xor(m, o));
     if ((threadIdx.x & 63) == 0) red[threadIdx.x >> 6] = m;
@@ -32,71 +35,53 @@
     (void)frexpf(mx, &q);
     return ldexpf(1.f, mx > 0.f ? 14 - q : 0);
 }
-
-template <int KT, int W>
-__device__ __forceinline__ void gfix_gram_wave(const GfixArgs& a, int f, float* red) {
-    constexpr int K = 32 * KT, TPW = KT * KT / 4, NB = KT == 2 ? 8 : 4;
+__device__ __forceinline__ float gfix_scale(const float* absmax, int f, float* red) {
+    float m = 0.f;
+    for (int i = threadIdx.x; i < 256; i += blockDim.x) m = fmaxf(m, absmax[f * 256 + i]);
+    return gfix_scale_of(m, red);
+}
+
+template <int W, bool AHEAD, bool SC1, class Scale, class Fetch>
+__device__ __forceinline__ void gfix_gram_job(int nslot, Scale scale, Fetch fetch, float* out) {
+    constexpr int K = 64, KT = 2, ti = W / KT, tj = W % KT;
     const int lane = threadIdx.x & 63, l31 = lane & 31, hi = lane >> 5;
-    const int64_t rows = a.rows[f];
-    const int64_t per = 16 * ((rows + 16 * GFIX_PARTS - 1) / (16 * GFIX_PARTS));
-    const int64_t r0 = (int64_t)blockIdx.x * per, r1 = r0 + per < rows ? r0 + per : rows;
-    const float* X = a.X[f] + 32 * 0 + l31;
-    f32x16 acc0[TPW], accr[TPW];
-#pragma unroll
-    for (int t = 0; t < TPW; ++t)
-#pragma unroll
-        for (int i = 0; i < 16; ++i) { acc0[t][i] = 0.f; accr[t][i] = 0.f; }
-    float v[NB][KT][8];
-#define GFIX_REQUEST(rb_)                                                                          \
-    _Pragma("unroll") for (int s = 0; s < NB; ++s)                                                 \
-    _Pragma("unroll") for (int q = 0; q < 8; ++q) {                                                \
-        const int64_t r = (rb_) + 16 * s + 8 * hi + q;                                             \
-        _Pragma("unroll") for (int c = 0; c < KT; ++c) v[s][c][q] = r < r1 ? X[r * K + 32 * c] : 0.f; \
-    }
-    GFIX_STAMP(0);
-    if (r0 < r1) { GFIX_REQUEST(r0) }
-    const float sc = gfix_scale(a.absmax, f, red), un = 1.f / (sc * sc);
-    GFIX_STAMP(1);
-    for (int64_t rb = r0; rb < r1; rb += 16 * NB) {
-        gf16x8 h[NB][KT], l[NB][KT];
-#pragma unroll
-        for (int s = 0; s < NB; ++s)
+    f32x16 acc0, accr;
+#pragma unroll
+    for (int i = 0; i < 16; ++i) { acc0[i] = 0.f; accr[i] = 0.f; }
+    float v[2][KT][8];
+#define GFIX_REQUEST(i_, s_)                                                                        \
+    _Pragma("unroll") for (int q = 0; q < 8; ++q)                                                   \
+    _Pragma("unroll") for (int c = 0; c < KT; ++c) v[s_][c][q] = fetch((i_), 16 * (s_) + 8 * hi + q, 32 * c + l31);
+    if (AHEAD && nslot > 0) { GFIX_REQUEST(0, 0) GFIX_REQUEST(0, 1) }
+    const float sc = scale(), un = 1.f / (sc * sc);
+    for (int i = 0; i < nslot; ++i) {
+#pragma unroll
+        for (int s = 0; s < 2; ++s) {
+            if (!AHEAD) { GFIX_REQUEST(i, s) }
+            gf16x8 h[KT], l[KT];
 #pragma unroll
             for (int c = 0; c < KT; ++c)
 #pragma unroll
                 for (int q = 0; q < 8; ++q) {
                     const float x = v[s][c][q] * sc;
                     const _Float16 t = (_Float16)x;
-                    h[s][c][q] = t;
-                    l[s][c][q] = (_Float16)(x - (float)t);
+                    h[c][q] = t;
+                    l[c][q] = (_Float16)(x - (float)t);
                 }
-        if (rb + 16 * NB < r1) { GFIX_REQUEST(rb + 16 * NB) }
-#pragma unroll
-        for (int s = 0; s < NB; ++s)
-#pragma unroll
-            for (int t = 0; t < TPW; ++t) {
-                constexpr int idx0 = W * TPW;
-                const int ti = (idx0 + t) / KT, tj = (idx0 + t) % KT;
-                acc0[t] = __builtin_amdgcn_mfma_f32_32x32x16_f16(h[s][ti], l[s][tj], acc0[t], 0, 0, 0);
-                accr[t] = __builtin_amdgcn_mfma_f32_32x32x16_f16(l[s][ti], l[s][tj], accr[t], 0, 0, 0);
-                acc0[t] = __builtin_amdgcn_mfma_f32_32x32x16_f16(h[s][ti], h[s][tj], acc0[t], 0, 0, 0);
-                accr[t] = __builtin_amdgcn_mfma_f32_32x32x16_f16(l[s][ti], h[s][tj], accr[t], 0, 0, 0);
-            }
+            if (AHEAD && s == 1 && i + 1 < nslot) { GFIX_REQUEST(i + 1, 0) GFIX_REQUEST(i + 1, 1) }
+            acc0 = __builtin_amdgcn_mfma_f32_32x32x16_f16(h[ti], l[tj], acc0, 0, 0, 0);
+            accr = __builtin_amdgcn_mfma_f32_32x32x16_f16(l[ti], l[tj], accr, 0, 0, 0);
+            acc0 = __builtin_amdgcn_mfma_f32_32x32x16_f16(h[ti], h[tj], acc0, 0, 0, 0);
+            accr = __builtin_amdgcn_mfma_f32_32x32x16_f16(l[ti], h[tj], accr, 0, 0, 0);
+        }
     }
 #undef GFIX_REQUEST
-    GFIX_STAMP(2);
-    float* out = a.part + ((int64_t)f * GFIX_PARTS + blockIdx.x) * 2 * K * K;
-#pragma unroll
-    for (int t = 0; t < TPW; ++t) {
-        const int ti = (W * TPW + t) / KT, tj = (W * TPW + t) % KT;
-#pragma unroll
-        for (int i = 0; i < 16; ++i) {
-            const int kp = 32 * ti + (i & 3) + 8 * (i >> 2) + 4 * hi, k = 32 * tj + l31;
-            out[kp * K + k] = acc0[t][i] * un;
-            out[K * K + kp * K + k] = accr[t][i] * un;
-        }
-    }
-    GFIX_STAMP(3);
+#pragma unroll
+    for (int i = 0; i < 16; ++i) {
+        const int kp = 32 * ti + (i & 3) + 8 * (i >> 2) + 4 * hi, k = 32 * tj + l31;
+        gfix_st<SC1>(out + kp * K + k, acc0[i] * un);
+        gfix_st<SC1>(out + K * K + kp * K + k, accr[i] * un);
+    }
 }
 template <int W>
 __device__ __forceinline__ void gfix_gram_wave_k128(const GfixArgs& a, int f, float* red, gf16x8* frag) {
@@ -174,13 +159,45 @@
         else if (w == 2) gfix_gram_wave_k128<2>(a, f, red, gfrag);
         else gfix_gram_wave_k128<3>(a, f, red, gfrag);
     } else {
-        if (w == 0) gfix_gram_wave<KT, 0>(a, f, red);
-        else if (w == 1) gfix_gram_wave<KT, 1>(a, f, red);
-        else if (w == 2) gfix_gram_wave<KT, 2>(a, f, red);
-        else gfix_gram_wave<KT, 3>(a, f, red);
-    }
-}
-
+        const int64_t rows = a.rows[f];
+        const float* X = a.X[f];
+        const int nslot = (int)((rows + GFIX_SPAN - 1) / GFIX_SPAN);
+        auto fetch = [&](int i, int rr, int k) {
+            const int64_t r = (int64_t)GFIX_GROUP * blockIdx.x + (int64_t)GFIX_SPAN * i + rr;
+            return r < rows ? X[r * 64 + k] : 0.f;
+        };
+        auto scale = [&]() { return gfix_scale(a.absmax, f, red); };
+        float* out = a.part + ((int64_t)f * GFIX_PARTS + blockIdx.x) * 2 * 64 * 64;
+        GFIX_STAMP(0);
+        if (w == 0) gfix_gram_job<0, true, false>(nslot, scale, fetch, out);
+        else if (w == 1) gfix_gram_job<1, true, false>(nslot, scale, fetch, out);
+        else if (w == 2) gfix_gram_job<2, true, false>(nslot, scale, fetch, out);
+        else gfix_gram_job<3, true, false>(nslot, scale, fetch, out);
+        GFIX_STAMP(1); GFIX_STAMP(2); GFIX_STAMP(3);
+    }
+}
+
+template <bool SC1, int NB>
+__device__ __forceinline__ void gfix_reduce_entry(const float* part, float* Q, int n, int f, int e, int q, bool live) {
+    static_assert(GFIX_PARTS == 256 && 64 % NB == 0, "four threads x 64 partials");
+    double s = 0.0;
+    if (live) {
+        const float* p = part + (int64_t)f * GFIX_PARTS * n + (int64_t)(q * 64) * n + e;
+#pragma unroll
+        for (int b = 0; b < 64; b += NB) {
+            float v[NB];
+#pragma unroll
+            for (int i = 0; i < NB; ++i) v[i] = gfix_ld<SC1>(p + (int64_t)(b + i) * n);
+#pragma unroll
+            for (int i = 0; i < NB; ++i) s += (double)v[i];
+        }
+    }
+    const int base = threadIdx.x & 60;
+    double tot = __shfl(s, base);
+#pragma unroll
+    for (int i = 1; i < 4; ++i) tot += __shfl(s, base + i);
+    if (live && q == 0) gfix_st<SC1>(Q + (int64_t)f * n + e, (float)tot);
+}
 __global__ __launch_bounds__(256) void k_gfix_reduce(GfixArgs a) {
     if (chain_halted(a.status)) return;
     const int f = blockIdx.y;
@@ -188,27 +205,105 @@
     GFIX_STAMP(4);
     const int n = 2 * a.K * a.K;
     const int t = blockIdx.x * 256 + threadIdx.x, e = t >> 2, q = t & 3;
-    static_assert(GFIX_PARTS == 128, "four threads x 32 partials");
-    double s = 0.0;
-    if (e < n) {
-        const float* p = a.part + (int64_t)f * GFIX_PARTS * n + (int64_t)(q * 32) * n + e;
-        float v[32];
-#pragma unroll
-        for (int i = 0; i < 32; ++i) v[i] = p[(int64_t)i * n];
-#pragma unroll
-        for (int i = 0; i < 32; ++i) s += (double)v[i];
-    }
-    const int base = threadIdx.x & 60;
-    double tot = __shfl(s, base);
-#pragma unroll
-    for (int i = 1; i < 4; ++i) tot += __shfl(s, base + i);
-    if (e < n && q == 0) a.Q[(int64_t)f * n + e] = (float)tot;
+    gfix_reduce_entry<false, 64>(a.part, a.Q, n, f, e, q, e < n);
     GFIX_STAMP(5);
 }
 
+template <int KT, int NT, bool SC1>
+__device__ __forceinline__ void gfix_q_fetch(const float* src, int t, float (&tq)[2][32 * KT / 8 / (NT / (32 * KT))][8], float* redq) {
+    constexpr int K = 32 * KT, TPK = NT / K, NBLK = K / 8 / TPK, NW = NT / 64;
+    const int kcol = t % K, kb0 = t / K;
+#pragma unroll
+    for (int m = 0; m < 2; ++m)
+#pragma unroll
+        for (int i = 0; i < NBLK; ++i)
+#pragma unroll
+            for (int e = 0; e < 8; ++e) tq[m][i][e] = gfix_ld<SC1>(src + (size_t)m * K * K + (size_t)(8 * (kb0 + TPK * i) + e) * K + kcol);
+    float mx[2] = {0.f, 0.f};
+#pragma unroll
+    for (int m = 0; m < 2; ++m)
+#pragma unroll
+        for (int i = 0; i < NBLK; ++i)
+#pragma unroll
+            for (int e = 0; e < 8; ++e) mx[m] = fmaxf(mx[m], fabsf(tq[m][i][e]));
+#pragma unroll
+    for (int o = 32; o > 0; o >>= 1) { mx[0] = fmaxf(mx[0], __shfl_xor(mx[0], o)); mx[1] = fmaxf(mx[1], __shfl_xor(mx[1], o)); }
+    if ((t & 63) == 0) { redq[0 * NW + (t >> 6)] = mx[0]; redq[1 * NW + (t >> 6)] = mx[1]; }
+}
+template <int NW>
+__device__ __forceinline__ void gfix_q_scales(const float* redq, float (&sq)[2]) {
+#pragma unroll
+    for (int m = 0; m < 2; ++m) {
+        float v = redq[m * NW];
+#pragma unroll
+        for (int i = 1; i < NW; ++i) v = fmaxf(v, redq[m * NW + i]);
+        int q = 0;
+        (void)frexpf(v, &q);
+        sq[m] = ldexpf(1.f, v > 0.f ? 14 - q : 0);
+    }
+}
+template <int KT, int NT>
+__device__ __forceinline__ void gfix_q_planes(const float (&tq)[2][32 * KT / 8 / (NT / (32 * KT))][8], int t, const float (&sq)[2], _Float16* qpl) {
+    constexpr int K = 32 * KT, LDQ = K + 8, TPK = NT / K, NBLK = K / 8 / TPK;
+    const int kcol = t % K, kb0 = t / K;
+#pragma unroll
+    for (int m = 0; m < 2; ++m) {
+        _Float16* ph = qpl + (size_t)((1 - m) * 2) * K * LDQ + (size_t)kcol * LDQ;
+        _Float16* pl = ph + (size_t)K * LDQ;
+#pragma unroll
+        for (int i = 0; i < NBLK; ++i) {
+            gf16x8 h8, l8;
+#pragma unroll
+            for (int e = 0; e < 8; ++e) {
+                const float v = tq[m][i][e] * sq[m];
+                const _Float16 h = (_Float16)v;
+                h8[e] = h;
+                l8[e] = (_Float16)(v - (float)h);
+            }
+            *reinterpret_cast<gf16x8*>(ph + 8 * (kb0 + TPK * i)) = h8;
+            *reinterpret_cast<gf16x8*>(pl + 8 * (kb0 + TPK * i)) = l8;
+        }
+    }
+}
+template <int KT, class XRow>
+__device__ __forceinline__ void gfix_apply_task(XRow xrow, const _Float16* qpl, int c, float sc, const float (&sq)[2], float (&cv)[16]) {
+    constexpr int K = 32 * KT, LDQ = K + 8;
+    const int lane = threadIdx.x & 63, l31 = lane & 31, hi = lane >> 5;
+    f32x16 acc1, acc2;
+#pragma unroll
+    for (int i = 0; i < 16; ++i) { acc1[i] = 0.f; acc2[i] = 0.f; }
+    const _Float16* qb = qpl + (size_t)(32 * c + l31) * LDQ + 8 * hi;
+#pragma unroll
+    for (int ks = 0; ks < K / 16; ++ks) {
+        float xv[8];
+        xrow(ks, xv);
+        gf16x8 xh, xl, xm;
+#pragma unroll
+        for (int e = 0; e < 8; ++e) {
+            const float v = xv[e] * sc;
+            const _Float16 h = (_Float16)v;
+            const float r1 = v - (float)h;
+            const _Float16 l = (_Float16)r1;
+            xh[e] = h; xl[e] = l; xm[e] = (_Float16)(r1 - (float)l);
+        }
+        const gf16x8 qrh = *reinterpret_cast<const gf16x8*>(qb + 16 * ks);
+        const gf16x8 qrl = *reinterpret_cast<const gf16x8*>(qb + (size_t)K * LDQ + 16 * ks);
+        const gf16x8 q0h = *reinterpret_cast<const gf16x8*>(qb + (size_t)2 * K * LDQ + 16 * ks);
+        const gf16x8 q0l = *reinterpret_cast<const gf16x8*>(qb + (size_t)3 * K * LDQ + 16 * ks);
+        acc1 = __builtin_amdgcn_mfma_f32_32x32x16_f16(xl, qrh, acc1, 0, 0, 0);
+        acc2 = __builtin_amdgcn_mfma_f32_32x32x16_f16(xm, q0h, acc2, 0, 0, 0);
+        acc1 = __builtin_amdgcn_mfma_f32_32x32x16_f16(xh, qrl, acc1, 0, 0, 0);
+        acc2 = __builtin_amdgcn_mfma_f32_32x32x16_f16(xl, q0l, acc2, 0, 0, 0);
+        acc1 = __builtin_amdgcn_mfma_f32_32x32x16_f16(xh, qrh, acc1, 0, 0, 0);
+        acc2 = __builtin_amdgcn_mfma_f32_32x32x16_f16(xl, q0h, acc2, 0, 0, 0);
+    }
+    const float u1 = 1.f / (sc * sq[1]), u2 = 1.f / (sc * sq[0]);
+#pragma unroll
+    for (int i = 0; i < 16; ++i) cv[i] = acc1[i] * u1 + acc2[i] * u2;
+}
 template <int KT>
 __global__ __launch_bounds__(KT == 4 ? 512 : 256) void k_gfix_apply(GfixArgs a) {
-    constexpr int K = 32 * KT, LDQ = K + 8;
+    constexpr int K = 32 * KT;
     constexpr int NT = KT == 4 ? 512 : 256, NW = NT / 64;
     extern __shared__ _Float16 qpl[];
     __shared__ float red[8];
@@ -231,59 +326,14 @@
     }
     const int64_t task0 = (int64_t)blockIdx.x * NW + w;
     if (task0 < ntask) GFIX_LOAD_X(task0)
-    constexpr int TPK = NT / K, NBLK = K / 8 / TPK;
-    const int kcol = tid % K, kb0 = tid / K;
-    float tq[2][NBLK][8];
-    {
-        const float* src = a.Q + (int64_t)(1 - f) * 2 * K * K;
-#pragma unroll
-        for (int m = 0; m < 2; ++m)
-#pragma unroll
-            for (int i = 0; i < NBLK; ++i)
-#pragma unroll
-                for (int e = 0; e < 8; ++e) tq[m][i][e] = src[(size_t)m * K * K + (size_t)(8 * (kb0 + TPK * i) + e) * K + kcol];
-    }
-    float mx[2] = {0.f, 0.f};
-#pragma unroll
-    for (int m = 0; m < 2; ++m)
-#pragma unroll
-        for (int i = 0; i < NBLK; ++i)
-#pragma unroll
-            for (int e = 0; e < 8; ++e) mx[m] = fmaxf(mx[m], fabsf(tq[m][i][e]));
-#pragma unroll
-    for (int o = 32; o > 0; o >>= 1) { mx[0] = fmaxf(mx[0], __shfl_xor(mx[0], o)); mx[1] = fmaxf(mx[1], __shfl_xor(mx[1], o)); }
-    __shared__ float redq[2][NW];
-    if (lane == 0) { redq[0][w] = mx[0]; redq[1][w] = mx[1]; }
+    float tq[2][K / 8 / (NT / K)][8];
+    __shared__ float redq[2 * NW];
+    gfix_q_fetch<KT, NT, false>(a.Q + (int64_t)(1 - f) * 2 * K * K, tid, tq, redq);
     const float sc = gfix_scale(a.absmax, f, red);
     GFIX_STAMP(7);
     float sq[2];
-#pragma unroll
-    for (int m = 0; m < 2; ++m) {
-        float v = redq[m][0];
-#pragma unroll
-        for (int i = 1; i < NW; ++i) v = fmaxf(v, redq[m][i]);
-        int q = 0;
-        (void)frexpf(v, &q);
-        sq[m] = ldexpf(1.f, v > 0.f ? 14 - q : 0);
-    }
-#pragma unroll
-    for (int m = 0; m < 2; ++m) {
-        _Float16* ph = qpl + (size_t)((1 - m) * 2) * K * LDQ + (size_t)kcol * LDQ;
-        _Float16* pl = ph + (size_t)K * LDQ;
-#pragma unroll
-        for (int i = 0; i < NBLK; ++i) {
-            gf16x8 h8, l8;
-#pragma unroll
-            for (int e = 0; e < 8; ++e) {
-                const float v = tq[m][i][e] * sq[m];
-                const _Float16 h = (_Float16)v;
-                h8[e] = h;
-                l8[e] = (_Float16)(v - (float)h);
-            }
-            *reinterpret_cast<gf16x8*>(ph + 8 * (kb0 + TPK * i)) = h8;
-            *reinterpret_cast<gf16x8*>(pl + 8 * (kb0 + TPK * i)) = l8;
-        }
-    }
+    gfix_q_scales<NW>(redq, sq);
+    gfix_q_planes<KT, NT>(tq, tid, sq, qpl);
     __syncthreads();
     GFIX_STAMP(8);
     for (int64_t task = (int64_t)blockIdx.x * NW + w; task < ntask; task += stride) {
@@ -291,37 +341,16 @@
         const int c = (int)(task % KT);
         const bool live = rt * 32 + l31 < rows;
         if (task != task0) GFIX_LOAD_X(task)
-        f32x16 acc1, acc2;
-#pragma unroll
-        for (int i = 0; i < 16; ++i) { acc1[i] = 0.f; acc2[i] = 0.f; }
-        const _Float16* qb = qpl + (size_t)(32 * c + l31) * LDQ + 8 * hi;
-#pragma unroll
-        for (int ks = 0; ks < K / 16; ++ks) {
-            gf16x8 xh, xl, xm;
-#pragma unroll
-            for (int e = 0; e < 8; ++e) {
-                const float v = (live ? x[ks][e >> 2][e & 3] : 0.f) * sc;
-                const _Float16 h = (_Float16)v;
-                const float r1 = v - (float)h;
-                const _Float16 l = (_Float16)r1;
-                xh[e] = h; xl[e] = l; xm[e] = (_Float16)(r1 - (float)l);
-            }
-            const gf16x8 qrh = *reinterpret_cast<const gf16x8*>(qb + 16 * ks);
-            const gf16x8 qrl = *reinterpret_cast<const gf16x8*>(qb + (size_t)K * LDQ + 16 * ks);
-            const gf16x8 q0h = *reinterpret_cast<const gf16x8*>(qb + (size_t)2 * K * LDQ + 16 * ks);
-            const gf16x8 q0l = *reinterpret_cast<const gf16x8*>(qb + (size_t)3 * K * LDQ + 16 * ks);
-            acc1 = __builtin_amdgcn_mfma_f32_32x32x16_f16(xl, qrh, acc1, 0, 0, 0);
-            acc2 = __builtin_amdgcn_mfma_f32_32x32x16_f16(xm, q0h, acc2, 0, 0, 0);
-            acc1 = __builtin_amdgcn_mfma_f32_32x32x16_f16(xh, qrl, acc1, 0, 0, 0);
-            acc2 = __builtin_amdgcn_mfma_f32_32x32x16_f16(xl, q0l, acc2, 0, 0, 0);
-            acc1 = __builtin_amdgcn_mfma_f32_32x32x16_f16(xh, qrh, acc1, 0, 0, 0);
-            acc2 = __builtin_amdgcn_mfma_f32_32x32x16_f16(xl, q0h, acc2, 0, 0, 0);
-        }
-        const float u1 = 1.f / (sc * sq[1]), u2 = 1.f / (sc * sq[0]);
+        auto xrow = [&](int ks, float (&v)[8]) {
+#pragma unroll
+            for (int e = 0; e < 8; ++e) v[e] = live ? x[ks][e >> 2][e & 3] : 0.f;
+        };
+        float cv[16];
+        gfix_apply_task<KT>(xrow, qpl, c, sc, sq, cv);
 #pragma unroll
         for (int i = 0; i < 16; ++i) {
             const int64_t r = rt * 32 + (i & 3) + 8 * (i >> 2) + 4 * hi;
-            if (r < rows) out[r * a.ld + 32 * c + l31] = acc1[i] * u1 + acc2[i] * u2;
+            if (r < rows) out[r * a.ld + 32 * c + l31] = cv[i];
         }
         GFIX_STAMP(9);
     }
diff --git a/proxmin_amd/csrc/k_update.hip b/proxmin_amd/csrc/k_update.hip
--- a/proxmin_amd/csrc/k_update.hip
+++ b/proxmin_amd/csrc/k_update.hip
@@ -1616,13 +1616,18 @@
     int slots[2];
     long long* prof;
     int prof_fine;
-};
-template <int NC>
+    int gfix;
+    int gfix_xs;
+    GfixArgs gf;
+};
+constexpr int TAIL_XS_PITCH = 64 + 4;
+constexpr size_t TAIL_QPL_HALVES = (size_t)4 * 64 * (64 + 8);
+template <int NC, bool GFX = false>
 __global__ __launch_bounds__(EW_THREADS) void k_ada_tail(TailArgs a) {
     __shared__ double scratch[4 * TAIL_NT * EW_WAVES];
     __shared__ double dbuf[EW_BLOCKS + 8];
     __shared__ unsigned s_word;
-    extern __shared__ float lds[];
+    extern __shared__ __attribute__((aligned(16))) float lds[];
     static_assert(EW_BLOCKS == 2 * MAXK, "the step-size phase gives one (block, component) to each workgroup");
     DevStatus* st = a.m.status;
     if (chain_halted(st)) return;
@@ -1633,7 +1638,8 @@
     int nstamp = 0;
     auto stamp = [&]() { if (a.prof != nullptr && blockIdx.x == 0 && tid == 0) a.prof[nstamp++] = wall_clock64(); };
     stamp();
-    if (tid == 0) gb_arrive(bar, ep + 1, true);
+    static_assert(!GFX || NC == 2, "the correction's head exists at K1's K = 64");
+    if (!GFX && tid == 0) gb_arrive(bar, ep + 1, true);
     const int64_t hw = ((int64_t)blockIdx.x * EW_THREADS + tid) >> 5;
     const int64_t nhw = ((int64_t)EW_BLOCKS * EW_THREADS) >> 5;
     const int nslot = a.slots[0] + a.slots[1];
@@ -1644,7 +1650,8 @@
     bool ok[NC];
 #pragma unroll
     for (int c = 0; c < NC; ++c) ok[c] = l32 + 32 * c < K;
-    const MomentScalars ms = moment_scalars(a.m);
+    MomentScalars ms;
+    if constexpr (!GFX) ms = moment_scalars(a.m);
     const bool any_prox = a.m.has_prox[0] || a.m.has_prox[1];
 
     float g_pre[NC], x_pre[NC];
@@ -1661,6 +1668,43 @@
         alpha1[c] = ok[c] ? st->alpha[1][l32 + 32 * c] : 0.f;
     }
     const int last_tau0 = st->last_tau[0], last_tau1 = st->last_tau[1];
+    float gsc0 = 1.f, gsc1 = 1.f;
+    float* XS = lds;
+    if constexpr (GFX) {
+        {
+            static_assert(GFIX_GROUP * 32 == EW_THREADS && GFIX_PARTS == EW_BLOCKS, "k_gfix_gram's row partition is this kernel's row map");
+            XS = lds + a.gfix_xs;
+            float* fs = reinterpret_cast<float*>(scratch);
+            const float am0 = tid < 256 ? a.gf.absmax[tid] : 0.f, am1 = tid < 256 ? a.gf.absmax[256 + tid] : 0.f;
+            for (int j = 0; j < 2; ++j)
+                for (int i = 0; i < a.slots[j]; ++i) {
+                    const int64_t r = hw + (int64_t)i * nhw;
+                    float x0 = 0.f, x1 = 0.f;
+                    if (r < a.gf.rows[j]) { const float* p = a.gf.X[j] + r * 64 + l32; x0 = p[0]; x1 = p[32]; }
+                    float* d = XS + (size_t)(((j ? a.slots[0] : 0) + i) * 32 + (tid >> 5)) * TAIL_XS_PITCH + l32;
+                    d[0] = x0; d[32] = x1;
+                }
+            gsc0 = gfix_scale_of(am0, fs);
+            gsc1 = gfix_scale_of(am1, fs + 16);
+            const int w = __builtin_amdgcn_readfirstlane(tid >> 6);
+            if (w < 8) {
+                const int f = w >> 2, ns = a.slots[f];
+                const float* xs = XS + (size_t)(f ? a.slots[0] : 0) * 32 * TAIL_XS_PITCH;
+                auto fetch = [&](int i, int rr, int k) { return xs[(size_t)(i * 32 + rr) * TAIL_XS_PITCH + k]; };
+                auto scale = [&]() { return f ? gsc1 : gsc0; };
+                float* out = a.gf.part + ((int64_t)f * GFIX_PARTS + blockIdx.x) * 2 * 64 * 64;
+                switch (w & 3) {
+                    case 0: gfix_gram_job<0, false, true>(ns, scale, fetch, out); break;
+                    case 1: gfix_gram_job<1, false, true>(ns, scale, fetch, out); break;
+                    case 2: gfix_gram_job<2, false, true>(ns, scale, fetch, out); break;
+                    default: gfix_gram_job<3, false, true>(ns, scale, fetch, out); break;
+                }
+            }
+            asm volatile("s_waitcnt vmcnt(0)" ::: "memory");
+            __syncthreads();
+            if (tid == 0) gb_arrive(bar, ep + 1, true);
+        }
+    }
     {
         if (tid == 0) s_word = gb_wait(bar, ep + 1, 200000);
         __syncthreads();
@@ -1676,6 +1720,53 @@
         ep += 1;
     }
     stamp();
+    if constexpr (GFX) {
+        {
+            if (tid < 256) {
+                const int n = 2 * 64 * 64, e2 = 64 * (int)blockIdx.x + (tid >> 2);
+                gfix_reduce_entry<true, 32>(a.gf.part, a.gf.Q, n, e2 / n, e2 % n, tid & 3, true);
+            }
+            stamp();
+            ms = moment_scalars(a.m);
+            gb_sync(bar, ++ep, st);
+            stamp();
+            float* fs = reinterpret_cast<float*>(scratch) + 32;
+            _Float16* qpl = reinterpret_cast<_Float16*>(lds);
+            const int grp = tid >> 8, t = tid & 255;
+            float tq[2][2][8];
+            if (grp < 2) gfix_q_fetch<2, 256, true>(a.gf.Q + (int64_t)grp * 2 * 64 * 64, t, tq, fs + 8 * grp);
+            __syncthreads();
+            if (grp < 2) {
+                float sqg[2];
+                gfix_q_scales<4>(fs + 8 * grp, sqg);
+                gfix_q_planes<2, 256>(tq, t, sqg, qpl + (size_t)grp * TAIL_QPL_HALVES);
+            }
+            __syncthreads();
+            const int w = __builtin_amdgcn_readfirstlane(tid >> 6), lane = tid & 63, hi = lane >> 5;
+            const int grpi = w >> 1, c = w & 1;
+            const bool task = w < 2 * nslot;
+            float cv[16];
+            if (task) {
+                const int f = grpi >= a.slots[0];
+                float sq[2];
+                gfix_q_scales<4>(fs + 8 * (1 - f), sq);
+                const float* xb = XS + (size_t)(grpi * 32 + (lane & 31)) * TAIL_XS_PITCH + 8 * hi;
+                auto xrow = [&](int ks, float (&v)[8]) {
+                    const f32x4 v0 = *reinterpret_cast<const f32x4*>(xb + 16 * ks), v1 = *reinterpret_cast<const f32x4*>(xb + 16 * ks + 4);
+#pragma unroll
+                    for (int e = 0; e < 4; ++e) { v[e] = v0[e]; v[4 + e] = v1[e]; }
+                };
+                gfix_apply_task<2>(xrow, qpl + (size_t)(1 - f) * TAIL_QPL_HALVES, c, f ? gsc1 : gsc0, sq, cv);
+            }
+            __syncthreads();
+            if (task) {
+#pragma unroll
+                for (int i = 0; i < 16; ++i) XS[(size_t)(grpi * 32 + (i & 3) + 8 * (i >> 2) + 4 * hi) * TAIL_XS_PITCH + 32 * c + (lane & 31)] = cv[i];
+            }
+            __syncthreads();
+            stamp();
+        }
+    }
     float mpsi0 = -1.f, mpsi1 = -1.f;
     for (int j = 0; j < 2; ++j) {
         const int64_t rows = a.m.rows[j];
@@ -1694,6 +1785,14 @@
                 load_grad<NC>(g, ok, a.m.slab[j], rows, K, r, l32);
 #pragma unroll
                 for (int c = 0; c < NC; ++c) xo[c] = ok[c] ? a.m.X[j][r * K + l32 + 32 * c] : 0.f;
+            }
+            if constexpr (GFX) {
+                {
+                    const float* cs = XS + (size_t)(((j ? a.slots[0] : 0) + i) * 32 + (tid >> 5)) * TAIL_XS_PITCH + l32;
+#pragma unroll
+                    for (int c = 0; c < NC; ++c)
+                        if (ok[c]) g[c] += cs[32 * c];
+                }
             }
 #pragma unroll
             for (int c = 0; c < NC; ++c) {
@@ -2602,21 +2701,28 @@
     DISPATCH_NC_ME(a.s.K, seq_has_me(a.s.prox[0]) || seq_has_me(a.s.prox[1]), k_ada_finish, dim3(EW_BLOCKS, 2), s, a);
 }
 void launch_ada_decide(const AdaDecideArgs& a, hipStream_t s) { hipLaunchKernelGGL(k_ada_decide, dim3(1), dim3(EW_THREADS), 0, s, a); }
-static size_t ada_tail_lds_bytes(const TailArgs& a) {
+static size_t ada_tail_lds_bytes(const TailArgs& a, int* xs = nullptr) {
     const int NC = a.m.K <= 32 ? 1 : (a.m.K <= 64 ? 2 : 4);
     const size_t arr = (size_t)(a.slots[0] + a.slots[1]) * NC * EW_THREADS * sizeof(float);
-    return 2 * arr + std::max(arr, (size_t)(EW_THREADS / 32) * MAXK * sizeof(float));
+    size_t n = 2 * arr + std::max(arr, (size_t)(EW_THREADS / 32) * MAXK * sizeof(float));
+    if (a.gfix) {
+        n = std::max(n, 2 * TAIL_QPL_HALVES * sizeof(_Float16));
+        if (xs) *xs = (int)(n / sizeof(float));
+        n += (size_t)(a.slots[0] + a.slots[1]) * 32 * TAIL_XS_PITCH * sizeof(float);
+    }
+    return n;
 }
 constexpr size_t ADA_TAIL_LDS_MAX = 160 * 1024 - 6 * 1024;
-template <int NC>
+template <int NC, bool GFX = false>
 static hipError_t launch_ada_tail_t(const TailArgs& a, hipStream_t s) {
     const size_t lds = ada_tail_lds_bytes(a);
-    hipError_t e = hipFuncSetAttribute((const void*)k_ada_tail<NC>, hipFuncAttributeMaxDynamicSharedMemorySize, (int)lds);
+    hipError_t e = hipFuncSetAttribute((const void*)k_ada_tail<NC, GFX>, hipFuncAttributeMaxDynamicSharedMemorySize, (int)lds);
     if (e != hipSuccess) return e;
-    hipLaunchKernelGGL(k_ada_tail<NC>, dim3(EW_BLOCKS), dim3(EW_THREADS), lds, s, a);
+    hipLaunchKernelGGL((k_ada_tail<NC, GFX>), dim3(EW_BLOCKS), dim3(EW_THREADS), lds, s, a);
     return hipGetLastError();
 }
 hipError_t launch_ada_tail(const TailArgs& a, hipStream_t s) {
+    if (a.gfix) return a.m.K > 32 && a.m.K <= 64 ? launch_ada_tail_t<2, true>(a, s) : hipErrorInvalidValue;
     if (a.m.K <= 32) return launch_ada_tail_t<1>(a, s);
     if (a.m.K <= 64) return launch_ada_tail_t<2>(a, s);
     return launch_ada_tail_t<4>(a, s);
diff --git a/proxmin_amd/csrc/pmx_api.hip b/proxmin_amd/csrc/pmx_api.hip
--- a/proxmin_amd/csrc/pmx_api.hip
+++ b/proxmin_amd/csrc/pmx_api.hip
@@ -19,9 +19,9 @@
 #include "k_grad_k128.hip"
 #include "k_grad_f16_k32.hip"
 #include "k_grad_f32pc.hip"
+#include "k_gfix.hip"
 #include "k_update.hip"
 #include "k_gram.hip"
-#include "k_gfix.hip"
 #include "k_small_f64.hip"
 #include "k_grad_f64.hip"
 #include "k_big_f64.hip"
@@ -143,6 +143,8 @@
     int hook_inject_k1 = 0;
     std::string hook_tail_lockfile;
     bool tail_fused = false;
+    bool gfix_in_tail = false;
+    bool fix_by_tail = false;
     GridBar* gridbar = nullptr;
     long long* tailprof = nullptr;
     unsigned* tickets = nullptr;
@@ -653,7 +655,7 @@
     info[4] = c->plan.gridX;
     info[5] = c->plan.gridY;
     info[6] = c->plan.RP;
-    info[7] = c->chainFaults + 1000 * c->tailFaults + (c->tail_fused ? 1000000 : 0) + 10000000 * std::min(c->rangeFaults, 9);
+    info[7] = c->chainFaults + 1000 * c->tailFaults + (c->tail_fused ? (c->gfix_in_tail ? 2000000 : 1000000) : 0) + 10000000 * std::min(c->rangeFaults, 9);
     return PMX_OK;
 }
 
@@ -1132,6 +1134,7 @@
 
 static int k1_prio_for(int kk) { return kk == 64 ? 0 : 1; }
 
+constexpr bool GFIX_IN_TAIL_DEFAULT = false;
 static int enqueue_gfix(pmx_ctx* c, const float* A, const float* St, int doA, int doS, hipStream_t stream) {
     GfixArgs f{};
     f.X[0] = A; f.X[1] = St;
@@ -1202,7 +1205,7 @@
     return k1_timed(c, [&] { return launch_small_front(c->plan, g, e, c->stream); });
 }
 
-static int enqueue_grad_once(pmx_ctx* c, const float* A, const float* St, int doA, int doS, bool absmax_fresh) {
+static int enqueue_grad_once(pmx_ctx* c, const float* A, const float* St, int doA, int doS, bool absmax_fresh, bool fix_by_tail = false) {
     const K1GramFold fold = c->k1_fold;
     c->k1_fold = K1GramFold{};
     if (c->host_grad) return PMX_OK;
@@ -1307,12 +1310,14 @@
     }
     if (rc != PMX_OK) return rc;
     if (grad) c->fix_on = inst == K1_HH;
+    if (grad) c->fix_by_tail = inst == K1_HH && fix_by_tail && c->k1 == K1_F16_V8;
+    if (grad && c->fix_by_tail) return PMX_OK;
     if (inst == K1_HH) return enqueue_gfix(c, A, St, doA, doS, c->stream);
     return PMX_OK;
 }
 
-static int enqueue_grad(pmx_ctx* c, const float* A, const float* St, int doA, int doS, bool absmax_fresh = false) {
-    int rc = enqueue_grad_once(c, A, St, doA, doS, absmax_fresh);
+static int enqueue_grad(pmx_ctx* c, const float* A, const float* St, int doA, int doS, bool absmax_fresh = false, bool fix_by_tail = false) {
+    int rc = enqueue_grad_once(c, A, St, doA, doS, absmax_fresh, fix_by_tail);
     if (rc != PMX_OK || !c->k1_sync_check || !k1_fp16(c->k1) || c->host_grad || !(doA | doS)) return rc;
     rc = read_status(c);
     if (rc != PMX_OK) return rc;
@@ -1320,7 +1325,7 @@
     int again = 0;
     rc = chain_fault_fallback(c, &again);
     if (rc != PMX_OK) return rc;
-    return enqueue_grad_once(c, A, St, doA, doS, false);
+    return enqueue_grad_once(c, A, St, doA, doS, false, fix_by_tail);
 }
 
 static SlabRef slab_ref(pmx_ctx* c, int j) {
@@ -1335,7 +1340,7 @@
     }
     s.base = c->slab[j];
     s.n = j == 0 ? c->nSlabA : c->nSlabS;
-    if (c->fix_on) s.extra = c->fixSlab[j];
+    if (c->fix_on && !c->fix_by_tail) s.extra = c->fixSlab[j];
     return s;
 }
 
@@ -2591,10 +2596,19 @@
         for (int j = 0; j < 2; ++j) probe.slots[j] = (int)((c->rows[j] + 8191) / 8192);
         if (ncu >= EW_BLOCKS && ada_tail_lds_bytes(probe) <= ADA_TAIL_LDS_MAX) {
             rc = dallocT(c, &c->gridbar, 1);
-            if (rc == PMX_OK && getenv("PMX_TAIL_PROF")) rc = dallocT(c, &c->tailprof, 16);
+            if (rc == PMX_OK && getenv("PMX_TAIL_PROF")) rc = dallocT(c, &c->tailprof, 24);
             if (rc != PMX_OK) return rc;
             c->tail_fused = true;
         }
+    }
+    c->gfix_in_tail = false;
+    if (c->tail_fused && c->k1 == K1_F16_V8 && c->Kk == 64 && c->W == nullptr && !c->comm && !c->ssplit && c->fixPart != nullptr &&
+        (getenv("PMX_GFIX_IN_TAIL") ? atoi(getenv("PMX_GFIX_IN_TAIL")) != 0 : GFIX_IN_TAIL_DEFAULT)) {
+        TailArgs probe{};
+        probe.m.K = (int)c->K;
+        probe.gfix = 1;
+        for (int j = 0; j < 2; ++j) probe.slots[j] = (int)((c->rows[j] + 8191) / 8192);
+        c->gfix_in_tail = c->K > 32 && 2 * (probe.slots[0] + probe.slots[1]) <= EW_WAVES && ada_tail_lds_bytes(probe) <= ADA_TAIL_LDS_MAX;
     }
     AlphaArgs al = alpha_args(c);
     al.use_fixed = p->use_fixed_steps;
@@ -2708,6 +2722,18 @@
     t.bar = c->gridbar;
     t.prof = c->tailprof;
     t.prof_fine = getenv("PMX_TAIL_PROF") && atoi(getenv("PMX_TAIL_PROF")) == 2;
+    if (c->fix_by_tail) {
+        t.gfix = 1;
+        t.gf.X[0] = c->Kk != c->K ? c->Xk[0] : c->X[0]; t.gf.X[1] = c->Kk != c->K ? c->Xk[1] : c->X[1];
+        t.gf.rows[0] = c->M; t.gf.rows[1] = c->N;
+        t.gf.K = (int)c->Kk;
+        t.gf.absmax = c->absmax;
+        t.gf.part = c->fixPart; t.gf.Q = c->fixQ;
+        t.gf.ld = (int)c->Kk;
+        t.gf.want[0] = t.gf.want[1] = 1;
+        t.gf.status = c->dstatus;
+        (void)ada_tail_lds_bytes(t, &t.gfix_xs);
+    }
     const char* lockfile = c->hook_tail_lockfile.empty() ? nullptr : c->hook_tail_lockfile.c_str();
     int lockfd = -1;
     if (lockfile) {
@@ -2855,7 +2881,7 @@
         for (int i = 0; i < chunk; ++i) {
             const int gi = done + i;
             if (c->tail_fused) {
-                rc = enqueue_grad(c, c->X[0], c->X[1], 1, 1, tails > 0);
+                rc = enqueue_grad(c, c->X[0], c->X[1], 1, 1, tails > 0, c->gfix_in_tail);
                 if (rc == PMX_OK) rc = ada_enqueue_tail_fused(c, it0 + gi, b1[gi], gi == 0 ? b1_prev : b1[gi - 1]);
                 ++tails;
                 if (rc != PMX_OK) return rc;
@@ -2897,14 +2923,18 @@
         if (c->hstatus->halt && c->hstatus->reason == HALT_ERROR) FAIL(PMX_E_HIP, "%s", chain_error_text(c));
     }
     if (c->tailprof && c->tail_fused) {
-        long long h[16];
+        long long h[24];
         HIP_CHECK(hipMemcpy(h, c->tailprof, sizeof(h), hipMemcpyDeviceToHost));
         static const char* nm[] = {"census", "moment", "B1", "maxpsi", "sub", "B2", "judge+replay", "finish", "B3", "decide"};
         static const char* nf[] = {"census", "moment", "B1", "maxpsi", "passesA", "sumsA", "passesS", "sumsS", "(end)", "B2", "judge+replay", "finish", "B3", "decide"};
+        static const char* nh[] = {"gfixR", "gfixB", "gfixA"};
         const bool fine = getenv("PMX_TAIL_PROF") && atoi(getenv("PMX_TAIL_PROF")) == 2;
-        const int np = fine ? 14 : 10;
+        const int nhead = c->fix_by_tail ? 3 : 0, np = (fine ? 14 : 10) + nhead;
         fprintf(stderr, "[tailprof] us:");
-        for (int i = 0; i < np; ++i) fprintf(stderr, " %s=%.2f", fine ? nf[i] : nm[i], (double)(h[i + 1] - h[i]) / 100.0);
+        for (int i = 0; i < np; ++i) {
+            const char* name = i == 0 ? (nhead ? "gfixG+census" : "census") : i <= nhead ? nh[i - 1] : fine ? nf[i - nhead] : nm[i - nhead];
+            fprintf(stderr, " %s=%.2f", name, (double)(h[i + 1] - h[i]) / 100.0);
+        }
         fprintf(stderr, " total=%.2f\n", (double)(h[np] - h[0]) / 100.0);
     }
     fill_result(c, res, it0);
diff --git a/proxmin_amd/engine.py b/proxmin_amd/engine.py
--- a/proxmin_amd/engine.py
+++ b/proxmin_amd/engine.py
@@ -384,6 +384,11 @@
         _lib.check(self.lib.pmx_time_grad(self.h, int(do_A), int(do_S), int(reps), C.byref(ms)))
         return ms.value
 
+    def gfix_in_tail(self):
+        v = (C.c_int * 8)()
+        _lib.check(self.lib.pmx_k1_info(self.h, v))
+        return (v[7] // 1000000) % 10 == 2
+
     def k1_info(self):
         v = (C.c_int * 8)()
         _lib.check(self.lib.pmx_k1_info(self.h, v))
```

Result: no change. 2849 (-0.1%).
